# zhibaishouheilab/HealthiVert-GAN

Hardware: AMD Instinct MI355X
Metric: sagittal slices/sec (train step, G+D) at 256x256 bs=16 (higher is better)
Workload: dtype f16; 1 GPU; two-stage coarse+refine generator + 3x PatchGAN D train step, 256x256, per-GPU bs=16, norm=batch, vanilla GAN; global_batch=16, parallelism=dp1, launch=hipGraph replay (1 graphs/step), 4 streams

## Files before the change

healthivert-gan_amd/csrc/conv_g4.hip:

```cpp
#include <stdlib.h>
#include <type_traits>

#include "conv_halo.h"

struct G4K {
    const void* x; const _Float16* w; const float* bias; void* y; const void* mul_src;
    float* stats;
    const void* bn_x; const float* bn_stats; float* bstats;
    int bn_x_ld, bn_x_coff, bn_ipg;
    int B, H, W, x_ld, x_coff, Cin;
    int Ho, Wo, y_ld, y_coff, Cout;
    int mul_ld, mul_coff, mul_act, act, accumulate;
    float alpha;
    int tiles_x, tiles;
    int Hc, Wc;
    unsigned x_bytes, w_bytes, w_rb;
    int dbg;
};

typedef __attribute__((address_space(3))) void* lds_ptr;
__device__ __forceinline__ void lds_dma16(__amdgpu_buffer_rsrc_t r, lds_ptr dst, unsigned voff, int soff) {
#if defined(__HIP_DEVICE_COMPILE__)
    __builtin_amdgcn_raw_ptr_buffer_load_lds(r, dst, 16, voff, soff, 0, 0);
#endif
}

__device__ __forceinline__ void g4_load_bias(const G4K& p, int cob, int lane, f32x4 (&bias_r)[4]) {
    const __amdgpu_buffer_rsrc_t bsrc = __builtin_amdgcn_make_buffer_rsrc(const_cast<float*>(p.bias), 0, p.bias ? (unsigned)p.Cout * 4u : 0u, 0x00020000);
#pragma unroll
    for (int n = 0; n < 4; ++n)
        bias_r[n] = __builtin_bit_cast(f32x4, __builtin_amdgcn_raw_buffer_load_b128(bsrc, (unsigned)(cob + n * 16 + (lane >> 4) * 4) * 4u, 0, 0));
}

template <int MODE, int MT>
__device__ __forceinline__ void g4_epilogue(const G4K& p, f32x4 (&acc)[4][MT], char* smem, const int (&cls_s)[2], const int (&cob_s)[2], int n_img, int i0,
                                            int j0, const f32x4 (&bias_r)[4]) {
    constexpr int TW = 16, TH = 4 * MT, NTHR = 512, LDO = 128 + 8;
    const int tid = threadIdx.x, lane = tid & 63, wave = __builtin_amdgcn_readfirstlane(tid >> 6);
    const int wm = wave >> 1, wn = wave & 1;
    _Float16* As = reinterpret_cast<_Float16*>(smem);
    constexpr int OITEMS = TH * TW * 16 / NTHR;
    const __amdgpu_buffer_rsrc_t msrc = __builtin_amdgcn_make_buffer_rsrc(const_cast<void*>(p.mul_src), 0, p.mul_src ? 0x7ffffff0u : 0u, 0x00020000);
    const __amdgpu_buffer_rsrc_t ysrc = __builtin_amdgcn_make_buffer_rsrc(p.y, 0, p.accumulate ? 0x7ffffff0u : 0u, 0x00020000);
    u32x4 mreg[OITEMS], yreg[OITEMS];
    long long ooff[OITEMS];
#pragma unroll
    for (int k = 0; k < OITEMS; ++k) {
        const int it = tid + k * NTHR;
        const int q = it >> 4, pc = it & 15, s = pc >> 3;
        const int i = i0 + (q >> 4), j = j0 + (q & 15);
        const int ch = cob_s[s] + (pc & 7) * 8;
        const bool ok = i < p.Hc && j < p.Wc && ch < p.Cout;
        int ho = i, wo = j;
        if (MODE == 1) { ho = 2 * i + (cls_s[s] >> 1); wo = 2 * j + (cls_s[s] & 1); }
        const long long opix = (long long)(n_img * p.Ho + ho) * p.Wo + wo;
        ooff[k] = ok ? opix * p.y_ld + p.y_coff + ch : -1;
        mreg[k] = __builtin_amdgcn_raw_buffer_load_b128(msrc, ok ? (unsigned)((opix * p.mul_ld + p.mul_coff + ch) * 2) : HV_OOB, 0, 0);
        yreg[k] = __builtin_amdgcn_raw_buffer_load_b128(ysrc, ok ? (unsigned)(ooff[k] * 2) : HV_OOB, 0, 0);
    }
    _Float16* ot = As;
    auto stage = [&](auto actf) __attribute__((always_inline)) {
#pragma unroll
        for (int m = 0; m < MT; ++m) {
            const int q = (wm * MT + m) * 16 + (lane & 15);
#pragma unroll
            for (int n = 0; n < 4; ++n) {
                f16x4v h;
#pragma unroll
                for (int r = 0; r < 4; ++r) h[r] = (_Float16)actf(acc[n][m][r] * p.alpha + bias_r[n][r]);
                *reinterpret_cast<f16x4v*>(ot + q * LDO + wn * 64 + n * 16 + (lane >> 4) * 4) = h;
            }
        }
    };
    switch (p.act) {
        case HV_ACT_ELU:
            stage([](float v) { const float e = __builtin_amdgcn_exp2f(v * 1.44269504f) - 1.f, sm = v + 0.5f * v * v; return v > 0.f ? v : (v > -0.00390625f ? sm : e); });
            break;
        case HV_ACT_RELU: stage([](float v) { return v > 0.f ? v : 0.f; }); break;
        case HV_ACT_LRELU: stage([](float v) { return v > 0.f ? v : 0.2f * v; }); break;
        case HV_ACT_SIGMOID: stage([](float v) { return __builtin_amdgcn_rcpf(1.f + __builtin_amdgcn_exp2f(-v * 1.44269504f)); }); break;
        case HV_ACT_CLAMP: stage([](float v) { return fminf(fmaxf(v, -1.f), 1.f); }); break;
        default: stage([](float v) { return v; }); break;
    }
    __syncthreads();
    _Float16* yb = reinterpret_cast<_Float16*>(p.y);
    u32x4 o[OITEMS];
#pragma unroll
    for (int k = 0; k < OITEMS; ++k) {
        const int it = tid + k * NTHR;
        o[k] = *reinterpret_cast<const u32x4*>(ot + (it >> 4) * LDO + (it & 15) * 8);
    }
    if (MODE != 1 && p.stats) {
        float s1[8], s2[8];
#pragma unroll
        for (int e = 0; e < 8; ++e) s1[e] = s2[e] = 0.f;
#pragma unroll
        for (int k = 0; k < OITEMS; ++k) {
            if (ooff[k] < 0) continue;
            const f16x8 v8 = __builtin_bit_cast(f16x8, o[k]);
#pragma unroll
            for (int e = 0; e < 8; ++e) { const float v = (float)v8[e]; s1[e] += v; s2[e] += v * v; }
        }
        __syncthreads();
        float* red = reinterpret_cast<float*>(smem);
        float* mine = red + ((tid >> 4) * 16 + (tid & 15)) * 16;
#pragma unroll
        for (int e = 0; e < 8; ++e) { mine[e] = s1[e]; mine[8 + e] = s2[e]; }
        __syncthreads();
        if (tid < 256) {
            const int pc = tid >> 4, e = tid & 15;
            float s = 0.f;
#pragma unroll 8
            for (int r = 0; r < 32; ++r) s += red[(r * 16 + pc) * 16 + e];
            const int ch = (int)blockIdx.y * 128 + pc * 8 + (e & 7);
            if (ch < p.Cout) p.stats[((long long)blockIdx.x * p.Cout + ch) * 2 + (e >> 3)] = s;
        }
    }
    if (p.mul_src) {
        auto mulf = [&](auto gradf) __attribute__((always_inline)) {
#pragma unroll
            for (int k = 0; k < OITEMS; ++k) {
                const f16x8 m8 = __builtin_bit_cast(f16x8, mreg[k]);
                f16x8 v8 = __builtin_bit_cast(f16x8, o[k]);
#pragma unroll
                for (int e = 0; e < 8; ++e) v8[e] = (_Float16)((float)v8[e] * gradf((float)m8[e]));
                o[k] = __builtin_bit_cast(u32x4, v8);
            }
        };
        switch (p.mul_act) {
            case HV_ACT_ELU: mulf([](float y) { return y > 0.f ? 1.f : y + 1.f; }); break;
            case HV_ACT_RELU: mulf([](float y) { return y > 0.f ? 1.f : 0.f; }); break;
            case HV_ACT_LRELU: mulf([](float y) { return y > 0.f ? 1.f : 0.2f; }); break;
            case HV_ACT_SIGMOID: mulf([](float y) { return y * (1.f - y); }); break;
            case HV_ACT_CLAMP: mulf([](float y) { return (y > -1.f && y < 1.f) ? 1.f : 0.f; }); break;
            default: break;
        }
    }
    if (p.accumulate) {
#pragma unroll
        for (int k = 0; k < OITEMS; ++k) {
            const f16x8 y8 = __builtin_bit_cast(f16x8, yreg[k]);
            f16x8 v8 = __builtin_bit_cast(f16x8, o[k]);
#pragma unroll
            for (int e = 0; e < 8; ++e) v8[e] = (_Float16)((float)v8[e] + (float)y8[e]);
            o[k] = __builtin_bit_cast(u32x4, v8);
        }
    }
#pragma unroll
    for (int k = 0; k < OITEMS; ++k)
        if (ooff[k] >= 0) *reinterpret_cast<u32x4*>(yb + ooff[k]) = o[k];
    if (p.bstats) {
        const int pc = tid & 15, s = pc >> 3;
        const int ch0 = cob_s[s] + (pc & 7) * 8;
        const int grp = n_img / p.bn_ipg;
        const __amdgpu_buffer_rsrc_t xsrc = __builtin_amdgcn_make_buffer_rsrc(const_cast<void*>(p.bn_x), 0, 0x7ffffff0u, 0x00020000);
        u32x4 xreg[OITEMS];
#pragma unroll
        for (int k = 0; k < OITEMS; ++k) {
            const int q = (tid + k * NTHR) >> 4;
            int ho = i0 + (q >> 4), wo = j0 + (q & 15);
            if (MODE == 1) { ho = 2 * ho + (cls_s[s] >> 1); wo = 2 * wo + (cls_s[s] & 1); }
            const long long opix = (long long)(n_img * p.Ho + ho) * p.Wo + wo;
            xreg[k] = __builtin_amdgcn_raw_buffer_load_b128(xsrc, ooff[k] >= 0 ? (unsigned)((opix * p.bn_x_ld + p.bn_x_coff + ch0) * 2) : HV_OOB, 0, 0);
        }
        float s1[8], s2[8];
#pragma unroll
        for (int e = 0; e < 8; ++e) s1[e] = s2[e] = 0.f;
#pragma unroll
        for (int k = 0; k < OITEMS; ++k) {
            if (ooff[k] < 0) continue;
            const f16x8 v8 = __builtin_bit_cast(f16x8, o[k]), x8 = __builtin_bit_cast(f16x8, xreg[k]);
#pragma unroll
            for (int e = 0; e < 8; ++e) {
                const float g = (float)v8[e];
                s1[e] += g; s2[e] += g * (float)x8[e];
            }
        }
        __syncthreads();
        float* red = reinterpret_cast<float*>(smem);
        float* mine = red + ((tid >> 4) * 16 + (tid & 15)) * 16;
#pragma unroll
        for (int e = 0; e < 8; ++e) { mine[e] = s1[e]; mine[8 + e] = s2[e]; }
        __syncthreads();
        if (tid < 128) {
            const int pq = tid >> 3, e = tid & 7;
            float sg = 0.f, sgx = 0.f;
#pragma unroll 8
            for (int r = 0; r < 32; ++r) { sg += red[(r * 16 + pq) * 16 + e]; sgx += red[(r * 16 + pq) * 16 + 8 + e]; }
            const int sl = pq >> 3, ch = cob_s[sl] + (pq & 7) * 8 + e;
            const long long part = MODE == 1 ? (long long)blockIdx.x * 4 + cls_s[sl] : (long long)blockIdx.x;
            if (ch < p.Cout) {
                const float mean = p.bn_stats[(long long)grp * 2 * p.Cout + ch], rstd = p.bn_stats[(long long)grp * 2 * p.Cout + p.Cout + ch];
                float* o2 = p.bstats + (part * p.Cout + ch) * 2;
                o2[0] = sg;
                o2[1] = rstd * (sgx - mean * sg);
            }
        }
    }
}

template <int MODE, int MT>
__global__ __launch_bounds__(512, 2) void conv_g4_kernel(const G4K p) {
    constexpr int TW = 16, TH = 4 * MT, NTHR = 512;
    constexpr int PH = TH + 1 + MODE, PW = TW + 1 + MODE;
    constexpr int NBP = (PH * PW + 15) / 16;
    constexpr int BPW = (NBP + 7) / 8;
    constexpr int ABUF = 32 * 512;
    constexpr int BBUF = NBP * 512;
    constexpr int NBUF = 3;
    constexpr int LDO = 128 + 8;
    extern __shared__ __attribute__((aligned(16))) char smem[];
    _Float16* As = reinterpret_cast<_Float16*>(smem);
    _Float16* Bs = As + NBUF * ABUF;

    const int tid = threadIdx.x, lane = tid & 63, wave = __builtin_amdgcn_readfirstlane(tid >> 6);
#ifdef G4_STAMPS
    unsigned long long st[8];
#define G4_STAMP(i) st[i] = __builtin_amdgcn_s_memrealtime()
#else
#define G4_STAMP(i)
#endif
    G4_STAMP(0);
    const int wm = wave >> 1, wn = wave & 1;
    int t = (int)blockIdx.x;
    const int n_img = t / p.tiles;
    t -= n_img * p.tiles;
    const int tile_y = t / p.tiles_x, tile_x = t - tile_y * p.tiles_x;
    const int i0 = tile_y * TH, j0 = tile_x * TW;
    const int Cin = p.Cin, KC = Cin >> 5;
    const int NCH = MODE == 0 ? 4 * KC : KC;

    int cls_s[2], cob_s[2];
#pragma unroll
    for (int s = 0; s < 2; ++s) {
        if (MODE == 0) { cls_s[s] = 0; cob_s[s] = (int)blockIdx.y * 128 + s * 64; }
        else {
            const int nco = p.Cout >> 6, sl = (int)blockIdx.y * 2 + s;
            cls_s[s] = sl / nco; cob_s[s] = (sl - cls_s[s] * nco) * 64;
        }
    }
    const __amdgpu_buffer_rsrc_t wsrc = __builtin_amdgcn_make_buffer_rsrc(const_cast<_Float16*>(p.w), 0, p.w_bytes, 0x00020000);
    const __amdgpu_buffer_rsrc_t xsrc = __builtin_amdgcn_make_buffer_rsrc(const_cast<void*>(p.x), 0, p.x_bytes, 0x00020000);
    f32x4 bias_r[4];
    g4_load_bias(p, cob_s[wn], lane, bias_r);

    int pbase[BPW], pval[BPW];
    const int xbase = (n_img * p.H * p.W * p.x_ld + p.x_coff) * 2;
#pragma unroll
    for (int i = 0; i < BPW; ++i) {
        const int pix = (wave + 8 * i) * 16 + (lane >> 2);
        const int c8 = (lane & 3) ^ (((pix >> 2) & 1) << 1);
        const int pr = pix / PW, pc = pix - pr * PW;
        const bool in = pix < PH * PW && wave + 8 * i < NBP;
        if (MODE == 0) {
            const int r0 = 2 * (i0 + pr) - 1, c0 = 2 * (j0 + pc) - 1;
            pbase[i] = xbase + ((r0 * p.W + c0) * p.x_ld + c8 * 8) * 2;
            int v = 0;
#pragma unroll
            for (int dd = 0; dd < 4; ++dd)
                if (in && (unsigned)(r0 + (dd >> 1)) < (unsigned)p.H && (unsigned)(c0 + (dd & 1)) < (unsigned)p.W) v |= 1 << dd;
            pval[i] = v;
        } else {
            const int r0 = i0 - 1 + pr, c0 = j0 - 1 + pc;
            pbase[i] = xbase + ((r0 * p.W + c0) * p.x_ld + c8 * 8) * 2;
            pval[i] = (in && (unsigned)r0 < (unsigned)p.H && (unsigned)c0 < (unsigned)p.W) ? 15 : 0;
        }
    }
    constexpr int DMA_PER_CHUNK = 4 + BPW;
    auto issue = [&](int c, int b) __attribute__((always_inline)) {
        int dy = 0, dx = 0, kc = c;
        if (MODE == 0) { dy = c / (2 * KC); const int rem = c - dy * 2 * KC; dx = rem / KC; kc = rem - dx * KC; }
#pragma unroll
        for (int i = 0; i < 4; ++i) {
            const int f = wave + 8 * i, rbw = f >> 2, tt = f & 3, s = rbw >> 2;
            const int rb = (cob_s[s] >> 4) + (rbw & 3);
            int tap;
            if (MODE == 0) tap = (2 * (tt >> 1) + dy) * 4 + 2 * (tt & 1) + dx;
            else { const int py = cls_s[s] >> 1, px = cls_s[s] & 1; tap = (1 - py + 2 * (tt >> 1)) * 4 + (1 - px + 2 * (tt & 1)); }
            lds_dma16(wsrc, (lds_ptr)(As + b * ABUF + f * 512), (unsigned)lane * 16u, rb * (int)p.w_rb + (tap * Cin + kc * 32) * 32);
        }
        const int coff = MODE == 0 ? ((dy * p.W + dx) * p.x_ld + kc * 32) * 2 : kc * 64;
        const int vb = MODE == 0 ? dy * 2 + dx : 0;
#pragma unroll
        for (int i = 0; i < BPW; ++i) {
            _Float16* dst = wave + 8 * i < NBP ? Bs + b * BBUF + (wave + 8 * i) * 512 : Bs + NBUF * BBUF;
            lds_dma16(xsrc, (lds_ptr)dst, ((pval[i] >> vb) & 1) ? (unsigned)(pbase[i] + coff) : HV_OOB, 0);
        }
    };

    int boffs[4][MT];
#pragma unroll
    for (int tt = 0; tt < 4; ++tt) {
        int dh, dw;
        if (MODE == 0) { dh = tt >> 1; dw = tt & 1; }
        else { const int py = cls_s[wn] >> 1, px = cls_s[wn] & 1; dh = py - (tt >> 1) + 1; dw = px - (tt & 1) + 1; }
#pragma unroll
        for (int m = 0; m < MT; ++m) {
            const int pix = (wm * MT + m + dh) * PW + (lane & 15) + dw;
            boffs[tt][m] = pix * 32 + (((lane >> 4) ^ (((pix >> 2) & 1) << 1)) << 3);
        }
    }
    f32x4 acc[4][MT];
#pragma unroll
    for (int n = 0; n < 4; ++n)
#pragma unroll
        for (int m = 0; m < MT; ++m) acc[n][m] = (f32x4){0.f, 0.f, 0.f, 0.f};
    const int aoff = (wn * 16) * 512 + lane * 8;

    f16x8 a[2][4], bf[2][MT];
    auto frags = [&](int b, int tt, int buf) __attribute__((always_inline)) {
        const _Float16* Ab = As + b * ABUF + aoff;
        const _Float16* Bb = Bs + b * BBUF;
#pragma unroll
        for (int n = 0; n < 4; ++n) a[buf][n] = *reinterpret_cast<const f16x8*>(Ab + (n * 4 + tt) * 512);
#pragma unroll
        for (int m = 0; m < MT; ++m) bf[buf][m] = *reinterpret_cast<const f16x8*>(Bb + boffs[tt][m]);
    };
    auto mfmas = [&](int buf) __attribute__((always_inline)) {
#ifdef G4_STAMPS
        if (p.dbg & 4) return;
#endif
#pragma unroll
        for (int m = 0; m < MT; ++m)
#pragma unroll
            for (int n = 0; n < 4; ++n) acc[n][m] = __builtin_amdgcn_mfma_f32_16x16x32_f16(a[buf][n], bf[buf][m], acc[n][m], 0, 0, 0);
    };
    auto chunk = [&](int c, int b) __attribute__((always_inline)) {
        const int bn = b == 2 ? 0 : b + 1;
#ifdef G4_STAMPS
        if (c + 2 < NCH && !(p.dbg & 1)) issue(c + 2, b == 0 ? 2 : b - 1);
#else
        if (c + 2 < NCH) issue(c + 2, b == 0 ? 2 : b - 1);
#endif
#pragma unroll
        for (int tt = 0; tt < 3; ++tt) {
            __builtin_amdgcn_sched_barrier(0);
            frags(b, tt + 1, (tt + 1) & 1);
            mfmas(tt & 1);
#pragma unroll
            for (int i = 0; i < 4 + MT; ++i) {
                __builtin_amdgcn_sched_group_barrier(0x100, 1, 0);
                __builtin_amdgcn_sched_group_barrier(0x008, (4 * MT) / (4 + MT), 0);
            }
            __builtin_amdgcn_sched_barrier(0);
        }
        if (c + 2 < NCH) __builtin_amdgcn_s_waitcnt(0x0070 | (DMA_PER_CHUNK & 15) | ((DMA_PER_CHUNK >> 4) << 14));
        else __builtin_amdgcn_s_waitcnt(0x0070);
        __builtin_amdgcn_s_barrier();
        if (c + 1 < NCH) frags(bn, 0, 0);
        mfmas(1);
#pragma unroll
        for (int i = 0; i < 4 + MT; ++i) {
            __builtin_amdgcn_sched_group_barrier(0x100, 1, 0);
            __builtin_amdgcn_sched_group_barrier(0x008, (4 * MT) / (4 + MT), 0);
        }
        __builtin_amdgcn_sched_barrier(0);
    };
    issue(0, 0);
    if (NCH > 1) issue(1, 1);
    G4_STAMP(1);
    if (NCH > 1) __builtin_amdgcn_s_waitcnt(0x0F70 | (DMA_PER_CHUNK & 15) | ((DMA_PER_CHUNK >> 4) << 14));
    else __builtin_amdgcn_s_waitcnt(0x0F70);
    __builtin_amdgcn_s_barrier();
    G4_STAMP(2);
    frags(0, 0, 0);
    for (int c = 0; c < NCH; c += 3) {
        chunk(c, 0);
        if (c + 1 < NCH) chunk(c + 1, 1);
        if (c + 2 < NCH) chunk(c + 2, 2);
    }
    __syncthreads();
    G4_STAMP(3);

    g4_epilogue<MODE, MT>(p, acc, smem, cls_s, cob_s, n_img, i0, j0, bias_r);
#ifdef G4_STAMPS
    __builtin_amdgcn_s_waitcnt(0);
    G4_STAMP(5);
    if (tid == 0 && blockIdx.x == gridDim.x / 2 && blockIdx.y == 0) {
        unsigned long long* d = reinterpret_cast<unsigned long long*>(p.y);
        for (int i = 0; i < 6; ++i) d[i] = st[i];
    }
#endif
}

template <int DG, int MT>
__device__ __forceinline__ void conv_g4s1_body(const G4K& p) {
    constexpr int TW = 16, TH = 4 * MT, PH = TH + 3, PW = 20;
    constexpr int NBP = (PH * PW + 15) / 16, BPW = (NBP + 7) / 8;
    static_assert(BPW <= 4, "one patch piece per tap");
    constexpr int ABUF = 32 * 512, BBUF = NBP * 512;
    extern __shared__ __attribute__((aligned(16))) char smem[];
    _Float16* As = reinterpret_cast<_Float16*>(smem);
    _Float16* Bs = As + 3 * ABUF;
    const int tid = threadIdx.x, lane = tid & 63, wave = __builtin_amdgcn_readfirstlane(tid >> 6);
    const int wm = wave >> 1, wn = wave & 1;
#ifdef G4_STAMPS
    unsigned long long st[8];
    st[0] = __builtin_amdgcn_s_memrealtime();
#endif
    int t = (int)blockIdx.x;
    const int n_img = t / p.tiles;
    t -= n_img * p.tiles;
    const int tile_y = t / p.tiles_x, tile_x = t - tile_y * p.tiles_x;
    const int i0 = tile_y * TH, j0 = tile_x * TW;
    const int Cin = p.Cin, KC = Cin >> 5, NS = 4 * KC;
    int cls_s[2] = {0, 0}, cob_s[2] = {(int)blockIdx.y * 128, (int)blockIdx.y * 128 + 64};
    const __amdgpu_buffer_rsrc_t wsrc = __builtin_amdgcn_make_buffer_rsrc(const_cast<_Float16*>(p.w), 0, p.w_bytes, 0x00020000);
    const __amdgpu_buffer_rsrc_t xsrc = __builtin_amdgcn_make_buffer_rsrc(const_cast<void*>(p.x), 0, p.x_bytes, 0x00020000);
    f32x4 bias_r[4];
    g4_load_bias(p, cob_s[wn], lane, bias_r);
    constexpr int ORG = DG ? 2 : 1;
    unsigned pvo[BPW];
    const int xbase = (n_img * p.H * p.W * p.x_ld + p.x_coff) * 2;
#pragma unroll
    for (int i = 0; i < BPW; ++i) {
        const int pix = (wave + 8 * i) * 16 + (lane >> 2);
        const int c8 = (lane & 3) ^ (((pix >> 2) & 1) << 1);
        const int pr = pix / PW, pc = pix - pr * PW;
        const int r0 = i0 - ORG + pr, c0 = j0 - ORG + pc;
        const bool ok = wave + 8 * i < NBP && pr < PH && pc < PW - 1 && (unsigned)r0 < (unsigned)p.H && (unsigned)c0 < (unsigned)p.W;
        pvo[i] = ok ? (unsigned)(xbase + ((r0 * p.W + c0) * p.x_ld + c8 * 8) * 2) : HV_OOB;
    }
    auto issueA = [&](int kc, int kh, int ab) __attribute__((always_inline)) {
#pragma unroll
        for (int i = 0; i < 4; ++i) {
            const int f = wave + 8 * i, rbw = f >> 2, kw = f & 3;
            const int rb = (cob_s[rbw >> 2] >> 4) + (rbw & 3);
            lds_dma16(wsrc, (lds_ptr)(As + ab * ABUF + f * 512), (unsigned)lane * 16u, rb * (int)p.w_rb + ((kh * 4 + kw) * Cin + kc * 32) * 32);
        }
    };
    auto issueA1 = [&](int kc, int kh, int ab, int i, bool live) __attribute__((always_inline)) {
        const int f = wave + 8 * i, rbw = f >> 2, kw = f & 3;
        const int rb = (cob_s[rbw >> 2] >> 4) + (rbw & 3);
        lds_dma16(wsrc, (lds_ptr)(As + ab * ABUF + f * 512), live ? (unsigned)lane * 16u : HV_OOB, rb * (int)p.w_rb + ((kh * 4 + kw) * Cin + kc * 32) * 32);
    };
    auto issueB1 = [&](int kc, int bb, int i, bool live) __attribute__((always_inline)) {
        _Float16* dst = wave + 8 * i < NBP ? Bs + bb * BBUF + (wave + 8 * i) * 512 : Bs + 2 * BBUF;
        lds_dma16(xsrc, (lds_ptr)dst, live ? pvo[i] : HV_OOB, kc * 64);
    };
    auto issueB = [&](int kc, int bb) __attribute__((always_inline)) {
#pragma unroll
        for (int i = 0; i < BPW; ++i) {
            _Float16* dst = wave + 8 * i < NBP ? Bs + bb * BBUF + (wave + 8 * i) * 512 : Bs + 2 * BBUF;
            lds_dma16(xsrc, (lds_ptr)dst, pvo[i], kc * 64);
        }
    };
    int bo[2][4][MT];
#pragma unroll
    for (int kw = 0; kw < 4; ++kw)
#pragma unroll
        for (int m = 0; m < MT; ++m) {
            const int pix = (wm * MT + m) * PW + (lane & 15) + (DG ? 3 - kw : kw);
            const int s0 = (pix >> 2) & 1;
            bo[0][kw][m] = pix * 32 + (((lane >> 4) ^ (s0 << 1)) << 3);
            bo[1][kw][m] = pix * 32 + (((lane >> 4) ^ ((s0 ^ 1) << 1)) << 3);
        }
    f32x4 acc[4][MT];
#pragma unroll
    for (int n = 0; n < 4; ++n)
#pragma unroll
        for (int m = 0; m < MT; ++m) acc[n][m] = (f32x4){0.f, 0.f, 0.f, 0.f};
    const int aoff = (wn * 16) * 512 + lane * 8;
    f16x8 a[2][4], bf[2][MT];
    auto sub = [&](int kc, auto KH, int ab) __attribute__((always_inline)) {
        constexpr int kh = decltype(KH)::value;
        constexpr int rs = DG ? 3 - kh : kh;
        const int s_ = kc * 4 + kh;
        constexpr int kh2 = (kh + 2) & 3;
        const int kc2 = kc + (kh >= 2 ? 1 : 0);
        const int ab2 = ab == 0 ? 2 : ab - 1;
        const bool live = s_ + 2 < NS;
        const _Float16* Ab = As + ab * ABUF + aoff;
        const _Float16* Bb = Bs + (kc & 1) * BBUF + rs * PW * 32;
        auto frags = [&](int kw, int buf) __attribute__((always_inline)) {
#pragma unroll
            for (int n = 0; n < 4; ++n) a[buf][n] = *reinterpret_cast<const f16x8*>(Ab + (n * 4 + kw) * 512);
#pragma unroll
            for (int m = 0; m < MT; ++m) bf[buf][m] = *reinterpret_cast<const f16x8*>(Bb + bo[rs & 1][kw][m]);
        };
        frags(0, 0);
#pragma unroll
        for (int kw = 0; kw < 4; ++kw) {
            __builtin_amdgcn_sched_barrier(0);
            issueA1(kc2, kh2, ab2, kw, live);
            if (kh == 2 && kw < BPW) issueB1(kc + 1, (kc + 1) & 1, kw, live);
            __builtin_amdgcn_sched_barrier(0);
            if (kw + 1 < 4) frags(kw + 1, (kw + 1) & 1);
#pragma unroll
            for (int m = 0; m < MT; ++m)
#pragma unroll
                for (int n = 0; n < 4; ++n) acc[n][m] = __builtin_amdgcn_mfma_f32_16x16x32_f16(a[kw & 1][n], bf[kw & 1][m], acc[n][m], 0, 0, 0);
            if (kw + 1 < 4) {
#pragma unroll
                for (int i = 0; i < 4 + MT; ++i) {
                    __builtin_amdgcn_sched_group_barrier(0x100, 1, 0);
                    __builtin_amdgcn_sched_group_barrier(0x008, (4 * MT) / (4 + MT), 0);
                }
            }
            __builtin_amdgcn_sched_barrier(0);
        }
        if (kh == 2) __builtin_amdgcn_s_waitcnt(0x0070 | ((4 + BPW) & 15));
        else __builtin_amdgcn_s_waitcnt(0x0070 | 4);
        __builtin_amdgcn_s_barrier();
    };
    issueB(0, 0);
    issueA(0, 0, 0);
    issueA(0, 1, 1);
    __builtin_amdgcn_s_waitcnt(0x0F70 | 4);
    __builtin_amdgcn_s_barrier();
#ifdef G4_STAMPS
    st[1] = __builtin_amdgcn_s_memrealtime();
#endif
    int ab = 0;
    for (int kc = 0; kc < KC; ++kc) {
        sub(kc, std::integral_constant<int, 0>(), ab); ab = ab == 2 ? 0 : ab + 1;
        sub(kc, std::integral_constant<int, 1>(), ab); ab = ab == 2 ? 0 : ab + 1;
        sub(kc, std::integral_constant<int, 2>(), ab); ab = ab == 2 ? 0 : ab + 1;
        sub(kc, std::integral_constant<int, 3>(), ab); ab = ab == 2 ? 0 : ab + 1;
    }
    __builtin_amdgcn_s_waitcnt(0x0F70);
    __syncthreads();
#ifdef G4_STAMPS
    st[2] = __builtin_amdgcn_s_memrealtime();
#endif
    g4_epilogue<0, MT>(p, acc, smem, cls_s, cob_s, n_img, i0, j0, bias_r);
#ifdef G4_STAMPS
    st[3] = __builtin_amdgcn_s_memrealtime();
    __builtin_amdgcn_s_waitcnt(0);
    st[4] = __builtin_amdgcn_s_memrealtime();
    if (tid == 0 && blockIdx.x == gridDim.x / 2 && blockIdx.y == 0) {
        unsigned long long* d = reinterpret_cast<unsigned long long*>(p.y);
        for (int i = 0; i < 5; ++i) d[i] = st[i];
    }
#endif
}

template <int DG, int MT>
__global__ __launch_bounds__(512, 2) void conv_g4s1_kernel(const G4K p) { conv_g4s1_body<DG, MT>(p); }

template <int DG, int MT>
static int launch_g4s1(G4K& k, int ny, hipStream_t s) {
    constexpr int TH = 4 * MT, PH = TH + 3, NBP = (PH * 20 + 15) / 16;
    constexpr size_t lds_loop = (size_t)(3 * 32 * 512 + (2 * NBP + 1) * 512) * 2, lds_out = (size_t)TH * 16 * 136 * 2, lds_red = 32 * 16 * 16 * 4;
    constexpr size_t lds = lds_loop > lds_out ? (lds_loop > lds_red ? lds_loop : lds_red) : (lds_out > lds_red ? lds_out : lds_red);
    static_assert(lds <= 160 * 1024, "LDS");
    k.tiles_x = hv_cdiv(k.Wc, 16);
    k.tiles = k.tiles_x * hv_cdiv(k.Hc, TH);
    auto kern = conv_g4s1_kernel<DG, MT>;
    static bool raised = false;
    if (!raised) {
        hipError_t e = hipFuncSetAttribute(reinterpret_cast<const void*>(kern), hipFuncAttributeMaxDynamicSharedMemorySize, 160 * 1024);
        if (e != hipSuccess) return -1000 - (int)e;
        raised = true;
    }
    hv_path_note = 8;
    HV_KNAME("conv_g4s1_kernel<%d, %d>", DG, MT);
    HV_WUSE(4);
    hipLaunchKernelGGL(kern, dim3(k.tiles * k.B, ny), dim3(512), lds, s, k);
    HV_LAUNCH_CHECK();
    return HV_OK;
}

template <int MODE, int MT>
static int launch_g4(G4K& k, int ny, hipStream_t s) {
    constexpr int TH = 4 * MT, PH = TH + 1 + MODE, PW = 17 + MODE;
    constexpr size_t lds_loop = (size_t)(3 * 32 * 512 + (3 * ((PH * PW + 15) / 16) + 1) * 512) * 2, lds_out = (size_t)TH * 16 * 136 * 2, lds_red = 32 * 16 * 16 * 4;
    constexpr size_t lds = lds_loop > lds_out ? (lds_loop > lds_red ? lds_loop : lds_red) : (lds_out > lds_red ? lds_out : lds_red);
    static_assert(lds <= 160 * 1024, "LDS");
    k.tiles_x = hv_cdiv(k.Wc, 16);
    k.tiles = k.tiles_x * hv_cdiv(k.Hc, TH);
    auto kern = conv_g4_kernel<MODE, MT>;
    static bool raised = false;
    if (!raised) {
        hipError_t e = hipFuncSetAttribute(reinterpret_cast<const void*>(kern), hipFuncAttributeMaxDynamicSharedMemorySize, 160 * 1024);
        if (e != hipSuccess) return -1000 - (int)e;
        raised = true;
    }
    hv_path_note = 8;
    HV_KNAME("conv_g4_kernel<%d, %d>", MODE, MT);
    HV_WUSE(4);
    hipLaunchKernelGGL(kern, dim3(k.tiles * k.B, ny), dim3(512), lds, s, k);
    HV_LAUNCH_CHECK();
    return HV_OK;
}

static int g4_tile_rows(int B, int Hc, int Wc, int ny) {
    return (long long)B * hv_cdiv(Hc, 16) * hv_cdiv(Wc, 16) * ny >= 200 ? 16 : 8;
}

size_t hv_conv2d_g4_bstats_parts(const hv_conv_desc* d);
static bool g4_eligible(const hv_conv_desc* d) {
    if (d->KH != 4 || d->KW != 4 || (d->stride != 2 && d->stride != 1) || d->pad != 1 || d->dil != 1 || d->in_shift || d->w_bstride || d->ch_scale) return false;
    if (d->precision != HV_F16 || !d->w_f16_tiled || !d->x_f16 || !d->y_f16 || d->accumulate > 1) return false;
    if (d->stride == 1) {
        if ((d->Cout & 127) || (d->Cin & 31)) return false;
    }
    if ((d->Cin & 31) || (d->Cout & 63) || (!d->transposed && (d->Cout & 127))) return false;
    if ((d->x_ld & 7) || (d->x_coff & 7) || ((uintptr_t)d->x & 15) || (d->y_ld & 7) || (d->y_coff & 7) || ((uintptr_t)d->y & 15) || ((uintptr_t)d->w_f16_tiled & 15))
        return false;
    if (d->mul_src && (!d->mul_f16 || (d->mul_ld & 7) || (d->mul_coff & 7) || ((uintptr_t)d->mul_src & 15))) return false;
    if (d->stride == 2 && !d->transposed && (d->Ho != d->H / 2 || d->Wo != d->W / 2 || (d->H & 1) || (d->W & 1))) return false;
    if (d->stride == 2 && d->transposed && (d->Ho != 2 * d->H || d->Wo != 2 * d->W)) return false;
    if (d->stride == 1 && (d->Ho != d->H + (d->transposed ? 1 : -1) || d->Wo != d->W + (d->transposed ? 1 : -1) || d->Ho < 1 || d->Wo < 1)) return false;
    if ((long long)d->B * d->H * d->W * d->x_ld >= (1ll << 30) || (long long)d->B * d->Ho * d->Wo * d->y_ld >= (1ll << 30)) return false;
    return true;
}

int hv_conv2d_g4(const hv_conv_desc* d, hipStream_t s) {
    if (!g4_eligible(d)) return HV_ERR_UNSUPPORTED;
    G4K k;
    k.dbg = 0;
#ifdef G4_STAMPS
    if (getenv("HV_G4_DBG")) k.dbg = atoi(getenv("HV_G4_DBG"));
#endif
    k.x = d->x; k.w = reinterpret_cast<const _Float16*>(d->w_f16_tiled); k.bias = d->bias; k.y = d->y; k.mul_src = d->mul_src;
    k.stats = d->transposed ? nullptr : d->stats;
    k.bn_x = nullptr; k.bn_stats = nullptr; k.bstats = nullptr; k.bn_x_ld = k.bn_x_coff = 0; k.bn_ipg = 1;
    if (d->bstats) {
        if (!hv_conv2d_g4_bstats_parts(d)) return HV_ERR_UNSUPPORTED;
        k.bn_x = d->bn_x; k.bn_stats = d->bn_stats; k.bstats = d->bstats; k.bn_x_ld = d->bn_x_ld; k.bn_x_coff = d->bn_x_coff;
        k.bn_ipg = d->B / (d->bn_groups > 0 ? d->bn_groups : 1);
    }
    k.B = d->B; k.H = d->H; k.W = d->W; k.x_ld = d->x_ld; k.x_coff = d->x_coff; k.Cin = d->Cin;
    k.Ho = d->Ho; k.Wo = d->Wo; k.y_ld = d->y_ld; k.y_coff = d->y_coff; k.Cout = d->Cout;
    k.mul_ld = d->mul_ld; k.mul_coff = d->mul_coff; k.mul_act = d->mul_act; k.act = d->act; k.accumulate = d->accumulate; k.alpha = d->alpha;
    k.x_bytes = (unsigned)((size_t)d->B * d->H * d->W * d->x_ld * 2);
    k.w_rb = (unsigned)(16 * 16 * d->Cin * 2);
    k.w_bytes = (unsigned)((size_t)hv_cdiv(d->Cout, 16) * k.w_rb);
    if (d->stride == 1) {
        k.Hc = d->Ho; k.Wc = d->Wo;
        const int ny = d->Cout / 128;
        k.stats = d->transposed ? nullptr : d->stats;
        if (g4_tile_rows(d->B, k.Hc, k.Wc, ny) == 16) return d->transposed ? launch_g4s1<1, 4>(k, ny, s) : launch_g4s1<0, 4>(k, ny, s);
        return d->transposed ? launch_g4s1<1, 2>(k, ny, s) : launch_g4s1<0, 2>(k, ny, s);
    }
    if (!d->transposed) {
        k.Hc = d->Ho; k.Wc = d->Wo;
        const int ny = d->Cout / 128;
        return g4_tile_rows(d->B, k.Hc, k.Wc, ny) == 16 ? launch_g4<0, 4>(k, ny, s) : launch_g4<0, 2>(k, ny, s);
    }
    k.Hc = d->H; k.Wc = d->W;
    const int ny = 2 * (d->Cout / 64);
    return g4_tile_rows(d->B, k.Hc, k.Wc, ny) == 16 ? launch_g4<1, 4>(k, ny, s) : launch_g4<1, 2>(k, ny, s);
}

size_t hv_conv2d_g4_bstats_parts(const hv_conv_desc* d) {
    if (!d->transposed || d->accumulate || !g4_eligible(d)) return 0;
    if (!d->bn_x || !d->bn_stats || !d->mul_src || (d->bn_x_ld & 7) || (d->bn_x_coff & 7) || ((uintptr_t)d->bn_x & 15) || ((uintptr_t)d->bn_stats & 15) || (d->Cout & 7)) return 0;
    const int G = d->bn_groups > 0 ? d->bn_groups : 1;
    if (d->B % G) return 0;
    if ((long long)d->B * d->Ho * d->Wo * d->bn_x_ld >= (1ll << 30)) return 0;
    if (d->stride == 1) {
        const int th = g4_tile_rows(d->B, d->Ho, d->Wo, d->Cout / 128);
        return (size_t)d->B * hv_cdiv(d->Ho, th) * hv_cdiv(d->Wo, 16);
    }
    const int th = g4_tile_rows(d->B, d->H, d->W, 2 * (d->Cout / 64));
    return (size_t)d->B * hv_cdiv(d->H, th) * hv_cdiv(d->W, 16) * 4;
}

size_t hv_conv2d_g4_stats_floats(const hv_conv_desc* d, int* nparts) {
    hv_conv_desc t = *d;
    if (t.transposed || t.accumulate || !g4_eligible(&t)) return 0;
    const int th = g4_tile_rows(t.B, t.Ho, t.Wo, t.Cout / 128);
    const int parts = t.B * hv_cdiv(t.Ho, th) * hv_cdiv(t.Wo, 16);
    if (nparts) *nparts = parts;
    return (size_t)parts * t.Cout * 2;
}
```

healthivert-gan_amd/csrc/conv_igemm.hip:

```cpp
#include <string.h>

#include "hv_common.h"
#include <stdlib.h>

#define HV_MAX_TAPS 25
#define HV_BK 32

thread_local int hv_path_note = 0;
thread_local int hv_wtable_used = 0;
extern "C" int hv_last_weight_tables(void) { return hv_wtable_used; }
thread_local char hv_kname[192] = "";
extern "C" const char* hv_last_kernel_name(void) { return hv_kname; }
extern "C" int hv_last_kernel_path(void) { return hv_path_note; }
thread_local hipEvent_t hv_ev_start = nullptr, hv_ev_stop = nullptr;
extern "C" int hv_set_kernel_timing(void* ev_start, void* ev_stop) {
    hv_ev_start = (hipEvent_t)ev_start; hv_ev_stop = (hipEvent_t)ev_stop;
    return HV_OK;
}

int hv_conv2d_halo(const hv_conv_desc* d, const void* w_f16, hipStream_t s);
int hv_conv2d_g4(const hv_conv_desc* d, hipStream_t s);
int hv_conv2d_thin_dgrad(const hv_conv_desc* d, hipStream_t s);
int hv_conv2d_logits_dgrad(const hv_conv_desc* d, hipStream_t s);
size_t hv_conv2d_g4_stats_floats(const hv_conv_desc* d, int* nparts);
size_t hv_conv2d_g4_bstats_parts(const hv_conv_desc* d);
size_t hv_conv2d_logits_bstats_parts(const hv_conv_desc* d);
size_t hv_wgrad_halo_workspace_bytes(const hv_wgrad_desc* d);
int hv_wgrad_halo(const hv_wgrad_desc* d, int* nslabs, hipStream_t s);
size_t hv_wgrad_tr_workspace_bytes(const hv_wgrad_desc* d);
int hv_wgrad_tr(const hv_wgrad_desc* d, int* nslabs, hipStream_t s);
int hv_wgrad_thin(const hv_wgrad_desc* d, int* nslabs, hipStream_t s);
size_t hv_wgrad_thin_workspace_bytes(const hv_wgrad_desc* d);
int hv_conv2d_narrow(const hv_conv_desc* d, hipStream_t s);
int hv_conv2d_thin_in(const hv_conv_desc* d, hipStream_t s);
int hv_conv2d_stem5(const hv_conv_desc* d, hipStream_t s);
int hv_conv2d_stem5_dgrad(const hv_conv_desc* d, hipStream_t s);
int hv_conv2d_head(const hv_conv_desc* d, hipStream_t s);
int hv_conv2d_px(const hv_conv_desc* d, hipStream_t s);
int hv_conv2d_s2t(const hv_conv_desc* d, hipStream_t s);

struct ConvCls {
    int ph, pw, Hc, Wc, ntaps, Ktot, m0, mcount;
    uint32_t taps[HV_MAX_TAPS];
};
struct ConvK {
    const void* x; const float* w; const float* bias; const float* scale; void* y;
    int x_half, y_half, mul_half;
    long long w_bs, scale_bs;
    int B, Hl, Wl, in_shift, Wp, img_stride, x_ld, x_coff, Cin;
    int Cout, w_row, y_ld, y_coff, Ho, Wo;
    int bstep, boff, ostep;
    float alpha; int act, accumulate, vec_store, ncls;
    int xcd_swizzle;
    const void* mul_src; int mul_ld, mul_coff, mul_act, mul_vec;
    ConvCls cls[4];
};

template <typename T> struct Stage;
template <> struct Stage<float> {
    static constexpr int LD = HV_BK + 4;
    static __device__ __forceinline__ void st4(float* dst, float4 v) { *reinterpret_cast<float4*>(dst) = v; }
};
template <> struct Stage<_Float16> {
    static constexpr int LD = HV_BK + 8;
    static __device__ __forceinline__ void st4(_Float16* dst, float4 v) {
        f16x4 h = {(_Float16)v.x, (_Float16)v.y, (_Float16)v.z, (_Float16)v.w};
        *reinterpret_cast<f16x4*>(dst) = h;
    }
};

template <typename T, int MT, int NT> struct Frags;
template <int MT, int NT> struct Frags<float, MT, NT> {
    float4 w[NT][2], x[MT][2];
    __device__ __forceinline__ void load(const float* Bs, const float* As, int wrow0, int xrow0, int lane) {
        const int off = (lane & 15) * Stage<float>::LD + (lane >> 4) * 8;
#pragma unroll
        for (int n = 0; n < NT; ++n) {
            const float* p = Bs + (wrow0 + n * 16) * Stage<float>::LD + off;
            w[n][0] = *reinterpret_cast<const float4*>(p);
            w[n][1] = *reinterpret_cast<const float4*>(p + 4);
        }
#pragma unroll
        for (int m = 0; m < MT; ++m) {
            const float* p = As + (xrow0 + m * 16) * Stage<float>::LD + off;
            x[m][0] = *reinterpret_cast<const float4*>(p);
            x[m][1] = *reinterpret_cast<const float4*>(p + 4);
        }
    }
    __device__ __forceinline__ void mma(f32x4 (&acc)[NT][MT]) {
#pragma unroll
        for (int n = 0; n < NT; ++n)
#pragma unroll
            for (int m = 0; m < MT; ++m) {
                f32x4 a = acc[n][m];
                a = __builtin_amdgcn_mfma_f32_16x16x4f32(w[n][0].x, x[m][0].x, a, 0, 0, 0);
                a = __builtin_amdgcn_mfma_f32_16x16x4f32(w[n][0].y, x[m][0].y, a, 0, 0, 0);
                a = __builtin_amdgcn_mfma_f32_16x16x4f32(w[n][0].z, x[m][0].z, a, 0, 0, 0);
                a = __builtin_amdgcn_mfma_f32_16x16x4f32(w[n][0].w, x[m][0].w, a, 0, 0, 0);
                a = __builtin_amdgcn_mfma_f32_16x16x4f32(w[n][1].x, x[m][1].x, a, 0, 0, 0);
                a = __builtin_amdgcn_mfma_f32_16x16x4f32(w[n][1].y, x[m][1].y, a, 0, 0, 0);
                a = __builtin_amdgcn_mfma_f32_16x16x4f32(w[n][1].z, x[m][1].z, a, 0, 0, 0);
                a = __builtin_amdgcn_mfma_f32_16x16x4f32(w[n][1].w, x[m][1].w, a, 0, 0, 0);
                acc[n][m] = a;
            }
    }
};
template <int MT, int NT> struct Frags<_Float16, MT, NT> {
    f16x8 w[NT], x[MT];
    __device__ __forceinline__ void load(const _Float16* Bs, const _Float16* As, int wrow0, int xrow0, int lane) {
        const int off = (lane & 15) * Stage<_Float16>::LD + (lane >> 4) * 8;
#pragma unroll
        for (int n = 0; n < NT; ++n) w[n] = *reinterpret_cast<const f16x8*>(Bs + (wrow0 + n * 16) * Stage<_Float16>::LD + off);
#pragma unroll
        for (int m = 0; m < MT; ++m) x[m] = *reinterpret_cast<const f16x8*>(As + (xrow0 + m * 16) * Stage<_Float16>::LD + off);
    }
    __device__ __forceinline__ void mma(f32x4 (&acc)[NT][MT]) {
#pragma unroll
        for (int n = 0; n < NT; ++n)
#pragma unroll
            for (int m = 0; m < MT; ++m) acc[n][m] = __builtin_amdgcn_mfma_f32_16x16x32_f16(w[n], x[m], acc[n][m], 0, 0, 0);
    }
};

template <typename T, int BM, int BN, int WM, int WN, bool ASC, bool XH>
__global__ __launch_bounds__(256) void conv_igemm_kernel(const ConvK p) {
    constexpr int LD = Stage<T>::LD;
    constexpr int APASS = BM / 32;
    constexpr int BPASS = (BN + 31) / 32;
    constexpr int TMW = BM / WM, TNW = BN / WN;
    constexpr int MT = TMW / 16, NT = TNW / 16;
    static_assert(WM * WN == 4 && MT >= 1 && NT >= 1, "bad tile");
    __shared__ __attribute__((aligned(16))) T As[BM * LD];
    __shared__ __attribute__((aligned(16))) T Bs[BN * LD];
    __shared__ uint32_t taps_s[32];

    const int tid = threadIdx.x, lane = tid & 63, wave = tid >> 6;
    int bx = blockIdx.x;
    if (p.xcd_swizzle) {
        const int q = gridDim.x >> 3, r = gridDim.x & 7, xcd = bx & 7, loc = bx >> 3;
        bx = xcd < r ? xcd * (q + 1) + loc : r * (q + 1) + (xcd - r) * q + loc;
    }
    int ci = 0;
#pragma unroll
    for (int i = 1; i < 4; ++i)
        if (i < p.ncls && bx >= p.cls[i].m0) ci = i;
    const ConvCls& C = p.cls[ci];
    const int ntaps = C.ntaps, Ktot = C.Ktot, Hc = C.Hc, Wc = C.Wc, Mc = C.mcount, ph = C.ph, pw = C.pw;
    if (tid < ntaps) taps_s[tid] = C.taps[tid];
    const int m_base = (bx - C.m0) * BM;
    const int n_base = blockIdx.y * BN;
    const int HWc = Hc * Wc;

    const int chunk = tid & 7, prow = tid >> 3;
    int a_nb[APASS], a_hw[APASS];
    const int sample0 = m_base / HWc;
#pragma unroll
    for (int i = 0; i < APASS; ++i) {
        const int m = m_base + prow + i * 32;
        int bh = -20000, bw = -20000, nb = 0;
        if (m < Mc) {
            const int n = m / HWc, rem = m - n * HWc;
            const int ii = rem / Wc, jj = rem - ii * Wc;
            bh = ii * p.bstep + p.boff;
            bw = jj * p.bstep + p.boff;
            nb = n * p.img_stride;
        }
        a_nb[i] = nb;
        a_hw[i] = (int)(((uint32_t)bh << 16) | ((uint32_t)bw & 0xffffu));
    }
    const float* wbase = p.w + (p.w_bs ? (long long)sample0 * p.w_bs : 0ll);
    const int nk = (Ktot + HV_BK - 1) / HV_BK;

    float4 ra[APASS], rb[BPASS];
    auto gload = [&](int kt) {
        const int kg = kt * HV_BK + chunk * 4;
        if (!ASC) {
            const bool kok = kg < Ktot;
            int tapi = 0, c = 0, dh = 0, dw = 0, widx = 0;
// ... 26 lines not shown
            int dh[4], dw[4], wo[4], cc[4];
            bool kok[4];
#pragma unroll
            for (int e4 = 0; e4 < 4; ++e4) {
                const int k = kg + e4;
                kok[e4] = k < Ktot;
                const int tapi = kok[e4] ? k / p.Cin : 0;
                cc[e4] = k - tapi * p.Cin;
                const uint32_t e = taps_s[tapi];
                dh[e4] = (int)(int8_t)(e & 0xff);
                dw[e4] = (int)(int8_t)((e >> 8) & 0xff);
                wo[e4] = (int)(e >> 16) * p.Cin + cc[e4];
            }
#pragma unroll
            for (int i = 0; i < APASS; ++i) {
                float v[4];
#pragma unroll
                for (int e4 = 0; e4 < 4; ++e4) {
                    const int hi = (a_hw[i] >> 16) + dh[e4], wi = (int)(int16_t)(a_hw[i] & 0xffff) + dw[e4];
                    v[e4] = 0.f;
                    if (kok[e4] && (unsigned)hi < (unsigned)p.Hl && (unsigned)wi < (unsigned)p.Wl)
                        v[e4] = hv_ld1(p.x, a_nb[i] + ((hi >> p.in_shift) * p.Wp + (wi >> p.in_shift)) * p.x_ld + p.x_coff + cc[e4], XH);
                }
                ra[i] = make_float4(v[0], v[1], v[2], v[3]);
            }
#pragma unroll
            for (int i = 0; i < BPASS; ++i) {
                const int r = prow + i * 32, n = n_base + r;
                float v[4];
#pragma unroll
                for (int e4 = 0; e4 < 4; ++e4) v[e4] = (kok[e4] && r < BN && n < p.Cout) ? wbase[(long long)n * p.w_row + wo[e4]] : 0.f;
                rb[i] = make_float4(v[0], v[1], v[2], v[3]);
            }
        }
    };
    auto lstore = [&]() {
#pragma unroll
        for (int i = 0; i < APASS; ++i) Stage<T>::st4(As + (prow + i * 32) * LD + chunk * 4, ra[i]);
#pragma unroll
        for (int i = 0; i < BPASS; ++i) {
            const int r = prow + i * 32;
            if (r < BN) Stage<T>::st4(Bs + r * LD + chunk * 4, rb[i]);
        }
    };

    f32x4 acc[NT][MT];
#pragma unroll
    for (int n = 0; n < NT; ++n)
#pragma unroll
        for (int m = 0; m < MT; ++m) acc[n][m] = (f32x4){0.f, 0.f, 0.f, 0.f};

    const int wm = wave / WN, wn = wave % WN;
    __syncthreads();
    if (nk > 0) {
        gload(0);
        lstore();
    }
    __syncthreads();
    Frags<T, MT, NT> fr;
    for (int kt = 0; kt < nk; ++kt) {
        const bool more = kt + 1 < nk;
        if (more) gload(kt + 1);
        fr.load(Bs, As, wn * TNW, wm * TMW, lane);
        fr.mma(acc);
        __syncthreads();
        if (more) lstore();
        __syncthreads();
    }

    const float* scale = p.scale ? p.scale + (p.scale_bs ? (long long)sample0 * p.scale_bs : 0ll) : nullptr;
    const HvEpi epi = {p.alpha, p.act, p.accumulate, p.vec_store, p.Cout, p.bias, scale, p.mul_act, p.mul_vec, p.y_half, p.mul_half};
#pragma unroll
    for (int m = 0; m < MT; ++m) {
        const int mm = m_base + wm * TMW + m * 16 + (lane & 15);
        if (mm >= Mc) continue;
        const int n = mm / HWc, rem = mm - n * HWc;
        const int ii = rem / Wc, jj = rem - ii * Wc;
        const int ho = ph + ii * p.ostep, wo = pw + jj * p.ostep;
        const long long opix = (long long)(n * p.Ho + ho) * p.Wo + wo;
        void* yp = hv_eptr(p.y, opix * p.y_ld + p.y_coff, p.y_half);
        const void* mp = p.mul_src ? hv_eptr(p.mul_src, opix * p.mul_ld + p.mul_coff, p.mul_half) : nullptr;
#pragma unroll
        for (int nn = 0; nn < NT; ++nn) {
            const int ch0 = n_base + wn * TNW + nn * 16 + (lane >> 4) * 4;
            hv_conv_epilogue4<!std::is_same<T, float>::value>(epi, acc[nn][m], ch0, yp, mp);
        }
    }
}

template <typename T, int BM, int BN, int WM, int WN, bool ASC>
static int launch_conv(const ConvK& k, int mtiles, hipStream_t s) {
    dim3 grid(mtiles, hv_cdiv(k.Cout, BN));
    const bool xh = sizeof(T) == 2 && k.x_half;
    HV_KNAME("conv_igemm_kernel<%s, %d, %d, %d, %d, %s, %s>", sizeof(T) == 2 ? "_Float16" : "float", BM, BN, WM, WN, ASC ? "true" : "false", xh ? "true" : "false");
    if constexpr (sizeof(T) == 2) {
        if (xh) {
            hipLaunchKernelGGL((conv_igemm_kernel<T, BM, BN, WM, WN, ASC, true>), grid, dim3(256), 0, s, k);
            HV_LAUNCH_CHECK();
            return HV_OK;
        }
    }
    hipLaunchKernelGGL((conv_igemm_kernel<T, BM, BN, WM, WN, ASC, false>), grid, dim3(256), 0, s, k);
    HV_LAUNCH_CHECK();
    return HV_OK;
}

template <typename T, bool ASC>
static int dispatch_conv(ConvK& k, hipStream_t s) {
    long long M = 0;
    for (int c = 0; c < k.ncls; ++c) M += k.cls[c].mcount;
    int BM, BN;
    if (k.Cout <= 16) { BN = 16; BM = 256; }
    else if (k.Cout <= 32) { BN = 32; BM = 256; }
    else if (k.Cout <= 64) { BN = 64; BM = 128; }
    else { BN = 128; BM = 128; }
    if (BN >= 64) {
        long long tiles = ((M + BM - 1) / BM) * ((k.Cout + BN - 1) / BN);
        constexpr long long kSmallTiles = 600;
        if (tiles < kSmallTiles) { BM = 64; BN = 64; }
    } else if (BN == 16 && (M + 255) / 256 < 256) {
        BM = 64;
    }
    if (k.w_bs || k.scale_bs) {
        for (int c = 0; c < k.ncls; ++c)
            if ((k.cls[c].Hc * k.cls[c].Wc) % BM) {
                if ((k.cls[c].Hc * k.cls[c].Wc) % 64 == 0) { BM = 64; BN = 64; }
                else return HV_ERR_UNSUPPORTED;
            }
    }
    int mt = 0;
    for (int c = 0; c < k.ncls; ++c) {
        k.cls[c].m0 = mt;
        mt += hv_cdiv(k.cls[c].mcount, BM);
    }
    if (mt <= 0) return HV_OK;
    {
        const int gy = (k.Cout + BN - 1) / BN;
        k.xcd_swizzle = (mt >= 64 && (gy == 1 || (mt & 7) == 0)) ? 1 : 0;
    }
    if (BM == 256 && BN == 16) return launch_conv<T, 256, 16, 4, 1, ASC>(k, mt, s);
    if (BM == 64 && BN == 16) return launch_conv<T, 64, 16, 4, 1, ASC>(k, mt, s);
    if (BM == 256 && BN == 32) return launch_conv<T, 256, 32, 4, 1, ASC>(k, mt, s);
    if (BM == 128 && BN == 64) return launch_conv<T, 128, 64, 2, 2, ASC>(k, mt, s);
    if (BM == 128 && BN == 128) return launch_conv<T, 128, 128, 2, 2, ASC>(k, mt, s);
    return launch_conv<T, 64, 64, 2, 2, ASC>(k, mt, s);
}

extern "C" size_t hv_conv2d_bstats_parts(const hv_conv_desc* d) {
    if (!d || !d->transposed || d->precision != HV_F16) return 0;
    if (d->Cin == 4 && d->KH == 4 && d->stride == 1) return hv_conv2d_logits_bstats_parts(d);
    return hv_conv2d_g4_bstats_parts(d);
}

static int conv2d_dispatch(const hv_conv_desc* d, void* stream) {
    hv_wtable_used = 0;
    if (!d || !d->x || !d->w || !d->y) return HV_ERR_ARG;
    if (d->B <= 0 || d->H <= 0 || d->W <= 0 || d->Cin <= 0 || d->Cout <= 0 || d->KH <= 0 || d->KW <= 0 ||
        d->stride <= 0 || d->dil <= 0 || d->pad < 0 || d->Ho <= 0 || d->Wo <= 0)
        return HV_ERR_ARG;
    if (d->KH * d->KW > HV_MAX_TAPS || d->in_shift < 0 || d->in_shift > 1) return HV_ERR_UNSUPPORTED;
    if (d->in_shift && ((d->H | d->W) & 1)) return HV_ERR_UNSUPPORTED;
    if (d->x_ld < d->x_coff + d->Cin || d->y_ld < d->y_coff + d->Cout) return HV_ERR_ARG;
    if (d->act < HV_ACT_NONE || d->act > HV_ACT_CLAMP) return HV_ERR_ARG;
    if (d->precision != HV_F32 && d->precision != HV_F16) return HV_ERR_ARG;
    if (d->precision == HV_F32 && (d->x_f16 || d->y_f16 || d->mul_f16)) return HV_ERR_UNSUPPORTED;
    const int Hp = d->H >> d->in_shift, Wp = d->W >> d->in_shift;
    if ((long long)d->B * Hp * Wp * d->x_ld >= (1ll << 31) || (long long)d->B * d->Ho * d->Wo * d->y_ld >= (1ll << 31))
        return HV_ERR_UNSUPPORTED;
    if (d->H > 16000 || d->W > 16000 || (d->KH - 1) * d->dil > 120 || (d->KW - 1) * d->dil > 120) return HV_ERR_UNSUPPORTED;

    if (d->stats && !hv_conv2d_g4_stats_floats(d, nullptr)) return HV_ERR_UNSUPPORTED;
    if (d->bstats && !hv_conv2d_bstats_parts(d)) return HV_ERR_UNSUPPORTED;
    if (d->xn_stats) {
        if (d->Cout != 1 || !d->workspace) return HV_ERR_UNSUPPORTED;
        return hv_conv2d_head(d, (hipStream_t)stream);
    }
    if (d->x1) {
        if (d->precision != HV_F16 || !d->w_f16 || !d->w_f16_tiled || !d->y_f16 || d->transposed || d->dil != 1 || d->stride != 1 || d->KH != 3 || d->KW != 3 || !d->w1 ||
            d->pool2 || d->stats || d->x1_ld < 1)
            return HV_ERR_UNSUPPORTED;
        return hv_conv2d_halo(d, d->w_f16, (hipStream_t)stream);
    }
    if (d->pool2) {
        if (d->precision != HV_F16 || !d->w_f16 || !d->y_f16 || (d->Ho & 1) || (d->Wo & 1) || d->dil != 1 || d->stride != 1 || d->KH != 3 || d->KW != 3 || d->bias ||
            d->act != HV_ACT_NONE || d->in_shift || d->stats)
            return HV_ERR_UNSUPPORTED;
        return hv_conv2d_halo(d, d->w_f16, (hipStream_t)stream);
    }
    if (d->precision == HV_F16 && d->Cin <= 16 && d->Cout <= 16 && d->stride == 1) {
        const int rc = hv_conv2d_px(d, (hipStream_t)stream);
        if (rc != HV_ERR_UNSUPPORTED) return rc;
    }
    constexpr int kNarrowMaxCin = 15;
    const bool halo_ok = d->precision == HV_F16 && d->w_f16 && d->dil == 1 && (d->Cin & 15) == 0 && !d->w_bstride && !d->ch_scale;
    if (d->Cout == 1 && d->workspace) {
        const int rc = hv_conv2d_head(d, (hipStream_t)stream);
        if (rc != HV_ERR_UNSUPPORTED) return rc;
    }
    if (d->Cout == 1 && !d->transposed && !d->mul_src && !(halo_ok && d->Cin > kNarrowMaxCin)) {
        const int rc = hv_conv2d_narrow(d, (hipStream_t)stream);
        if (rc != HV_ERR_UNSUPPORTED) return rc;
    }
    if (d->Cin <= 4 && !d->transposed && !d->mul_src) {
        const int rc = hv_conv2d_thin_in(d, (hipStream_t)stream);
        if (rc != HV_ERR_UNSUPPORTED) return rc;
    }
    if (d->Cin == 4 && d->KH == 5 && d->precision == HV_F16 && d->w_f16) {
        const int rc = hv_conv2d_stem5(d, (hipStream_t)stream);
        if (rc != HV_ERR_UNSUPPORTED) return rc;
    }
    if (d->Cout == 4 && d->Cin == 16 && d->KH == 5 && d->transposed && d->precision == HV_F16 && d->w_f16) {
        const int rc = hv_conv2d_stem5_dgrad(d, (hipStream_t)stream);
        if (rc != HV_ERR_UNSUPPORTED) return rc;
    }
    if (d->precision == HV_F16 && d->transposed && d->Cin == 4 && d->KH == 4 && d->stride == 1) {
        const int rc = hv_conv2d_logits_dgrad(d, (hipStream_t)stream);
        if (rc != HV_ERR_UNSUPPORTED) return rc;
    }
    if (d->precision == HV_F16 && d->transposed && d->Cin <= 4 && d->KH == 3) {
        const int rc = hv_conv2d_thin_dgrad(d, (hipStream_t)stream);
        if (rc != HV_ERR_UNSUPPORTED) return rc;
    }
    if (d->precision == HV_F16 && d->w_f16 && d->KH == 4 && d->w_f16_tiled) {
        const int rc = hv_conv2d_g4(d, (hipStream_t)stream);
        if (rc != HV_ERR_UNSUPPORTED) return rc;
    }
    if (d->precision == HV_F16 && d->w_f16 && d->transposed && d->stride == 2) {
        const int rc = hv_conv2d_s2t(d, (hipStream_t)stream);
        if (rc != HV_ERR_UNSUPPORTED) return rc;
    }
    if (d->precision == HV_F16 && d->w_f16) {
        const int rc = hv_conv2d_halo(d, d->w_f16, (hipStream_t)stream);
        if (rc != HV_ERR_UNSUPPORTED) return rc;
    }
    ConvK k;
    k.x_half = d->x_f16 ? 1 : 0; k.y_half = d->y_f16 ? 1 : 0; k.mul_half = d->mul_f16 ? 1 : 0;
    k.x = d->x; k.w = d->w; k.bias = d->bias; k.scale = d->ch_scale; k.y = d->y;
    k.w_bs = d->w_bstride; k.scale_bs = d->ch_scale ? d->ch_scale_bstride : 0;
    k.mul_src = d->mul_src; k.mul_ld = d->mul_ld; k.mul_coff = d->mul_coff; k.mul_act = d->mul_act;
    k.mul_vec = (d->mul_src && !(d->mul_ld & 3) && !(d->mul_coff & 3) && !((uintptr_t)d->mul_src & 15)) ? 1 : 0;
    k.B = d->B; k.Hl = d->H; k.Wl = d->W; k.in_shift = d->in_shift; k.Wp = Wp; k.img_stride = Hp * Wp * d->x_ld;
    k.x_ld = d->x_ld; k.x_coff = d->x_coff; k.Cin = d->Cin;
    k.Cout = d->Cout; k.w_row = d->KH * d->KW * d->Cin; k.y_ld = d->y_ld; k.y_coff = d->y_coff; k.Ho = d->Ho; k.Wo = d->Wo;
    k.alpha = d->alpha; k.act = d->act; k.accumulate = d->accumulate;
    k.vec_store = ((d->y_ld & 3) == 0 && (d->y_coff & 3) == 0 && ((uintptr_t)d->y & 15) == 0) ? 1 : 0;
    if (!d->transposed) {
        const int eh = (d->H + 2 * d->pad - d->dil * (d->KH - 1) - 1) / d->stride + 1;
        const int ew = (d->W + 2 * d->pad - d->dil * (d->KW - 1) - 1) / d->stride + 1;
        if (eh != d->Ho || ew != d->Wo) return HV_ERR_ARG;
        k.ncls = 1; k.bstep = d->stride; k.boff = -d->pad; k.ostep = 1;
        ConvCls& c = k.cls[0];
        c.ph = c.pw = 0; c.Hc = d->Ho; c.Wc = d->Wo; c.ntaps = d->KH * d->KW; c.Ktot = c.ntaps * d->Cin;
        c.mcount = d->B * d->Ho * d->Wo;
        for (int r = 0; r < d->KH; ++r)
            for (int s = 0; s < d->KW; ++s) {
                const int t = r * d->KW + s;
                c.taps[t] = (uint32_t)(uint8_t)(int8_t)(r * d->dil) | ((uint32_t)(uint8_t)(int8_t)(s * d->dil) << 8) | ((uint32_t)t << 16);
            }
    } else {
        if (d->stride > 2) return HV_ERR_UNSUPPORTED;
        k.bstep = 1; k.boff = 0; k.ostep = d->stride; k.ncls = 0;
        for (int ph = 0; ph < d->stride; ++ph)
            for (int pw = 0; pw < d->stride; ++pw) {
                ConvCls& c = k.cls[k.ncls];
                c.ph = ph; c.pw = pw;
                c.Hc = (d->Ho - ph + d->stride - 1) / d->stride;
                c.Wc = (d->Wo - pw + d->stride - 1) / d->stride;
                if (c.Hc <= 0 || c.Wc <= 0) continue;
                c.ntaps = 0;
                for (int r = 0; r < d->KH; ++r) {
                    const int vh = ph + d->pad - r * d->dil;
                    if (((vh % d->stride) + d->stride) % d->stride) continue;
                    for (int s = 0; s < d->KW; ++s) {
                        const int vw = pw + d->pad - s * d->dil;
                        if (((vw % d->stride) + d->stride) % d->stride) continue;
                        const int dh = vh / d->stride, dw = vw / d->stride;
                        if (dh < -127 || dh > 127 || dw < -127 || dw > 127) return HV_ERR_UNSUPPORTED;
                        c.taps[c.ntaps++] = (uint32_t)(uint8_t)(int8_t)dh | ((uint32_t)(uint8_t)(int8_t)dw << 8) |
                                            ((uint32_t)(r * d->KW + s) << 16);
                    }
                }
                c.Ktot = c.ntaps * d->Cin;
                c.mcount = d->B * c.Hc * c.Wc;
                ++k.ncls;
            }
        if (k.ncls == 0) return HV_ERR_ARG;
    }
    const bool vec_in = (d->Cin & 3) == 0 && (d->x_ld & 3) == 0 && (d->x_coff & 3) == 0 && ((uintptr_t)d->x & 15) == 0 &&
                        ((uintptr_t)d->w & 15) == 0 && (d->w_bstride & 3) == 0;
    hipStream_t s = (hipStream_t)stream;
    hv_path_note = 0;
    HV_WUSE(1);
    if (d->precision == HV_F32) return vec_in ? dispatch_conv<float, false>(k, s) : dispatch_conv<float, true>(k, s);
    return vec_in ? dispatch_conv<_Float16, false>(k, s) : dispatch_conv<_Float16, true>(k, s);
}

thread_local int hv_probe_only = 0;
extern "C" int hv_conv2d_supported(const hv_conv_desc* d) {
    if (!d) return 0;
    if (d->bstats && !hv_conv2d_bstats_parts(d)) return 0;
    if (!d->x1 && !d->pool2 && !d->xn_stats) return d->stats ? (hv_conv2d_g4_stats_floats(d, nullptr) ? 1 : 0) : 1;
    hv_probe_only = 1;
    const int rc = conv2d_dispatch(d, nullptr);
    hv_probe_only = 0;
    return rc == HV_OK ? 1 : 0;
}

extern "C" int hv_conv2d(const hv_conv_desc* d, void* stream) {
    HV_TIMING_BEGIN((hipStream_t)stream);
    const int rc = conv2d_dispatch(d, stream);
    HV_TIMING_END((hipStream_t)stream);
    return rc;
}

struct WgradK {
    const void* x; const void* g; float* out;
    int half;
    int B, Hl, Wl, in_shift, Wp, img_stride, x_ld, x_coff, Cin;
    int Ho, Wo, g_ld, g_coff, Cout;
    int KW, stride, pad, dil, J , M , chunk;
    int lw, lhw;
    int kt_q, kt_r;
    unsigned x_bytes, g_bytes;
    long long slab;
    float* bias_out;
};

typedef unsigned int u32x4 __attribute__((ext_vector_type(4)));
#define HV_OOB 0x80000000u

template <typename T, int BN, int BC, int WN, int WC, int KT, bool FAST, bool SH>
__global__ __launch_bounds__(WN * WC * 64) void wgrad_kernel(const WgradK p) {
    typedef HvSt<SH> SS;
    typedef typename SS::R SR;
    constexpr unsigned SB = SS::B;
    constexpr int NTHR = WN * WC * 64;
    constexpr bool F16 = sizeof(T) == 2;
    constexpr int LDG = F16 ? (KT + 16) : (BN + ((BN % 32 == 16) ? 0 : 16));
    constexpr int LDX = F16 ? (KT + 16) : (BC + ((BC % 32 == 16) ? 0 : 16));
    __shared__ __attribute__((aligned(16))) T Gs[F16 ? BN * LDG : KT * LDG];
    __shared__ __attribute__((aligned(16))) T Xs[F16 ? BC * LDX : KT * LDX];
    constexpr int TNW = BN / WN, TCW = BC / WC, NT = TNW / 16, CT = TCW / 16;
    static_assert(WN * WC == 4 && NT >= 1 && CT >= 1 && KT % 32 == 0 && (!F16 || KT % 64 == 0), "bad tile");
    constexpr int GI = (BN / 4) * (KT / 8);
    constexpr int XI = (BC / 4) * (KT / 8);
    constexpr int XPT = (XI + NTHR - 1) / NTHR;
    static_assert(GI <= NTHR && (XI <= NTHR || XI % NTHR == 0), "one G item per thread; X items fill whole thread passes");

    const int tid = threadIdx.x, lane = tid & 63, wave = tid >> 6;
    const int n_base = blockIdx.y * BN, j_base = blockIdx.z * BC;
    const int pix_begin = blockIdx.x * p.chunk;
    const int pix_end = min(p.M, pix_begin + p.chunk);
    const int HWo = p.Ho * p.Wo;

    const bool has_g = tid < GI;
    const int xt = XI < NTHR ? tid - (NTHR - XI) : tid;
    const bool has_x = xt >= 0;
    const int g_cg = tid % (BN / 4), g_run = tid / (BN / 4);
    int x_cg[XPT], x_run[XPT], dh[XPT], dw[XPT], cx[XPT];
    bool jok[XPT];
#pragma unroll
    for (int it = 0; it < XPT; ++it) {
        const int xi = (has_x ? xt : 0) + it * NTHR;
        x_cg[it] = xi % (BC / 4);
        x_run[it] = xi / (BC / 4);
        const int jx = j_base + x_cg[it] * 4;
        jok[it] = has_x && jx < p.J;
        dh[it] = dw[it] = cx[it] = 0;
        if (jok[it]) {
            const int tap = jx / p.Cin;
            cx[it] = jx - tap * p.Cin;
            const int r = tap / p.KW, q = tap - r * p.KW;
            dh[it] = r * p.dil - p.pad;
            dw[it] = q * p.dil - p.pad;
        }
    }
    const int gch = n_base + g_cg * 4;
    const bool gok = has_g && gch < p.Cout;

    const __amdgpu_buffer_rsrc_t xsrc = __builtin_amdgcn_make_buffer_rsrc(const_cast<void*>(p.x), 0, p.x_bytes, 0x00020000);
    const __amdgpu_buffer_rsrc_t gsrc = __builtin_amdgcn_make_buffer_rsrc(const_cast<void*>(p.g), 0, p.g_bytes, 0x00020000);

    int xs_n[XPT], xs_ho[XPT], xs_wo[XPT];
#pragma unroll
    for (int it = 0; it < XPT; ++it) {
        xs_n[it] = xs_ho[it] = xs_wo[it] = 0;
        if (!FAST) {
            const int m0 = pix_begin + x_run[it] * 8;
            xs_n[it] = m0 / HWo;
            const int rem = m0 - xs_n[it] * HWo;
            xs_ho[it] = rem / p.Wo;
            xs_wo[it] = rem - xs_ho[it] * p.Wo;
        }
    }
    SR rg[8], rx[XPT][8];
    auto load_g = [&](int pix0) __attribute__((always_inline)) {
        const int m0 = pix0 + g_run * 8;
        if (FAST) {
            unsigned off = (gok && m0 < pix_end) ? (unsigned)(m0 * p.g_ld + p.g_coff + gch) * SB : HV_OOB;
            const unsigned step = (unsigned)p.g_ld * SB;
#pragma unroll
            for (int e = 0; e < 8; ++e, off += step) rg[e] = SS::ld(gsrc, off, 0);
        } else {
#pragma unroll
            for (int e = 0; e < 8; ++e) {
                const unsigned off = (gok && m0 + e < pix_end) ? (unsigned)((m0 + e) * p.g_ld + p.g_coff + gch) * SB : HV_OOB;
                rg[e] = SS::ld(gsrc, off, 0);
            }
        }
    };
    auto load_x1 = [&](int pix0, int it, SR (&r)[8]) __attribute__((always_inline)) {
        const int m0 = pix0 + x_run[it] * 8;
        if (FAST) {
            const int n = m0 >> p.lhw, ho = (m0 >> p.lw) & (p.Ho - 1), wo0 = m0 & (p.Wo - 1);
            const int hi = ho * p.stride + dh[it];
            const bool rok = jok[it] && m0 < pix_end && (unsigned)hi < (unsigned)p.Hl;
            const int base = n * p.img_stride + (hi >> p.in_shift) * p.Wp * p.x_ld + p.x_coff + cx[it];
            int wi = wo0 * p.stride + dw[it];
#pragma unroll
            for (int e = 0; e < 8; ++e, wi += p.stride) {
                const unsigned off = (rok && (unsigned)wi < (unsigned)p.Wl) ? (unsigned)(base + (wi >> p.in_shift) * p.x_ld) * SB : HV_OOB;
                r[e] = SS::ld(xsrc, off, 0);
            }
        } else if (p.Wo >= 8) {
            const int cross = p.Wo - xs_wo[it];
            int ho1 = xs_ho[it] + 1, n1 = xs_n[it];
            if (ho1 == p.Ho) { ho1 = 0; ++n1; }
            const int hiA = xs_ho[it] * p.stride + dh[it], hiB = ho1 * p.stride + dh[it];
            const bool rokA = jok[it] && (unsigned)hiA < (unsigned)p.Hl, rokB = jok[it] && (unsigned)hiB < (unsigned)p.Hl;
            const int baseA = xs_n[it] * p.img_stride + (hiA >> p.in_shift) * p.Wp * p.x_ld + p.x_coff + cx[it];
            const int baseB = n1 * p.img_stride + (hiB >> p.in_shift) * p.Wp * p.x_ld + p.x_coff + cx[it];
#pragma unroll
            for (int e = 0; e < 8; ++e) {
                const bool nb = e >= cross;
                const int wi = (xs_wo[it] + e - (nb ? p.Wo : 0)) * p.stride + dw[it];
                const bool ok = (nb ? rokB : rokA) && m0 + e < pix_end && (unsigned)wi < (unsigned)p.Wl;
                const unsigned off = ok ? (unsigned)((nb ? baseB : baseA) + (wi >> p.in_shift) * p.x_ld) * SB : HV_OOB;
                r[e] = SS::ld(xsrc, off, 0);
            }
        } else {
            int n = xs_n[it], ho = xs_ho[it], wo = xs_wo[it];
#pragma unroll
            for (int e = 0; e < 8; ++e) {
                const int hi = ho * p.stride + dh[it], wi = wo * p.stride + dw[it];
                const bool ok = jok[it] && m0 + e < pix_end && (unsigned)hi < (unsigned)p.Hl && (unsigned)wi < (unsigned)p.Wl;
                const unsigned off = ok ? (unsigned)(n * p.img_stride + ((hi >> p.in_shift) * p.Wp + (wi >> p.in_shift)) * p.x_ld + p.x_coff + cx[it]) * SB : HV_OOB;
                r[e] = SS::ld(xsrc, off, 0);
                if (++wo == p.Wo) { wo = 0; if (++ho == p.Ho) { ho = 0; ++n; } }
            }
        }
        if (!FAST) {
            xs_wo[it] += p.kt_r; xs_ho[it] += p.kt_q;
            if (xs_wo[it] >= p.Wo) { xs_wo[it] -= p.Wo; ++xs_ho[it]; }
// ... 354 lines not shown
```

healthivert-gan_amd/csrc/prep.hip:

```cpp
#include <stdlib.h>

#include "hv_common.h"

#define SN_EPS 1e-12f
#define PREP_THREADS 512
#define PREP_MAXK 4608
#define PREP_MAXCO 1024

__device__ __forceinline__ long long wsrc_index(const hv_wprep_layer& L, int co, int ci, int tap) {
    return L.transposed_src ? ((long long)ci * L.Cout + co) * L.taps + tap : ((long long)co * L.Cin + ci) * L.taps + tap;
}

__global__ __launch_bounds__(PREP_THREADS) void weight_prep_kernel(const hv_wprep_layer* __restrict__ layers) {
    const hv_wprep_layer L = layers[blockIdx.x];
    __shared__ float v_s[PREP_MAXK];
    __shared__ float u_s[PREP_MAXCO];
    __shared__ float red[20];
    const int tid = threadIdx.x, lane = tid & 63, wave = tid >> 6, nwave = PREP_THREADS / 64;
    const int K = L.Cin * L.taps;
    float sigma = 1.f;
    if (L.sn) {
        const float* W = L.w_orig;
        for (int i = tid; i < L.Cout; i += PREP_THREADS) u_s[i] = L.u[i];
        for (int i = tid; i < K; i += PREP_THREADS) v_s[i] = L.v[i];
// ... 551 lines not shown
    return HV_OK;
}

__global__ void adam_tick_kernel(float* step) { step[0] += 1.f; }

__global__ __launch_bounds__(256) void adam_kernel(const hv_adam_tensor* __restrict__ ts, const float* __restrict__ lr_p, float beta1,
                                                   float beta2, float eps, const float* __restrict__ step_p) {
    const hv_adam_tensor t = ts[blockIdx.y];
    const long long base = (long long)blockIdx.x * 1024;
    if (base >= t.n) return;
    const float step = step_p[0], lr = lr_p[0];
    const float bc1 = 1.f - powf(beta1, step), bc2 = 1.f - powf(beta2, step);
    const float step_size = lr / bc1, bc2_sqrt = sqrtf(bc2);
#pragma unroll
    for (int k = 0; k < 4; ++k) {
        const long long i = base + k * 256 + threadIdx.x;
        if (i < t.n) {
            const float g = t.g[i];
            const float m = t.m[i] + (g - t.m[i]) * (1.f - beta1);
            const float v = t.v[i] * beta2 + (1.f - beta2) * g * g;
            t.m[i] = m;
            t.v[i] = v;
            const float denom = sqrtf(v) / bc2_sqrt + eps;
            t.p[i] = t.p[i] - step_size * (m / denom);
        }
    }
}

__global__ __launch_bounds__(256) void grad_unscale_check_kernel(float* __restrict__ g, long long n, float mul, float* __restrict__ state) {
    bool bad = false;
    const bool scale = mul != 1.f;
    for (long long i = ((long long)blockIdx.x * 256 + threadIdx.x) * 4; i < n; i += (long long)gridDim.x * 1024) {
        if (i + 3 < n) {
            float4 v = *reinterpret_cast<const float4*>(g + i);
            bad |= !(fabsf(v.x) <= 3.0e38f) | !(fabsf(v.y) <= 3.0e38f) | !(fabsf(v.z) <= 3.0e38f) | !(fabsf(v.w) <= 3.0e38f);
            if (scale) { v.x *= mul; v.y *= mul; v.z *= mul; v.w *= mul; *reinterpret_cast<float4*>(g + i) = v; }
        } else {
            for (long long j = i; j < n; ++j) { bad |= !(fabsf(g[j]) <= 3.0e38f); if (scale) g[j] *= mul; }
        }
    }
    if (__any(bad) && (threadIdx.x & 63) == 0) { hv_publish(state + 1, 1.f); hv_stores_done(); }
    __syncthreads();
    if (threadIdx.x == 0) {
        unsigned* ticket = reinterpret_cast<unsigned*>(state + 4);
        if (hv_take_ticket_is_last(ticket, gridDim.x)) {
            const bool any_bad = hv_collect(state + 1) != 0.f;
            if (any_bad) state[2] += 1.f; else state[0] += 1.f;
            state[3] = any_bad ? 1.f : 0.f;
            hv_publish(state + 1, 0.f);
            hv_ticket_reset(ticket);
        }
    }
}
__global__ __launch_bounds__(256) void adam_guarded_kernel(const hv_adam_tensor* __restrict__ ts, const float* __restrict__ lr_p, float beta1,
                                                           float beta2, float eps, const float* __restrict__ state) {
    if (state[3] != 0.f) return;
    const hv_adam_tensor t = ts[blockIdx.y];
    const long long base = (long long)blockIdx.x * 1024;
    if (base >= t.n) return;
    const float step = state[0], lr = lr_p[0];
    const float bc1 = 1.f - powf(beta1, step), bc2 = 1.f - powf(beta2, step);
    const float step_size = lr / bc1, bc2_sqrt = sqrtf(bc2);
#pragma unroll
    for (int k = 0; k < 4; ++k) {
        const long long i = base + k * 256 + threadIdx.x;
        if (i < t.n) {
            const float g = t.g[i];
            const float m = t.m[i] + (g - t.m[i]) * (1.f - beta1);
            const float v = t.v[i] * beta2 + (1.f - beta2) * g * g;
            t.m[i] = m;
            t.v[i] = v;
            const float denom = sqrtf(v) / bc2_sqrt + eps;
            t.p[i] = t.p[i] - step_size * (m / denom);
        }
    }
}
extern "C" int hv_adam_step_guarded(const hv_adam_tensor* d_tensors, int n_tensors, long long max_numel, const float* d_lr, float beta1,
                                    float beta2, float eps, float* d_state, float* flat_grad, long long n_grad, float grad_mul, void* stream) {
    if (!d_tensors || n_tensors <= 0 || max_numel <= 0 || !d_lr || !d_state || !flat_grad || n_grad <= 0 || ((uintptr_t)flat_grad & 15) || !(grad_mul > 0.f))
        return HV_ERR_ARG;
    const int blocks = (int)(n_grad / 4096 + 1 < 256 ? n_grad / 4096 + 1 : 256);
    hipLaunchKernelGGL(grad_unscale_check_kernel, dim3(blocks), dim3(256), 0, (hipStream_t)stream, flat_grad, n_grad, grad_mul, d_state);
    HV_LAUNCH_CHECK();
    dim3 grid(hv_cdiv(max_numel, 1024), n_tensors);
    hipLaunchKernelGGL(adam_guarded_kernel, grid, dim3(256), 0, (hipStream_t)stream, d_tensors, d_lr, beta1, beta2, eps, d_state);
    HV_LAUNCH_CHECK();
    return HV_OK;
}

extern "C" int hv_adam_step(const hv_adam_tensor* d_tensors, int n_tensors, long long max_numel, const float* d_lr, float beta1,
                            float beta2, float eps, float* d_step, void* stream) {
    if (!d_tensors || n_tensors <= 0 || max_numel <= 0 || !d_lr || !d_step) return HV_ERR_ARG;
    hipLaunchKernelGGL(adam_tick_kernel, dim3(1), dim3(1), 0, (hipStream_t)stream, d_step);
    HV_LAUNCH_CHECK();
    dim3 grid(hv_cdiv(max_numel, 1024), n_tensors);
    hipLaunchKernelGGL(adam_kernel, grid, dim3(256), 0, (hipStream_t)stream, d_tensors, d_lr, beta1, beta2, eps, d_step);
    HV_LAUNCH_CHECK();
    return HV_OK;
}

__global__ void fill_kernel(float* p, long long n, float v) {
    long long i = (long long)blockIdx.x * blockDim.x + threadIdx.x;
    const long long st = (long long)gridDim.x * blockDim.x;
    for (; i < n; i += st) p[i] = v;
}
__global__ void axpy_kernel(float* y, const float* x, long long n, float a, int assign) {
    long long i = (long long)blockIdx.x * blockDim.x + threadIdx.x;
    const long long st = (long long)gridDim.x * blockDim.x;
    for (; i < n; i += st) y[i] = assign ? a * x[i] : y[i] + a * x[i];
}
static int ew_grid(long long n) { long long b = (n + 255) / 256; return (int)(b > 4096 ? 4096 : (b < 1 ? 1 : b)); }
extern "C" int hv_fill(float* p, long long n, float value, void* stream) {
    if (!p || n <= 0) return HV_ERR_ARG;
    hipLaunchKernelGGL(fill_kernel, dim3(ew_grid(n)), dim3(256), 0, (hipStream_t)stream, p, n, value);
    HV_LAUNCH_CHECK();
    return HV_OK;
}
extern "C" int hv_axpy(float* y, const float* x, long long n, float a, void* stream) {
    if (!y || !x || n <= 0) return HV_ERR_ARG;
    hipLaunchKernelGGL(axpy_kernel, dim3(ew_grid(n)), dim3(256), 0, (hipStream_t)stream, y, x, n, a, 0);
    HV_LAUNCH_CHECK();
    return HV_OK;
}
__global__ void affine_kernel(float* y, const float* x, long long n, float a, float b) {
    long long i = (long long)blockIdx.x * blockDim.x + threadIdx.x;
    const long long st = (long long)gridDim.x * blockDim.x;
    for (; i < n; i += st) y[i] = a * x[i] + b;
}
extern "C" int hv_affine(float* y, const float* x, long long n, float a, float b, void* stream) {
    if (!y || !x || n <= 0) return HV_ERR_ARG;
    hipLaunchKernelGGL(affine_kernel, dim3(ew_grid(n)), dim3(256), 0, (hipStream_t)stream, y, x, n, a, b);
    HV_LAUNCH_CHECK();
    return HV_OK;
}

__global__ void mul_kernel(float* y, const float* x, const float* z, long long n) {
    long long i = (long long)blockIdx.x * blockDim.x + threadIdx.x;
    const long long st = (long long)gridDim.x * blockDim.x;
    for (; i < n; i += st) y[i] = z ? (y[i] * x[i]) * z[i] : y[i] * x[i];
}
extern "C" int hv_mul(float* y, const float* x, long long n, void* stream) {
    if (!y || !x || n <= 0) return HV_ERR_ARG;
    hipLaunchKernelGGL(mul_kernel, dim3(ew_grid(n)), dim3(256), 0, (hipStream_t)stream, y, x, (const float*)nullptr, n);
    HV_LAUNCH_CHECK();
    return HV_OK;
}
extern "C" int hv_mul3(float* y, const float* x, const float* z, long long n, void* stream) {
    if (!y || !x || !z || n <= 0) return HV_ERR_ARG;
    hipLaunchKernelGGL(mul_kernel, dim3(ew_grid(n)), dim3(256), 0, (hipStream_t)stream, y, x, z, n);
    HV_LAUNCH_CHECK();
    return HV_OK;
}

extern "C" int hv_version(void) { return 104; }
extern "C" const char* hv_arch(void) { return "gfx950"; }
```

healthivert-gan_amd/engine.py:

```python
import contextlib
import ctypes
import os
import types

import torch

from . import lib as _lib
from . import ops
from .lib import ptr, stream
from .ops import Act, rup


def precision_note(precision):
    if precision in ('fp16', 'f16'):
        return 'fp16 MFMA operands / fp32 accumulate; activations and gradients stored as fp16 (image tensors, attention scores, weights, statistics fp32)'
    return 'fp32 MFMA (v_mfma_f32_16x16x4_f32), fp32 storage'


class ConvParams:

    def __init__(self, name, weight, bias, cin, cout, k, cin_fwd=None, cin_wg=None, u=None, v=None, transposed_src=False):
        self.name, self.weight, self.bias = name, weight, bias
        self.cin, self.cout, self.k, self.taps = cin, cout, k, k * k
        self.cin_fwd = rup(cin, 4) if cin_fwd is None else cin_fwd
# ... 56 lines not shown
        for c in self.convs:
            a, b, d = c.sizes()
            c.w_fwd = store[off:off + a]; off += a
            c.w_bwd = store[off:off + b]; off += b
            c.dw = store[off:off + d]; off += d
            c.sigma = store[off:off + 4]; off += 4
            c.sigma[0] = 1.0
        self._store = store
        hstore = torch.zeros(sum(c.sizes()[0] + c.sizes()[1] + 16 for c in self.convs), dtype=torch.float16, device=device)
        off = 0
        for c in self.convs:
            a, b, _ = c.sizes()
            c.w_fwd_h = hstore[off:off + a]; off += (a + 7) // 8 * 8
            c.w_bwd_h = hstore[off:off + b]; off += (b + 7) // 8 * 8
        self._hstore = hstore
        tsz = [(ops.tiled_elems(c.cout, c.taps, c.cin_fwd), ops.tiled_elems(c.cin_fwd, c.taps, c.coutP),
                ops.tiled_elems(c.cout, c.taps, c.split_k) if c.split_k else 0) for c in self.convs]
        tstore = torch.zeros(sum(a + b + e for a, b, e in tsz) + 8, dtype=torch.float16, device=device)
        off = 0
        for c, (a, b, e) in zip(self.convs, tsz):
            c.w_fwd_t = tstore[off:off + a] if a else None; off += a
            c.w_bwd_t = tstore[off:off + b] if b else None; off += b
            c.w_fwd_t2 = tstore[off:off + e] if e else None; off += e
        self._tstore = tstore
        ps = self.trainable()
        n = sum(p.numel() for p in ps)
        home = getattr(self, 'grad_home', None)
        if home is not None and home.numel() == n and home.device == torch.device(device) and home.dtype == torch.float32:
            self.flat_grad = home
            self.flat_grad.zero_()
        else:
            self.flat_grad = torch.zeros(n, dtype=torch.float32, device=device)
        self.grad_factor = 1.0
        off = 0
        for p in ps:
            p.grad = self.flat_grad[off:off + p.numel()].view_as(p)
            off += p.numel()
        for pi in (True, False):
            self.t_prep[pi].update(self._prep_rows(pi, False), key, device)
        for acc in (True, False):
            rows = []
            for c in self.convs:
                rows.append(dict(dw_ohwi=c.dw, w_fwd=c.w_fwd, u=c.u if c.sn else None, v=c.v if c.sn else None, sigma=c.sigma,
                                 dw_orig=c.weight.grad, Cout=c.cout, Cin=c.cin, taps=c.taps,
                                 CinP=c.coutP if c.transposed_src else c.cin_wg, sn=int(c.sn),
                                 transposed_src=int(c.transposed_src), accumulate=int(acc)))
            self.t_bwd[acc].update(rows, key, device)

    def attach_grads(self):
        self.grad_factor = 1.0
        off = 0
        for p in self.trainable():
            n = p.numel()
            if p.grad is None or p.grad.data_ptr() != self.flat_grad.data_ptr() + 4 * off:
                p.grad = self.flat_grad[off:off + n].view_as(p)
            off += n

    def _prep_rows(self, pi, lean):
        rows = []
        for c in self.convs:
            mf = mb = 7
            if lean and not c.transposed_src:
                mf = (c.use_fwd or 7) | (1 if c.sn else 0)
                mb = c.use_bwd or 7
            rows.append(dict(w_orig=c.weight.data, u=c.u if c.sn else None, v=c.v if c.sn else None, sigma=c.sigma,
                             w_fwd=c.w_fwd if mf & 1 else None, w_bwd=c.w_bwd if mb & 1 else None, w_fwd_h=c.w_fwd_h if mf & 2 else None,
                             w_bwd_h=c.w_bwd_h if mb & 2 else None, w_fwd_t=c.w_fwd_t if mf & 4 else None, w_bwd_t=c.w_bwd_t if mb & 4 else None,
                             Cout=c.cout, Cin=c.cin, taps=c.taps, CinP=c.cin_fwd, CoutF=c.cout, CoutP=c.coutP, CinB=c.cin_fwd, sn=int(c.sn),
                             power_iter=int(pi and c.sn), transposed_src=int(c.transposed_src), w_fwd_t2=c.w_fwd_t2, K2=int(c.split_k or 0)))
        return rows

    def weights_changed(self):
        self.version += 1

    def prep(self, device, power_iter, only_if_stale=False):
        self._ensure(device)
        pi = bool(power_iter)
        table = self.t_prep[pi]
        tset = 'full'
        if LEAN and ops.precision_id(None) == ops.F16:
            tset = tuple((c.use_fwd, c.use_bwd) for c in self.convs)
        if only_if_stale and not pi and PREP_SKIP and self.prepared is not None and self.prepared[0] == self.version and self.prepared[1] in ('full', tset):
            return
        self.prepared = (self.version, tset)
        if LEAN and ops.precision_id(None) == ops.F16:
            key = (self._key, pi, tuple((c.use_fwd, c.use_bwd) for c in self.convs))
            table = self.t_lean.get(key)
            if table is None:
                table = self.t_lean[key] = ops.LayerTable('hv_wprep_layer')
                table.update(self._prep_rows(pi, True), key, device)
        ops.weight_prep(table, max(c.sizes()[0] + c.sizes()[1] for c in self.convs), any_sn=any(c.sn for c in self.convs),
                        any_legacy=any(c.transposed_src for c in self.convs))

    def fold_chain(self):
        h = torch.cuda.current_stream().cuda_stream
        c = self.fold_chains.get(h)
        if c is None:
            c = self.fold_chains[h] = ops.FoldChain(h)
        return c

    def flush_folds(self):
        h = torch.cuda.current_stream().cuda_stream
        for k, c in self.fold_chains.items():
            if k == h:
                c.flush()
            else:
                assert c.pending is None, 'a weight-gradient fold chain of another stream was not flushed before finish_backward()'

    def finish_backward(self, accumulate=False):
        self.flush_folds()
        ops.weight_prep_backward(self.t_bwd[bool(accumulate)], max(c.cout * c.cin * c.taps for c in self.convs), any(c.sn for c in self.convs))


class ConvNode:
    __slots__ = ('p', 'x', 'y', 'k', 's', 'pad', 'd', 'act', 'shift', 'need_dx', 'transposed', 'use_bias', 'dx_c', 'pool_to', 'split', 'full')

    def __init__(self, p, x, y, s=1, pad=0, d=1, act='none', shift=0, need_dx=True, transposed=False, use_bias=True, dx_c=None):
        self.p, self.x, self.y, self.k, self.s, self.pad, self.d = p, x, y, p.k, s, pad, d
        self.act, self.shift, self.need_dx, self.transposed, self.use_bias = act, shift, need_dx, transposed, use_bias
        self.dx_c = dx_c
        self.pool_to = None
        self.split = None
        self.full = None

    def forward_call(self, prec, xn=None, x_raw=None):
        p = self.p
        kw = dict(bias=p.bias if self.use_bias else None, act=self.act, w_h=p.w_fwd_h, precision=prec, cout=p.cout, wuse=(p, 'use_fwd'))
        if self.split is not None and p.w_fwd_t2 is not None and ops.precision_id(prec) == ops.F16:
            low, x1 = self.split
            if low.f16 and self.y.f16 and low.C == p.split_k:
                call = ops.ConvCall(low, p.w_fwd, self.y, self.k, self.s, self.pad, self.d, w_t=p.w_fwd_t2, in_shift=1, cin=p.split_k,
                                    x1=(x1, p.w_fwd, p.split_k, p.taps * p.cin_fwd, p.cin_fwd), **kw)
                if call.supported():
                    return call
        src = self.x if x_raw is None else x_raw
        return ops.ConvCall(Act(src.t, p.cin_fwd, src.coff), p.w_fwd, self.y, self.k, self.s, self.pad, self.d, w_t=p.w_fwd_t, in_shift=self.shift,
                            transposed=self.transposed, xn=xn, **kw)

    def split_forward(self, prec):
        return bool(self.forward_call(prec).d.x1)

    def forward(self, prec, stats=None, xn=None, x_raw=None):
        self.forward_call(prec, xn, x_raw).launch(stats)

    def stats_parts(self, prec):
        return self.forward_call(prec).stats_parts()

    def dx_view(self, book, form):
        a = self.pool_to[0] if form == 'pool_to' else self.x
        g = book.twin(a)
        C = a.C if form == 'pool_to' else self.p.cin_fwd
        return Act(g.t, C if form == 'src' else self.dx_c or C, g.coff)

    def dx_call(self, book, prec, form, dst, accumulate, mul_x=None, bn=None):
        p = self.p
        gy = book.twin(self.y)
        mul = None
        if form == 'pool_to' and self.pool_to[1] != 'none':
            mul = (Act(self.pool_to[0].t, dst.C, self.pool_to[0].coff), self.pool_to[1])
        elif form in ('pool', 'plain') and mul_x:
            mul = (Act(self.x.t, p.cin_fwd, self.x.coff), mul_x)
        return ops.ConvCall(Act(gy.t, p.coutP, gy.coff), p.w_bwd, dst, self.k, self.s, self.pad, self.d, transposed=form != 'src', pool2=form in ('pool', 'pool_to'),
                            accumulate=int(accumulate), precision=prec, w_h=p.w_bwd_h, w_t=p.w_bwd_t, mul=mul, bn=bn, wuse=(p, 'use_bwd'))

    def full_scratch(self):
        if self.full is None:
            x = self.x
            self.full = Act(torch.zeros(x.B, x.H * 2, x.W * 2, x.ld, dtype=x.t.dtype, device=x.t.device), self.p.cin_fwd, 0)
        return self.full

    def pooled(self, book, prec, form='pool', mul_x=None):
        dst = self.dx_view(book, form)
        return self.dx_call(book, prec, form, dst, book.accumulates(dst), mul_x=mul_x).supported()


NO_FORK_STREAMS = set()
_named_streams = {}


def named_stream(name, device, priority=0):
    dev = torch.device(device)
    key = (name, dev.index if dev.index is not None else torch.cuda.current_device(), priority)
    st = _named_streams.get(key)
    if st is None:
        st = _named_streams[key] = torch.cuda.Stream(device=dev, priority=priority)
    return st


PREP_SKIP = os.environ.get('HV_PREP_SKIP', '1') != '0'
LEAN = False


@contextlib.contextmanager
def lean_tables(on=True):
    global LEAN
    prev, LEAN = LEAN, bool(on)
    try:
        yield
    finally:
        LEAN = prev


SERIAL = False


class GradBook:

    def __init__(self):
        self.twins = {}
        self.written = set()
        self.side = None
        self._side_of = None
        self.wgrad_block = WgradBlock()

    def fork(self):
        cur = torch.cuda.current_stream()
        if self.side is None or self._side_of != cur.cuda_stream:
            self.side, self._side_of = named_stream('wgrad-side-of-%x' % cur.cuda_stream, cur.device), cur.cuda_stream
        self.side.wait_stream(cur)
        return self.side

    def join(self):
        if self.side is not None:
            torch.cuda.current_stream().wait_stream(self.side)

    def twin(self, a):
        t = self.twins.get(id(a.t))
        if t is None:
            t = torch.zeros_like(a.t)
            self.twins[id(a.t)] = t
        return Act(t, a.C, a.coff)

    def reset(self):
        self.written.clear()

    def accumulates(self, a):
        return (id(a.t), a.coff, a.C) in self.written

    def mark(self, a):
        acc = self.accumulates(a)
        self.written.add((id(a.t), a.coff, a.C))
        return acc


class WgradBlock:
    __slots__ = ('side', 'collecting', 'queue', 'later', 'pset')

    def __init__(self):
        self.side, self.collecting, self.queue, self.later, self.pset = None, False, [], [], None

    def open(self, pset, device):
        fork = not SERIAL and torch.cuda.current_stream().cuda_stream not in NO_FORK_STREAMS
        self.side = named_stream('generator-wgrad-block', device) if fork else None
        self.collecting, self.queue, self.later, self.pset = fork, [], [], pset

    def add(self, run):
        self.queue.append(run)

    def before_next_block(self, run):
        if self.collecting:
            self.later.append(run)
        else:
            run()

    def launch(self, keep_collecting=False):
        if self.side is None:
            return
        self.side.wait_stream(torch.cuda.current_stream())
        with torch.cuda.stream(self.side):
            for run in self.queue:
                run()
            self.pset.fold_chain().flush()
        self.queue, self.later, self.collecting = self.later, [], keep_collecting

    def join(self):
        assert not self.queue and not self.later, 'WgradBlock.join(): queued weight gradients were never launched'
        if self.side is not None:
            torch.cuda.current_stream().wait_stream(self.side)
        self.side, self.collecting = None, False


def _wgrad(node, p, xin, gfull, accumulate, prec, dbias=None, dbias_accumulate=False):
    chain = p.owner.fold_chain() if p.owner is not None else None
    if node.transposed:
        ops.conv2d_wgrad(gfull, xin, p.dw, node.k, node.s, node.pad, node.d, accumulate=accumulate, precision=prec, chain=chain)
    else:
        ops.conv2d_wgrad(xin, gfull, p.dw, node.k, node.s, node.pad, node.d, in_shift=node.shift, accumulate=accumulate, precision=prec,
                         dbias=dbias, dbias_accumulate=dbias_accumulate, chain=chain)


def conv_backward(node, book, prec, dbias_accumulate=False, wgrad_accumulate=False, wgrad=True, x_wg=None, premultiplied=False,
                  mul_x=None, dbias_done=False, bn=None):
    p = node.p
    assert bn is None or (node.need_dx and not node.transposed and node.pool_to is None and not node.shift), 'conv_backward: bn= needs the plain data-gradient branch'
    gy = book.twin(node.y)
    want_dbias = p.bias is not None and node.use_bias and wgrad and not dbias_done
    fuse_dbias = want_dbias and not node.transposed and p.coutP == p.cout
    if (node.act != 'none' and not premultiplied) or (want_dbias and not fuse_dbias):
        ops.act_backward(gy, node.y, 'none' if premultiplied else node.act, dbias=p.bias.grad if (want_dbias and not fuse_dbias) else None, dbias_accumulate=dbias_accumulate)
    gfull = Act(gy.t, p.coutP, gy.coff)
    if wgrad:
        xs = node.x if x_wg is None else x_wg
        xin = Act(xs.t, p.cin_wg, xs.coff)
        if book.wgrad_block.collecting:
            book.wgrad_block.add(lambda node=node, p=p, xin=xin, gfull=gfull, acc=wgrad_accumulate, db=p.bias.grad if fuse_dbias else None, dba=dbias_accumulate:
                                 _wgrad(node, p, xin, gfull, acc, prec, dbias=db, dbias_accumulate=dba))
        else:
            _wgrad(node, p, xin, gfull, wgrad_accumulate, prec, dbias=p.bias.grad if fuse_dbias else None, dbias_accumulate=dbias_accumulate)
    if not node.need_dx:
        return
    if node.transposed:
        form = 'src'
    elif node.pool_to is not None and node.pooled(book, prec, 'pool_to'):
        form = 'pool_to'
    elif node.shift:
        form = 'pool' if node.pooled(book, prec, 'pool', mul_x) else 'full'
    else:
        form = 'plain'
    if form == 'full':
        assert not mul_x
        full = node.full_scratch()
        node.dx_call(book, prec, 'full', full, False).launch()
        gx = node.dx_view(book, 'plain')
        ops.copy_channels(full, gx, mode=3, accumulate=book.mark(gx))
    else:
        dst = node.dx_view(book, form)
        node.dx_call(book, prec, form, dst, book.mark(dst), mul_x=mul_x, bn=bn).launch()


_branch_streams = {}


def branch_stream():
    if SERIAL:
        return None
    cur = torch.cuda.current_stream()
    if cur.cuda_stream in NO_FORK_STREAMS:
        return None
    key = cur.device.index
    st = _branch_streams.get(key)
    if st is None:
        st = _branch_streams[key] = named_stream('generator-branch', cur.device)
        NO_FORK_STREAMS.add(st.cuda_stream)
    return st


def chain_link(n, nxt, book, prec):
    if not (nxt is not None and n.need_dx and not n.transposed and nxt.act != 'none'
            and n.x.t is nxt.y.t and n.x.coff == nxt.y.coff and n.p.cin_fwd <= nxt.y.t.shape[-1] - nxt.y.coff):
        return False
    return not n.shift or n.pooled(book, prec, 'pool', nxt.act)


def conv_backward_chain(nodes, book, prec, premultiplied_first=False, stop_before=None):
    pre = premultiplied_first
    for i, n in enumerate(nodes):
        nxt = nodes[i + 1] if i + 1 < len(nodes) else stop_before
        link = chain_link(n, nxt, book, prec)
        conv_backward(n, book, prec, premultiplied=pre, mul_x=nxt.act if link else None)
        pre = link


CA_GRAM = True
CA_GEMM = True


def _bgemm(A, B, C, M, N, K, batch, alpha=1.0, colscale=None, b_split=0):
    _lib.get().call('hv_bgemm_nt_h' if C.dtype == torch.float16 else 'hv_bgemm_nt', ptr(A), int(A.dtype == torch.float16), K, ctypes.c_longlong(M * K), ptr(B), int(B.dtype == torch.float16), K,
                    ctypes.c_longlong(N * K), ptr(C), N, ctypes.c_longlong(M * N), M, N, K, batch, ctypes.c_float(alpha), ptr(colscale),
                    ctypes.c_longlong(N if colscale is not None else 0), int(b_split), stream())


def attention_route(prec, f, C, h, w):
    if not (CA_GEMM and ops.precision_id(prec) == ops.F16 and (9 * C) % 32 == 0 and (h * w) % 32 == 0 and C % 4 == 0):
        return 'conv'
    return 'gram' if CA_GRAM and f.f16 and C == 64 and w in (32, 64) and f.ld % 8 == 0 and f.coff == 0 else 'gemm'


CA_TABLES = dict(conv=dict(forward='fd wp wpT raw rawT A f32 out32', backward='AT dOrawT dwp dout32 df32'),
                 gemm=dict(forward='fd wp wp_h raw_h rawT_h A_h O', backward='wpT_h dwp dOraw_h dOrawT_h AT_h df32'),
                 gram=dict(forward='fd_h fdT_h q raw_h rawT_h A_h O', backward='dOraw_h dOrawT_h AT_h df32'),
                 shared=dict(forward='S0 S1 norm rnorm mm argmax', per_sample='mm_b', backward='dA dS1 dS0 Gs coef'))


class AttentionPlan:

    def __init__(self, B, H, W, C, device, img_hw, scale=10.0, fuse=True):
        self.B, self.H, self.W, self.C, self.dims, self.device = B, H, W, C, (B, H, W, C), device
        self.h, self.w, self.L = h, w, L = H // 2, W // 2, (H // 2) * (W // 2)
        assert h == w and H % 2 == 0, "contextual attention expects a square, even-sized feature map"
        self.img_hw, self.scale, self.fuse = img_hw, scale, fuse
        self.fused_adjoint = fuse and h == 32 and w == 32
        self.unused = set() if fuse and not self.fused_adjoint else {'dS0'} if fuse else {'S1', 'dS0'}
        f32, f16 = torch.float32, torch.float16
        LL, fmap, vec, tab, tabT = (f32, (B, h, w, L)), (f32, (B, H, W, C)), (f32, (B, L)), (f16, (B, L, 16 * C)), (f16, (B, 16 * C, L))
        self.spec = dict(S0=LL, S1=LL, dS0=LL, A=LL, AT=LL, dA=LL, dS1=LL, Gs=LL, f32=fmap, out32=fmap, dout32=fmap, df32=fmap, norm=vec, rnorm=vec, q=vec, mm_b=vec, mm=(f32, (L,)),
                         argmax=(torch.int32, (B * L,)), coef=(f32, (33 * B, L)), fd=(f32, (B, h, w, C)), dwp=(f32, (B, h, w, 9 * C)), wp=(f32, (B, L, 9 * C)), wpT=(f32, (B, 9 * C, L)),
                         raw=(f32, (B, L, 16 * C)), rawT=(f32, (B, C, 16 * L)), dOrawT=(f32, (B, C, 16 * L)), wp_h=(f16, (B, L, 9 * C)), wpT_h=(f16, (B, 9 * C, L)), raw_h=tab, rawT_h=tabT,
                         O=tab, dOraw_h=tab, dOrawT_h=tabT, A_h=(f16, (B, L, L)), AT_h=(f16, (B, L, L)), fd_h=(f16, (B, L, C)), fdT_h=(f16, (B, C, L)))
        self.owned, self.sets, self.route, self.last = {}, {}, None, None
        self.buffers('shared', 'forward')

    gemm = property(lambda self: self.route in ('gemm', 'gram'))
    gram = property(lambda self: self.route == 'gram')
    nbytes = lambda self: sum(t.numel() * t.element_size() for t in self.owned.values())

    def buffers(self, route, stage, skip=()):
        r = self if route == 'shared' else self.sets.setdefault(route, types.SimpleNamespace())
        for n in CA_TABLES[route][stage].split():
            if (route, n) in self.owned or n in self.unused or n in skip:
                continue
            if torch.cuda.is_current_stream_capturing():
                raise RuntimeError('AttentionPlan%s: %s route, %s would allocate %s inside a stream capture -- run it eagerly once first' % (self.dims, route, stage, n))
            t = self.owned[route, n] = torch.zeros(*self.spec[n][1], dtype=self.spec[n][0], device=self.device)
            setattr(r, n, Act(t) if t.dim() == 4 else t)
        return r

    def forward(self, f, mask_img, out, prec, want_argmax=False, per_sample_mask=False):
        route, self.route, self.last = attention_route(prec, f, self.C, self.h, self.w), None, None
        L_, B, L, (patches, scores, paste) = _lib.get(), self.B, self.L, self.steps[route][:3]
        r = self.buffers(route, 'forward', skip=[n for n, a in (('f32', f), ('out32', out)) if not a.f16])
        mm, mm_stride = (self.buffers('shared', 'per_sample').mm_b, L) if per_sample_mask else (self.mm, 0)
        patches(self, r, f)
        mask = ('hv_ca_mask_batched', ptr(mask_img), B, ctypes.c_longlong(self.img_hw[0] * self.img_hw[1])) if per_sample_mask else ('hv_ca_mask', ptr(mask_img))
        L_.call(*mask, *self.img_hw, self.h, self.w, ptr(mm), stream())
        scores(self, r, prec)
        if self.fuse:
            L_.call('hv_ca_fuse', ptr(self.S0.t), ptr(self.S1.t), B, self.h, self.w, 0, stream())
        s = self.S1 if self.fuse else self.S0
        if route != 'conv':
            L_.call('hv_ca_softmax_f16', ptr(s.t), ptr(mm), ctypes.c_longlong(mm_stride), ptr(r.A_h), B, L, ctypes.c_float(self.scale), ptr(self.argmax) if want_argmax else None, stream())
        elif per_sample_mask:
            L_.call('hv_ca_softmax_batched', ptr(s.t), ptr(mm), ctypes.c_longlong(mm_stride), ptr(r.A.t), B, L, ctypes.c_float(self.scale), ptr(self.argmax) if want_argmax else None, stream())
        else:
            L_.call('hv_ca_softmax', ptr(s.t), ptr(mm), ptr(r.A.t), B, L, ctypes.c_float(self.scale), ptr(self.argmax) if want_argmax else None, stream())
        paste(self, r, out, prec)
        self.route, self.last = route, (ops.precision_id(prec), per_sample_mask)

    def backward(self, dout, df, accumulate, prec):
        if self.route is None or self.last != (ops.precision_id(prec), False):
            raise RuntimeError('AttentionPlan%s: backward(prec=%s) does not follow the last forward: route %s, (precision, per-sample mask) %s' % (self.dims, prec, self.route, self.last))
        L_, B, L, (paste_grad, score_grad) = _lib.get(), self.B, self.L, self.steps[self.route][3:]
        r = self.buffers(self.route, 'backward', skip=[n for n, a in (('dout32', dout), ('df32', df)) if not a.f16])
        self.buffers('shared', 'backward')
        df_user, df = df, r.df32 if df.f16 else df
        paste_grad(self, r, dout, df, accumulate and df is df_user, prec)
        name, A = ('hv_ca_softmax_backward', r.A.t) if self.route == 'conv' else ('hv_ca_softmax_backward_f16', r.A_h)
        L_.call(name, ptr(self.dA.t), ptr(A), ptr(self.mm), ptr(self.dS1.t), B, L, ctypes.c_float(self.scale), stream())
        if self.fused_adjoint:
            L_.call('hv_ca_fuse_backward_prep', ptr(self.dS1.t), ptr(self.S0.t), ptr(self.norm), ptr(self.rnorm), ptr(self.Gs.t), ptr(self.coef), B, self.h, self.w, stream())
        else:
            if self.fuse:
                L_.call('hv_ca_fuse', ptr(self.dS1.t), ptr(self.dS0.t), B, self.h, self.w, 1, stream())
            L_.call('hv_ca_score_backward_prep', ptr((self.dS0 if self.fuse else self.dS1).t), ptr(self.S0.t), ptr(self.norm), ptr(self.rnorm), ptr(self.Gs.t), ptr(self.coef), B, L, stream())
        score_grad(self, r, df, prec)
        if df is not df_user:
            ops.copy_channels(df, df_user, mode=0, accumulate=bool(accumulate))

    def _conv_patches(self, r, f):
        if f.f16:
            ops.copy_channels(f, r.f32, mode=0)
            f = r.f32
        _lib.get().call('hv_ca_patches', ptr(f.t), f.f16, *self.dims, f.ld, ptr(r.fd.t), ptr(r.wp), ptr(r.wpT), ptr(self.norm), ptr(self.rnorm), stream())
        _lib.get().call('hv_ca_raw_patches', ptr(f.t), *self.dims, f.ld, ptr(r.raw), ptr(r.rawT), stream())

    def _conv_scores(self, r, prec):
        ops.conv2d(r.fd, r.wp, self.S0, 3, 1, 1, 1, w_bstride=self.L * 9 * self.C, ch_scale=self.rnorm, ch_scale_bstride=self.L, precision=prec)

    def _conv_paste(self, r, out, prec):
        ops.conv2d(r.A, r.rawT, r.out32 if out.f16 else out, 4, 2, 1, 1, transposed=True, alpha=0.25, w_bstride=self.C * 16 * self.L, precision=prec)
        if out.f16:
            ops.copy_channels(r.out32, out, mode=0)

    def _conv_paste_grad(self, r, dout, df, accumulate, prec):
        if dout.f16:
            ops.copy_channels(dout, r.dout32, mode=0)
            dout = r.dout32
# ... 45 lines not shown
```

healthivert-gan_amd/models/networks.py:

```python
import functools

import torch
import torch.nn as nn
from torch.nn import init
from torch.optim import lr_scheduler

from ._backend import engine as E
from ._backend import lib as _lib
from ._backend import ops
Act, rup = ops.Act, ops.rup


class Identity(nn.Module):
    def forward(self, x):
        return x


def get_norm_layer(norm_type='instance'):
    if norm_type == 'batch':
        return functools.partial(nn.BatchNorm2d, affine=True, track_running_stats=True)
    if norm_type == 'instance':
        return functools.partial(nn.InstanceNorm2d, affine=False, track_running_stats=False)
    if norm_type == 'none':
        return lambda x: Identity()
    raise NotImplementedError('normalization layer [%s] is not found' % norm_type)


def get_scheduler(optimizer, opt):
    if opt.lr_policy == 'linear':
        def lambda_rule(epoch):
            return 1.0 - max(0, epoch + opt.epoch_count - opt.n_epochs) / float(opt.n_epochs_decay + 1)
        return lr_scheduler.LambdaLR(optimizer, lr_lambda=lambda_rule)
    if opt.lr_policy == 'step':
        return lr_scheduler.StepLR(optimizer, step_size=opt.lr_decay_iters, gamma=0.1)
    if opt.lr_policy == 'plateau':
        return lr_scheduler.ReduceLROnPlateau(optimizer, mode='min', factor=0.2, threshold=0.01, patience=5)
    if opt.lr_policy == 'cosine':
        return lr_scheduler.CosineAnnealingLR(optimizer, T_max=opt.n_epochs, eta_min=0)
    return NotImplementedError('learning rate policy [%s] is not implemented', opt.lr_policy)


def init_weights(net, init_type='normal', init_gain=0.02):
    def init_func(m):
        classname = m.__class__.__name__
        if hasattr(m, 'weight') and (classname.find('Conv') != -1 or classname.find('Linear') != -1):
            if init_type == 'normal':
                init.normal_(m.weight.data, 0.0, init_gain)
            elif init_type == 'xavier':
                init.xavier_normal_(m.weight.data, gain=init_gain)
            elif init_type == 'kaiming':
                init.kaiming_normal_(m.weight.data, a=0, mode='fan_in')
            elif init_type == 'orthogonal':
                init.orthogonal_(m.weight.data, gain=init_gain)
            else:
                raise NotImplementedError('initialization method [%s] is not implemented' % init_type)
            if hasattr(m, 'bias') and m.bias is not None:
                init.constant_(m.bias.data, 0.0)
        elif classname.find('BatchNorm2d') != -1:
            init.normal_(m.weight.data, 1.0, init_gain)
            init.constant_(m.bias.data, 0.0)

    print('initialize network with %s' % init_type)
    net.apply(init_func)


def init_net(net, init_type='normal', init_gain=0.02, gpu_ids=[]):
    init_weights(net, init_type, init_gain=init_gain)
    if len(gpu_ids) > 0:
        assert torch.cuda.is_available()
        net.to(gpu_ids[0])
    return net


def define_G(input_nc, output_nc, ngf, netG, norm='batch', use_dropout=False, init_type='normal', init_gain=0.02, gpu_ids=[]):
    if netG in ('resnet_9blocks', 'resnet_6blocks', 'unet_128', 'unet_256'):
        raise NotImplementedError("define_G('%s'): not on the HealthiVert-GAN hot path (Pix2PixModel builds inpaint_networks.Generator; "
                                  "UnetG_CT_mask.define_G is the U-Net variant provided)" % netG)
    raise NotImplementedError('Generator model name [%s] is not recognized' % netG)


def define_D(input_nc, ndf, netD, n_layers_D=3, norm='batch', init_type='normal', init_gain=0.02, gpu_ids=[]):
    norm_layer = get_norm_layer(norm_type=norm)
    if netD == 'basic':
        net = NLayerDiscriminator(input_nc, ndf, n_layers=3, norm_layer=norm_layer)
    elif netD == 'n_layers':
        net = NLayerDiscriminator(input_nc, ndf, n_layers_D, norm_layer=norm_layer)
    elif netD in ('pixel', 'seg'):
        raise NotImplementedError("define_D('%s'): not on the HealthiVert-GAN hot path" % netD)
    else:
        raise NotImplementedError('Discriminator model name [%s] is not recognized' % netD)
    return init_net(net, init_type, init_gain, gpu_ids)


class _GanLossFn(torch.autograd.Function):
    @staticmethod
    def forward(ctx, pred, target_is_real, mode):
        loss = torch.zeros((), device=pred.device)
        dz = torch.empty_like(pred)
        ops.gan_loss(pred.contiguous(), target_is_real, mode, loss=loss, dz=dz)
        ctx.save_for_backward(dz)
        return loss

    @staticmethod
    def backward(ctx, g):
        (dz,) = ctx.saved_tensors
        return dz * g, None, None


class GANLoss(nn.Module):
    def __init__(self, gan_mode, target_real_label=1.0, target_fake_label=0.0):
        super().__init__()
        self.register_buffer('real_label', torch.tensor(target_real_label))
        self.register_buffer('fake_label', torch.tensor(target_fake_label))
        self.gan_mode = gan_mode
        if gan_mode not in ('lsgan', 'vanilla', 'wgangp'):
            raise NotImplementedError('gan mode %s not implemented' % gan_mode)
        if target_real_label != 1.0 or target_fake_label != 0.0:
            raise NotImplementedError("GANLoss HIP path: labels 1.0 / 0.0")

    def get_target_tensor(self, prediction, target_is_real):
        return (self.real_label if target_is_real else self.fake_label).expand_as(prediction)

    def __call__(self, prediction, target_is_real):
        if self.gan_mode == 'wgangp':
            raise NotImplementedError("GANLoss('wgangp') is not on the HealthiVert-GAN hot path")
        _lib.require_gpu(prediction)
        return _GanLossFn.apply(prediction, bool(target_is_real), self.gan_mode)


CONV_BSTATS = True
HEAD_NORM = True


class _Stem:
    __slots__ = ('p', 'y', 'node')

    def __init__(self, p, y):
        self.p, self.y, self.node = p, y, None


class _Normed:
    __slots__ = ('p', 'node', 'z', 'y', 'stats', 'norm', 'bparts_used', 'head_fused', '_fstats', '_bsums', '_head_ok')

    def __init__(self, p, node, z, y, stats, norm):
        self.p, self.node, self.z, self.y, self.stats, self.norm = p, node, z, y, stats, norm
        self.bparts_used = 0
        self.head_fused = False
        self._fstats = None
        self._bsums = {}
        self._head_ok = {}

    def _partials(self, parts):
        return torch.zeros(max(1, parts) * self.p.cout * 2, dtype=torch.float32, device=self.z.t.device), parts

    def forward_stats(self, prec):
        if self._fstats is None:
            self._fstats = self._partials(int(self.node.stats_parts(prec)))
        return self._fstats if self._fstats[1] else (None, 0)

    def backward_sums(self, consumer, book, prec, mul_x, groups):
        if groups not in self._bsums:
            gx = consumer.dx_view(book, 'plain')
            call = consumer.dx_call(book, prec, 'plain', gx, book.accumulates(gx), mul_x=mul_x, bn=(self.z, self.stats, groups, None))
            self._bsums[groups] = self._partials(call.bstats_parts())
        return self._bsums[groups] if self._bsums[groups][1] else (None, 0)

    def head_call(self, head, prec, groups):
        nm = self.norm
        bn = isinstance(nm, nn.BatchNorm2d)
        xn = (self.stats, nm.weight if bn else None, nm.bias if bn else None, groups if bn else self.z.B, 'lrelu', self.y)
        call = head.node.forward_call(prec, xn=xn, x_raw=self.z)
        if groups not in self._head_ok:
            self._head_ok[groups] = call.supported()
        return call if self._head_ok[groups] else None


class _Logits:
    __slots__ = ('p', 'node', 'y', 'carrier')

    def __init__(self, p, node, y, carrier):
        self.p, self.node, self.y, self.carrier = p, node, y, carrier

    @property
    def loss_head_ready(self):
        g = self.carrier
        return g.f16 and g.t.shape[-1] == 4 and g.coff == 0


class _DiscPlan:
    def __init__(self, net, B, H, W, device):
        self.B, self.H, self.W = B, H, W
        dt = ops.storage_dtype(net.precision)
        z = lambda h, w, C: Act(torch.zeros(B, h, w, rup(C, 4), dtype=dt, device=device), C, 0)
        self.book = E.GradBook()
        self.x4 = z(H, W, 1)
        self.layers = []
        h, w = H, W
        prev = None
        for li, L in enumerate(net._spec):
            ho, wo = ops.conv_out_size(h, 4, L['stride'], 1, 1), ops.conv_out_size(w, 4, L['stride'], 1, 1)
            p = net._pset_convs[li]
            if li == 0:
                ent = _Stem(p, z(ho, wo, p.cout))
            elif L['last']:
                self.logits = torch.zeros(B, 1, ho, wo, dtype=torch.float32, device=device)
                y = Act(self.logits.view(B, ho, wo, 1))
                ent = _Logits(p, E.ConvNode(p, prev, y, L['stride'], 1, 1, 'none', use_bias=True), y, z(ho, wo, 1))
                self.book.twins[id(y.t)] = ent.carrier.t
            else:
                zraw = z(ho, wo, p.cout)
                ent = _Normed(p, E.ConvNode(p, prev, zraw, L['stride'], 1, 1, 'none', use_bias=L['bias']), zraw, z(ho, wo, p.cout),
                              torch.zeros(2 * B * p.cout, dtype=torch.float32, device=device), net.model[L['norm']])
            prev = ent.y
            h, w = ho, wo
            self.layers.append(ent)
        self.dx = torch.zeros(B, 1, H, W, dtype=torch.float32, device=device)
        self.pending = None
        self.x_in = None
        self.training, self.groups = False, 1

    def bind_input(self, x, training, groups):
        if self.x_in is not None:
            self.book.twins.pop(id(self.x_in.t), None)
        self.x_in = Act(x.view(self.B, self.H, self.W, 1))
        self.book.twins[id(self.x_in.t)] = self.dx.view(self.B, self.H, self.W, 1)
        stem = self.layers[0]
        stem.node = E.ConvNode(stem.p, self.x_in, stem.y, 2, 1, 1, 'lrelu', use_bias=True)
        self.training, self.groups = training, groups


def _stat_momentum(m, order):
    if order == 'swapped_first':
        return m / (1.0 - m * (1.0 - m))
    if order == 'swapped_second':
        return m * (1.0 - m)
    return m


class NLayerDiscriminator(nn.Module):

    def __init__(self, input_nc, ndf=64, n_layers=3, norm_layer=nn.BatchNorm2d):
        super().__init__()
        if type(norm_layer) == functools.partial:
            use_bias = norm_layer.func == nn.InstanceNorm2d
            norm_cls = norm_layer.func
        else:
            use_bias = norm_layer == nn.InstanceNorm2d
            norm_cls = norm_layer
        print(norm_layer)
        if input_nc != 1:
            raise NotImplementedError("NLayerDiscriminator HIP path: input_nc == 1")
        if norm_cls not in (nn.BatchNorm2d, nn.InstanceNorm2d):
            raise NotImplementedError("NLayerDiscriminator HIP path: norm in {batch, instance}")
        self.norm_kind = 'batch' if norm_cls == nn.BatchNorm2d else 'instance'
        kw, padw = 4, 1
        seq = [nn.Conv2d(input_nc, ndf, kernel_size=kw, stride=2, padding=padw), nn.LeakyReLU(0.2, True)]
        spec = [dict(conv=0, norm=None, stride=2, bias=True, last=False)]
        nf_mult = 1
        for n in range(1, n_layers):
            nf_prev, nf_mult = nf_mult, min(2 ** n, 8)
            spec.append(dict(conv=len(seq), norm=len(seq) + 1, stride=2, bias=use_bias, last=False))
            seq += [nn.Conv2d(ndf * nf_prev, ndf * nf_mult, kernel_size=kw, stride=2, padding=padw, bias=use_bias),
                    norm_layer(ndf * nf_mult), nn.LeakyReLU(0.2, True)]
        nf_prev, nf_mult = nf_mult, min(2 ** n_layers, 8)
        spec.append(dict(conv=len(seq), norm=len(seq) + 1, stride=1, bias=use_bias, last=False))
        seq += [nn.Conv2d(ndf * nf_prev, ndf * nf_mult, kernel_size=kw, stride=1, padding=padw, bias=use_bias),
                norm_layer(ndf * nf_mult), nn.LeakyReLU(0.2, True)]
        spec.append(dict(conv=len(seq), norm=None, stride=1, bias=True, last=True))
        seq += [nn.Conv2d(ndf * nf_mult, 1, kernel_size=kw, stride=1, padding=padw)]
        self.model = nn.Sequential(*seq)
        self._spec = spec
        self.precision = None
        self._pset = None
        self._pset_convs = None
        self._plans = {}

    def paramset(self):
        if self._pset is None:
            convs, extra = [], []
            for li, L in enumerate(self._spec):
                m = self.model[L['conv']]
                cin, cout = m.in_channels, m.out_channels
                if li == 0:
                    convs.append(E.ConvParams('model.%d' % L['conv'], m.weight, m.bias, cin, cout, 4, cin_fwd=1, cin_wg=4))
                else:
                    convs.append(E.ConvParams('model.%d' % L['conv'], m.weight, m.bias, cin, cout, 4))
                if L['norm'] is not None and self.norm_kind == 'batch':
                    nm = self.model[L['norm']]
                    extra += [nm.weight, nm.bias]
            self._pset_convs = convs
            self._pset = E.ParamSet(convs, extra)
        return self._pset

    def load_state_dict(self, *args, **kwargs):
        r = super().load_state_dict(*args, **kwargs)
        if self._pset is not None:
            self._pset.weights_changed()
        return r

    def _plan(self, B, H, W, device, slot=0):
        key = (B, H, W, str(device), slot, ops.precision_id(self.precision))
        if key not in self._plans:
            self.paramset()
            self._plans[key] = _DiscPlan(self, B, H, W, device)
        return self._plans[key]

    def _free_plan_slot(self, B, H, W, device):
        slot = 1
        while True:
            P = self._plans.get((B, H, W, str(device), slot, ops.precision_id(self.precision)))
            if P is None or P.pending is None or P.pending() is None:
                return slot
            slot += 1

    def run_forward(self, x, training=None, prep=True, groups=1, stat_order=None, slot=0):
        _lib.require_gpu(x)
        training = self.training if training is None else training
        prec = ops.precision_id(self.precision)
        x = x.contiguous().float()
        B, _, H, W = x.shape
        P = self._plan(B, H, W, x.device, slot)
        P.book.join()
        if prep:
            self.paramset().prep(x.device, power_iter=False, only_if_stale=(prep == 'if_stale'))
        P.bind_input(x, training, groups)
        bn = self.norm_kind == 'batch'
        head = P.layers[-1]
        P.layers[0].node.forward(prec)
        for ent in P.layers[1:-1]:
            nm = ent.norm
            fused = ent.head_call(head, prec, groups) if (HEAD_NORM and ent is P.layers[-2] and ent.z.f16) else None
            ent.head_fused = fused is not None
            partials, parts = ent.forward_stats(prec) if (bn and training) else (None, 0)
            ent.node.forward(prec, stats=partials)
            y_out = None if fused is not None else ent.y
            if bn:
                ops.norm_act_forward(ent.z, y_out, 'batch', training, ent.stats, nm.weight, nm.bias, nm.running_mean,
                                     nm.running_var, nm.num_batches_tracked, act='lrelu', eps=nm.eps, momentum=_stat_momentum(nm.momentum, stat_order),
                                     groups=groups, partials=partials, n_partials=parts)
            else:
                ops.norm_act_forward(ent.z, y_out, 'instance', training, ent.stats, act='lrelu', eps=nm.eps)
        (fused or head.node.forward_call(prec)).launch()
        return P

    def _loss_seed(self, P, ranges, mode, grad_weight, loss_weight=1.0, param_grads=True, accumulate=False, dz=None):
        head = P.layers[-1]
        if head.loss_head_ready:
            want_db = param_grads and head.p.bias is not None and head.node.use_bias
            args = [a for rows, real, loss in ranges for a in (P.logits[rows], real, loss, Act(head.carrier.t[rows], 4, 0))]
            ops.gan_loss_pair(*args, mode=mode, loss_weight=loss_weight, grad_weight=grad_weight, dbias=head.p.bias.grad if want_db else None,
                              dbias_accumulate=accumulate)
            return None, True
        if dz is None:
            dz = torch.empty_like(P.logits)
        for rows, real, loss in ranges:
            ops.gan_loss(P.logits[rows], real, mode, loss=loss, loss_weight=loss_weight, dz=dz[rows], grad_weight=grad_weight)
        return dz, False

    def loss_backward(self, P, target_is_real, mode, loss, grad_weight, need_dx=False, param_grads=True, accumulate=False, loss_weight=1.0, dz=None,
                      backward=True):
        dz, ready = self._loss_seed(P, [(slice(None), target_is_real, loss)], mode, grad_weight, loss_weight, param_grads, accumulate, dz)
        if not backward:
            return None
        return self.run_backward(P, dz, need_dx=need_dx, param_grads=param_grads, accumulate=accumulate, logits_ready=ready)

    def loss_backward_halves(self, P, mode, loss_fake, loss_real, grad_weight, dz=None):
        B = P.B // 2
        dz, ready = self._loss_seed(P, [(slice(0, B), False, loss_fake), (slice(B, None), True, loss_real)], mode, grad_weight, dz=dz)
        return self.run_backward(P, dz, need_dx=False, param_grads=True, accumulate=False, logits_ready=ready)

    def run_backward(self, P, dlogits, need_dx=False, param_grads=True, accumulate=False, logits_ready=False):
        prec = ops.precision_id(self.precision)
        book = P.book
        book.reset()
        B = P.B
        stem, head = P.layers[0], P.layers[-1]
        if not logits_ready:
            ops.copy_channels(Act(dlogits.contiguous().view(B, head.y.H, head.y.W, 1)), head.carrier, mode=0)
        bn = self.norm_kind == 'batch'
        fuse0 = stem.node.act != 'none' and not P.layers[1].node.shift
        sums = (None, 0)
        for li in range(len(P.layers) - 1, 0, -1):
            ent, below = P.layers[li], P.layers[li - 1]
            node = ent.node
            prev_normed = li >= 2 and not node.shift
            if ent is not head:
                nm = ent.norm
                ent.bparts_used = sums[1]
                ops.norm_act_backward(book.twin(ent.y), ent.y, ent.z, book.twin(ent.z), self.norm_kind, P.training, ent.stats,
                                      gamma=nm.weight if bn else None, act='none', dgamma=nm.weight.grad if (bn and param_grads) else None,
                                      dbeta=nm.bias.grad if (bn and param_grads) else None, param_accumulate=accumulate,
                                      groups=P.groups, partials=sums[0], n_partials=sums[1])
            mul_x = stem.node.act if (li == 1 and fuse0) else ('lrelu' if prev_normed else None)
            sums = (None, 0)
            if prev_normed and mul_x and CONV_BSTATS and bn and P.training:
                sums = below.backward_sums(node, book, prec, mul_x, P.groups)
            E.conv_backward(node, book, prec, dbias_accumulate=accumulate, wgrad_accumulate=accumulate, wgrad=param_grads, dbias_done=bool(logits_ready and ent is head),
                            mul_x=mul_x, bn=(below.z, below.stats, P.groups, sums[0]) if sums[1] else None)
        if param_grads:
            ops.copy_channels(P.x_in, P.x4, mode=0)
        stem.node.need_dx = need_dx
        E.conv_backward(stem.node, book, prec, dbias_accumulate=accumulate, wgrad_accumulate=accumulate, wgrad=param_grads,
                        x_wg=P.x4 if param_grads else None, premultiplied=fuse0)
        return book.twin(P.x_in).t.view(B, 1, P.H, P.W) if need_dx else None

    def finish(self):
        for P in self._plans.values():
            P.book.join()
        self.paramset().finish_backward(accumulate=False)
        self.paramset().attach_grads()

    def forward(self, input):
        if torch.is_grad_enabled() and (input.requires_grad or any(p.requires_grad for p in self.parameters())):
            B, _, H, W = input.shape
            P = self.run_forward(input, slot=self._free_plan_slot(B, H, W, input.device))
            anchor = next((p for p in self.parameters() if p.requires_grad), None)
            return _DiscFn.apply(input, anchor, self, P, P.logits)
        return self.run_forward(input).logits.clone()


class _PlanToken:
    """Alive as long as the autograd node that owns a plan's activations is."""


def grads_are_fresh(net):
    ps = list(net.parameters())
    fresh = getattr(ps[0], '_hv_fresh', False) or ps[0].grad is None
    for p in ps:
        p._hv_fresh = False
    return fresh


class _DiscFn(torch.autograd.Function):
    @staticmethod
    def forward(ctx, x, anchor, net, plan, logits):
        import weakref
        ctx.net, ctx.plan, ctx.need_dx = net, plan, x.requires_grad
        ctx.token = _PlanToken()
        plan.pending = weakref.ref(ctx.token)
        return logits.clone()

    @staticmethod
    def backward(ctx, g):
        net, plan = ctx.net, ctx.plan
        if plan.pending is None or plan.pending() is not ctx.token:
            raise RuntimeError("NLayerDiscriminator: the activations of this forward pass were overwritten before its backward ran")
        pg = any(p.requires_grad for p in net.parameters())
        acc = pg and not grads_are_fresh(net)
        S = ops.grad_scale(net.precision)
        pset = net.paramset()
        if acc:
            ops.scale_inplace(pset.flat_grad, S / pset.grad_factor)
        if pg:
            pset.attach_grads()
        dx = net.run_backward(plan, g.contiguous() * S if S != 1.0 else g.contiguous(), need_dx=ctx.need_dx, param_grads=pg, accumulate=acc)
        if pg:
            net.finish()
            ops.scale_inplace(pset.flat_grad, 1.0 / S)
        plan.pending = None
        if dx is not None:
            dx = dx.clone()
            ops.scale_inplace(dx, 1.0 / S)
        return dx, None, None, None, None
```

healthivert-gan_amd/ops.py:

```python
import ctypes
import os

import torch

from . import lib as _lib
from .lib import ACT, NORM, F16, F32, ptr, stream

_PRECISION = {'fp32': F32, 'f32': F32, 'fp16': F16, 'f16': F16}


_TIMER = None


def timer():
    return _TIMER


def set_timer(t):
    global _TIMER
    _TIMER = t


def default_precision():
    return _PRECISION[os.environ.get('HV_PRECISION', 'fp32').lower()]


def precision_id(p):
    if p is None:
        return default_precision()
    if isinstance(p, str):
        return _PRECISION[p.lower()]
    return int(p)


def rup(v, m):
    return (v + m - 1) // m * m


def cpad(C):
    return rup(C, 8) if C > 16 else rup(C, 4)


def grad_scale(precision):
    s = float(os.environ.get('HV_GRAD_SCALE', '8192' if precision_id(precision) == F16 else '1'))
    if s <= 0 or (s != 1 and not s.is_integer()) or int(s) & (int(s) - 1):
        raise ValueError('HV_GRAD_SCALE must be a power of two')
    return s


def scale_inplace(t, factor):
    if factor != 1.0 and t is not None and t.numel():
        _lib.get().call('hv_affine', ptr(t), ptr(t), ctypes.c_longlong(t.numel()), ctypes.c_float(factor), ctypes.c_float(0.0), stream())


def storage_dtype(precision):
    return torch.float16 if precision_id(precision) == F16 else torch.float32


class Act:
    __slots__ = ('t', 'B', 'H', 'W', 'C', 'ld', 'coff', 'f16')

    def __init__(self, t, C=None, coff=0):
        assert t.dim() == 4 and t.dtype in (torch.float32, torch.float16) and t.is_contiguous(), (t.shape, t.dtype)
        _lib.require_gpu(t)
        self.t = t
        self.f16 = int(t.dtype == torch.float16)
        self.B, self.H, self.W, self.ld = t.shape
        self.coff = coff
        self.C = self.ld - coff if C is None else C
        assert 0 < self.C and self.coff + self.C <= self.ld

    @staticmethod
    def empty(B, H, W, C, device, ld=None, zero=False, dtype=torch.float32):
        ld = C if ld is None else ld
        t = (torch.zeros if zero else torch.empty)(B, H, W, ld, dtype=dtype, device=device)
        return Act(t, C, 0)

    def slice(self, coff, C):
        return Act(self.t, C, self.coff + coff)

    def like(self, zero=False):
        return Act.empty(self.B, self.H, self.W, self.ld, self.t.device, zero=zero, dtype=self.t.dtype).slice(self.coff, self.C) \
            if (self.coff or self.C != self.ld) else Act.empty(self.B, self.H, self.W, self.C, self.t.device, zero=zero, dtype=self.t.dtype)

    @property
    def npix(self):
        return self.B * self.H * self.W

    def nchw(self):
        if self.C == 1 and self.ld == 1 and not self.f16:
            return self.t.view(self.B, 1, self.H, self.W)
        out = torch.empty(self.B, self.C, self.H, self.W, dtype=torch.float32, device=self.t.device)
        L = _lib.get()
        L.call('hv_nhwc_to_nchw', ptr(self.t), self.f16, ptr(out), self.B, self.C, self.H, self.W, self.ld, self.coff, 0, stream())
        return out


def from_nchw(x, CP=None, dtype=torch.float32):
    _lib.require_gpu(x)
    x = x.contiguous().float()
    B, C, H, W = x.shape
    if C == 1 and CP in (None, 1) and dtype == torch.float32:
        return Act(x.view(B, H, W, 1))
    ld = C if CP is None else CP
    a = Act.empty(B, H, W, C, x.device, ld=ld, zero=ld != C, dtype=dtype)
    _lib.get().call('hv_nchw_to_nhwc', ptr(x), ptr(a.t), a.f16, B, C, H, W, ld, 0, stream())
    return a


class _Workspace:
    def __init__(self):
        self.buf = {}
        self.retired = []

    def get(self, nbytes, device, slot=0):
        key = (device, slot)
        b = self.buf.get(key)
        if b is None or b.numel() < nbytes:
            if b is not None:
                self.retired.append(b)
            b = torch.empty(max(int(nbytes), 1 << 20), dtype=torch.uint8, device=device)
            self.buf[key] = b
        return b


WS = _Workspace()


def _ws(nbytes, device, slot=0):
    b = WS.get(nbytes + 64, device, (slot, torch.cuda.current_stream(device).cuda_stream))
    return b, ctypes.c_size_t(b.numel())


def conv_out_size(n, k, stride, pad, dil):
    return (n + 2 * pad - dil * (k - 1) - 1) // stride + 1


_PROBES = {}


class ConvCall:
    __slots__ = ('d', 'x', 'y', 'wuse')

    def __init__(self, x, w, y, k, stride=1, pad=0, dil=1, bias=None, act='none', transposed=False, in_shift=0, alpha=1.0, accumulate=0, ch_scale=None,
                 w_bstride=0, ch_scale_bstride=0, precision=None, cin=None, cout=None, w_h=None, mul=None, w_t=None, pool2=False, x1=None, wuse=None, bn=None,
                 xn=None):
        L = _lib.get()
        self.d = d = L.hv_conv_desc()
        self.x, self.y, self.wuse = x, y, wuse
        kh, kw = (k, k) if isinstance(k, int) else k
        d.x = ptr(x.t).value
        d.B, d.H, d.W = x.B, x.H << in_shift, x.W << in_shift
        d.in_shift, d.x_ld, d.x_coff, d.Cin = in_shift, x.ld, x.coff, (x.C if cin is None else cin)
        d.w = ptr(w).value
        d.w_bstride = w_bstride
        d.Cout, d.KH, d.KW, d.stride, d.pad, d.dil, d.transposed = (y.C if cout is None else cout), kh, kw, stride, pad, dil, int(transposed)
        d.bias = None if bias is None else ptr(bias).value
        d.ch_scale = None if ch_scale is None else ptr(ch_scale).value
        d.ch_scale_bstride = ch_scale_bstride
        d.alpha, d.act, d.accumulate = alpha, ACT[act], int(accumulate)
        d.y = ptr(y.t).value
        d.Ho, d.Wo, d.y_ld, d.y_coff = (y.H << 1 if pool2 else y.H), (y.W << 1 if pool2 else y.W), y.ld, y.coff
        d.pool2 = int(bool(pool2))
        if x1 is not None:
            xa, wfull, ch, w1_row, w1_tap = x1
            assert xa.C == 1 and xa.H == d.H and xa.W == d.W
            d.x1, d.x1_f16, d.x1_ld, d.x1_coff = ptr(xa.t).value, xa.f16, xa.ld, xa.coff
            d.w1, d.w1_row, d.w1_tap = ptr(wfull).value + 4 * ch, w1_row, w1_tap
        d.precision = precision_id(precision)
        d.w_f16 = None if w_h is None else ptr(w_h).value
        d.w_f16_tiled = None if (w_t is None or w_h is None) else ptr(w_t).value
        d.x_f16, d.y_f16 = x.f16, y.f16
        if mul is not None:
            m, mact = mul
            d.mul_src, d.mul_ld, d.mul_coff, d.mul_act, d.mul_f16 = ptr(m.t).value, m.ld, m.coff, ACT[mact], m.f16
        if bn is not None:
            bx, bstat, bgroups, bpart = bn
            assert bx.f16 == y.f16 and bx.H == y.H and bx.W == y.W and bx.B == y.B
            d.bn_x, d.bn_x_ld, d.bn_x_coff = ptr(bx.t).value, bx.ld, bx.coff
            d.bn_stats, d.bn_groups = ptr(bstat).value, int(bgroups)
            if bpart is not None:
                d.bstats = ptr(bpart).value
        if xn is not None:
            nstat, ngam, nbet, ngroups, nact, nout = xn
            d.xn_stats, d.xn_groups, d.xn_act = ptr(nstat).value, int(ngroups), ACT[nact]
            if ngam is not None:
                d.xn_gamma, d.xn_beta = ptr(ngam).value, ptr(nbet).value
            if nout is not None:
                assert nout.f16 and nout.B == x.B and nout.H == x.H and nout.W == x.W
                d.xn_out, d.xn_out_ld, d.xn_out_coff = ptr(nout.t).value, nout.ld, nout.coff
        if d.Cout == 1:
            need = L.size('hv_conv2d_workspace_bytes', ctypes.byref(d))
            if need:
                b, _ = _ws(need, x.t.device, slot=1)
                d.workspace, d.workspace_bytes = ptr(b).value, b.numel()

    def _probe(self, fn):
        key = (fn, bytes(self.d))
        if key not in _PROBES:
            _PROBES[key] = _lib.get().size(fn, ctypes.byref(self.d))
        return _PROBES[key]

    def supported(self):
        return bool(self._probe('hv_conv2d_supported'))

    def stats_parts(self):
        return self._probe('hv_conv2d_stats_parts')

    def bstats_parts(self):
        return self._probe('hv_conv2d_bstats_parts')

    def launch(self, stats=None):
        L, d, x, y = _lib.get(), self.d, self.x, self.y
        if stats is not None:
            d.stats = ptr(stats).value
        if _TIMER is not None:
            taps = d.KH * d.KW if not d.transposed else max(1, (d.KH * d.KW) // (d.stride * d.stride))
            flops = 2.0 * y.B * y.H * y.W * d.Cout * taps * d.Cin
            wbytes = (2 if (d.w_f16 and d.precision == F16 and not d.w_bstride) else 4) * d.Cout * d.KH * d.KW * d.Cin * (x.B if d.w_bstride else 1)
            xb, yb = (2 if x.f16 else 4), (2 if y.f16 else 4)
            nbytes = xb * x.B * x.H * x.W * d.Cin + yb * y.B * y.H * y.W * d.Cout * (2 if d.accumulate else 1) + wbytes + \
                ((2 if d.mul_f16 else 4) * y.B * y.H * y.W * d.Cout if d.mul_src else 0)
            _TIMER.wrap(('conv', x.B, d.H, d.W, d.Cin, d.Cout, d.KH, d.stride, d.dil, d.transposed), flops,
                        lambda: L.call('hv_conv2d', ctypes.byref(d), stream()), nbytes)
        else:
            L.call('hv_conv2d', ctypes.byref(d), stream())
        if self.wuse is not None:
            setattr(self.wuse[0], self.wuse[1], getattr(*self.wuse) | int(L.cdll.hv_last_weight_tables()))
        return y


def conv2d(*args, stats=None, **kw):
    return ConvCall(*args, **kw).launch(stats)


def conv2d_supported(*args, **kw):
    return ConvCall(*args, **kw).supported()


def conv2d_stats_parts(*args, **kw):
    return ConvCall(*args, **kw).stats_parts()


def conv2d_bstats_parts(*args, **kw):
    return ConvCall(*args, **kw).bstats_parts()


def pool2_ok(g, y_low, k, stride, pad, dil, precision, w_h, w_t, cout=None, w=None):
    if w_h is None or w_t is None or precision_id(precision) != F16 or g.H != 2 * y_low.H or g.W != 2 * y_low.W:
        return False
    return conv2d_supported(g, w_h if w is None else w, Act(y_low.t, y_low.C if cout is None else cout, y_low.coff), k, stride, pad, dil, transposed=True,
                            pool2=True, precision=precision, w_h=w_h, w_t=w_t)


class FoldChain:
    __slots__ = ('pending', 'slot', 'stream')

    def __init__(self, stream_handle):
        self.pending, self.slot, self.stream = None, 0, stream_handle

    def flush(self):
        if self.pending is not None:
            assert torch.cuda.current_stream().cuda_stream == self.stream, 'FoldChain.flush() on another stream than its weight gradients'
            f, self.pending = self.pending, None
            _lib.get().call('hv_wgrad_fold_now', ctypes.byref(f), stream())


FOLD_CHAIN = True


def conv2d_wgrad(x, g, dw, k, stride=1, pad=0, dil=1, in_shift=0, accumulate=False, precision=None, cin=None, cout=None, dbias=None,
                 dbias_accumulate=False, chain=None):
    L = _lib.get()
    d = L.hv_wgrad_desc()
    kh, kw = (k, k) if isinstance(k, int) else k
    d.x = ptr(x.t).value
    d.B, d.H, d.W, d.in_shift = x.B, x.H << in_shift, x.W << in_shift, in_shift
    d.x_ld, d.x_coff, d.Cin = x.ld, x.coff, (x.C if cin is None else cin)
    d.g = ptr(g.t).value
    d.Ho, d.Wo, d.g_ld, d.g_coff, d.Cout = g.H, g.W, g.ld, g.coff, (g.C if cout is None else cout)
    d.KH, d.KW, d.stride, d.pad, d.dil = kh, kw, stride, pad, dil
    d.dw = ptr(dw).value
    d.accumulate = int(accumulate)
    d.precision = precision_id(precision)
    d.dbias = None if dbias is None else ptr(dbias).value
    d.dbias_accumulate = int(dbias_accumulate)
    d.x_f16, d.g_f16 = x.f16, g.f16
    d.workspace, d.workspace_bytes = None, 0
    if chain is not None and not FOLD_CHAIN:
        chain = None
    need = L.size('hv_conv2d_wgrad_workspace_bytes', ctypes.byref(d))
    fold = None
    if chain is not None:
        assert torch.cuda.current_stream(x.t.device).cuda_stream == chain.stream, 'a FoldChain belongs to one stream'
        if chain.pending is not None:
            d.carry = ctypes.pointer(chain.pending)
        if need:
            b, _ = _ws(need, x.t.device, slot=('fold-chain', chain.slot))
            chain.slot ^= 1
            d.workspace, d.workspace_bytes = ptr(b).value, b.numel()
            fold = L.hv_wgrad_fold()
            d.pending = ctypes.pointer(fold)
    elif need:
        b, _ = _ws(need, x.t.device)
        d.workspace, d.workspace_bytes = ptr(b).value, b.numel()
    if _TIMER is not None:
        flops = 2.0 * g.B * g.H * g.W * d.Cout * kh * kw * d.Cin
        nbytes = (2 if x.f16 else 4) * x.B * x.H * x.W * d.Cin + (2 if g.f16 else 4) * g.B * g.H * g.W * d.Cout + 4 * d.Cout * kh * kw * d.Cin
        _TIMER.wrap(('wgrad', x.B, d.H, d.W, d.Cin, d.Cout, kh, stride, dil, 0), flops,
                    lambda: L.call('hv_conv2d_wgrad', ctypes.byref(d), stream()), nbytes)
    else:
        L.call('hv_conv2d_wgrad', ctypes.byref(d), stream())
    if chain is not None:
        chain.pending = fold if (fold is not None and fold.nslabs > 0) else None
    return dw


class LayerTable:

    def __init__(self, struct_name):
        self.struct_name = struct_name
        self.key = None
        self.dev = None
        self.n = 0

    def update(self, rows, key, device):
        if key == self.key:
            return
        L = _lib.get()
        S = getattr(L, self.struct_name)
        arr = (S * len(rows))()
        for i, r in enumerate(rows):
            for f, v in r.items():
                if torch.is_tensor(v):
                    v = ptr(v).value
                setattr(arr[i], f, v)
        raw = bytes(arr)
        host = torch.frombuffer(bytearray(raw), dtype=torch.uint8)
        self.dev = host.to(device)
        self.key, self.n = key, len(rows)

    def ptr(self):
        return ptr(self.dev)


def tiled_elems(rows, taps, K):
    return _lib.get().size('hv_weight_tiled_elems', int(rows), int(taps), int(K))


def tile_weights(w_h, rows, taps, K):
    n = tiled_elems(rows, taps, K)
    if not n:
        return None
    out = torch.empty(n, dtype=torch.float16, device=w_h.device)
    _lib.get().call('hv_weight_tile_f16', ptr(w_h), ptr(out), int(rows), int(taps), int(K), stream())
    return out


def weight_prep(table, max_numel, any_sn=True, any_legacy=True):
    _lib.get().call('hv_weight_prep2', ctypes.cast(table.ptr(), ctypes.POINTER(_lib.get().hv_wprep_layer)), table.n,
                    ctypes.c_longlong(max_numel), int(any_sn), int(any_legacy), stream())


def weight_prep_backward(table, max_numel, any_sn):
    _lib.get().call('hv_weight_prep_backward', ctypes.cast(table.ptr(), ctypes.POINTER(_lib.get().hv_wprep_bwd_layer)), table.n,
                    ctypes.c_longlong(max_numel), int(any_sn), stream())




def act_backward(dy, y, act, dbias=None, dbias_accumulate=False):
    L = _lib.get()
    need = L.size('hv_act_backward_workspace_bytes', ctypes.c_longlong(dy.npix), dy.C) if dbias is not None else 0
    b, nb = _ws(need, dy.t.device)
    L.call('hv_act_backward', ptr(dy.t), dy.f16, ptr(y.t), y.f16, ctypes.c_longlong(dy.npix), dy.C, dy.ld, dy.coff, y.ld, y.coff, ACT[act],
           ptr(dbias), int(dbias_accumulate), ptr(b), nb, stream())


def head_seed_backward(seed, y, carrier, act, dbias=None, dbias_accumulate=False):
    L = _lib.get()
    npix = carrier.npix
    need = L.size('hv_head_seed_workspace_bytes', ctypes.c_longlong(npix)) if dbias is not None else 0
    b, nb = _ws(need, carrier.t.device)
    L.call('hv_head_seed_backward', ptr(seed), ptr(y.t), y.f16, y.ld, y.coff, ptr(carrier.t), ctypes.c_longlong(npix), ACT[act], ptr(dbias),
           int(dbias_accumulate), ptr(b), nb, stream())


def copy_channels(src, dst, mode=0, accumulate=False):
    assert src.C == dst.C
    _lib.get().call('hv_copy_channels', ptr(src.t), src.f16, ptr(dst.t), dst.f16, dst.B, dst.H, dst.W, dst.C, src.ld, src.coff, dst.ld, dst.coff,
                    mode, int(accumulate), stream())


def add_channels(a, b, dst):
    assert a.C == b.C == dst.C and a.npix == b.npix == dst.npix
    _lib.get().call('hv_add_channels', ptr(a.t), a.f16, a.ld, a.coff, ptr(b.t), b.f16, b.ld, b.coff, ptr(dst.t), dst.f16, dst.ld, dst.coff,
                    ctypes.c_longlong(dst.npix), dst.C, stream())


def fill(t, value=0.0):
    _lib.get().call('hv_fill', ptr(t), ctypes.c_longlong(t.numel()), ctypes.c_float(value), stream())


def axpy(y, x, a=1.0):
    assert y.numel() == x.numel()
    _lib.get().call('hv_axpy', ptr(y), ptr(x), ctypes.c_longlong(y.numel()), ctypes.c_float(a), stream())


def gen_input(x, seg, mask, ratio, dst, order):
    _lib.get().call('hv_gen_input', ptr(x), ptr(seg), ptr(mask), ptr(ratio), ptr(dst.t), dst.f16, dst.B, dst.H, dst.W, dst.ld, order, stream())


def gap_fc_sigmoid(x, fc_w, fc_b, pooled, pred):
    L = _lib.get()
    need = L.size('hv_gap_fc_workspace_bytes', x.B, x.C)
    b, nb = _ws(need, x.t.device)
    L.call('hv_gap_fc_sigmoid', ptr(x.t), x.f16, x.B, x.H * x.W, x.C, x.ld, ptr(fc_w), ptr(fc_b), ptr(pooled), ptr(pred), ptr(b), nb, stream())

# ... 112 lines not shown
```

include/hvgan.h:

```cpp
#ifndef HVGAN_H
#define HVGAN_H
#include <stddef.h>
#include <stdint.h>

#ifdef __cplusplus
extern "C" {
#endif

#define HV_OK 0
#define HV_ERR_ARG (-1)
#define HV_ERR_UNSUPPORTED (-2)
#define HV_ERR_WORKSPACE (-3)

enum { HV_F32 = 0, HV_F16 = 1 };
enum { HV_ACT_NONE = 0, HV_ACT_ELU = 1, HV_ACT_RELU = 2, HV_ACT_LRELU = 3, HV_ACT_SIGMOID = 4, HV_ACT_CLAMP = 5 };
enum { HV_NORM_NONE = 0, HV_NORM_BATCH = 1, HV_NORM_INSTANCE = 2 };

int hv_version(void);
const char* hv_arch(void);
int hv_last_kernel_path(void);
const char* hv_last_kernel_name(void);
int hv_set_kernel_timing(void* ev_start, void* ev_stop);
int hv_set_s2t_mode(int mode);

typedef struct {
    const float* x; int B, H, W;
    int in_shift; int x_ld, x_coff, Cin;
    const float* w; long long w_bstride;
    int Cout, KH, KW, stride, pad, dil, transposed;
    const float* bias;
    const float* ch_scale;
    long long ch_scale_bstride;
    float alpha; int act; int accumulate;
    float* y; int Ho, Wo, y_ld, y_coff;
    int precision;
    const void* w_f16;
    const void* w_f16_tiled;
    const float* mul_src; int mul_ld, mul_coff, mul_act;
    int x_f16, y_f16, mul_f16;
    void* workspace; size_t workspace_bytes;
    float* stats;
    const void* x1;
    int x1_f16, x1_ld, x1_coff;
    const float* w1; int w1_row, w1_tap;
    int pool2;
    const void* bn_x; int bn_x_ld, bn_x_coff;
    const float* bn_stats; int bn_groups;
    float* bstats;
    const float* xn_stats; const float* xn_gamma; const float* xn_beta; int xn_groups, xn_act;
    void* xn_out; int xn_out_ld, xn_out_coff;
} hv_conv_desc;
int hv_conv2d(const hv_conv_desc* d, void* stream);
size_t hv_conv2d_bstats_parts(const hv_conv_desc* d);
size_t hv_conv2d_workspace_bytes(const hv_conv_desc* d);
size_t hv_conv2d_stats_parts(const hv_conv_desc* d);
int hv_last_weight_tables(void);
int hv_conv2d_supported(const hv_conv_desc* d);

typedef struct {
    const float* slabs; float* dw; long long numel; int nslabs; int accumulate;
    const float* bias_slabs; float* dbias; int Cout; int dbias_accumulate;
} hv_wgrad_fold;

typedef struct {
    const float* x; int B, H, W; int in_shift; int x_ld, x_coff, Cin;
    const float* g; int Ho, Wo, g_ld, g_coff, Cout;
    int KH, KW, stride, pad, dil;
    float* dw; int accumulate;
    float* workspace; size_t workspace_bytes;
    int precision;
    int x_f16, g_f16;
    float* dbias; int dbias_accumulate;
    hv_wgrad_fold* pending;
    const hv_wgrad_fold* carry;
} hv_wgrad_desc;
int hv_wgrad_fold_now(const hv_wgrad_fold* fold , void* stream);
size_t hv_conv2d_wgrad_workspace_bytes(const hv_wgrad_desc* d);
int hv_conv2d_wgrad(const hv_wgrad_desc* d, void* stream);

typedef struct {
    const float* w_orig;
    float* u; float* v;
    float* sigma;
    float* w_fwd;
    float* w_bwd;
    void* w_fwd_h; void* w_bwd_h;
    void* w_fwd_t; void* w_bwd_t;
    int Cout, Cin, taps, CinP, CoutF, CoutP, CinB;
    int sn, power_iter, transposed_src;
    void* w_fwd_t2; int K2;
} hv_wprep_layer;
int hv_weight_prep(const hv_wprep_layer* d_layers, int n_layers, long long max_numel, void* stream);
int hv_weight_prep2(const hv_wprep_layer* d_layers, int n_layers, long long max_numel, int any_sn, int any_legacy, void* stream);

size_t hv_weight_tiled_elems(int rows, int taps, int K);
int hv_weight_tile_f16(const void* w_f16, void* w_tiled, int rows, int taps, int K, void* stream);

typedef struct {
    const float* dw_ohwi; const float* w_fwd; const float* u; const float* v; const float* sigma;
    float* dw_orig; int Cout, Cin, taps, CinP, sn, transposed_src, accumulate;
} hv_wprep_bwd_layer;
int hv_weight_prep_backward(const hv_wprep_bwd_layer* d_layers, int n_layers, long long max_numel, int any_sn, void* stream);

size_t hv_head_seed_workspace_bytes(long long npix);
int hv_head_seed_backward(const float* seed, const void* y, int y_f16, int y_ld, int y_coff, void* carrier_f16, long long npix, int act, float* dbias,
                          int dbias_accumulate, float* workspace, size_t workspace_bytes, void* stream);

int hv_act_backward(void* dy, int dy_f16, const void* y, int y_f16 , long long npix, int C, int dy_ld, int dy_coff,
                    int y_ld, int y_coff, int act, float* dbias, int dbias_accumulate, float* workspace, size_t workspace_bytes, void* stream);
size_t hv_act_backward_workspace_bytes(long long npix, int C);

typedef struct {
    const void* x; void* y; int B, HW, C; int x_ld, x_coff, y_ld, y_coff;
    int norm; int training; float eps, momentum;
    const float* gamma; const float* beta; float* running_mean; float* running_var; long long* num_batches_tracked;
    float* stats; int act; int post_sigmoid;
    float* workspace; size_t workspace_bytes;
    int groups;
    int f16;
    const float* partials; int n_partials;
} hv_norm_desc;
size_t hv_norm_workspace_bytes(int B, int HW, int C);
int hv_norm_act_forward(const hv_norm_desc* d, void* stream);
typedef struct {
    const void* dy; const void* y; const void* x; void* dx; int B, HW, C;
    int dy_ld, dy_coff, y_ld, y_coff, x_ld, x_coff, dx_ld, dx_coff;
    int norm; int training; const float* gamma; const float* stats;
    int act; int post_sigmoid;
    float* dgamma; float* dbeta; int param_accumulate;
    float* workspace; size_t workspace_bytes;
    int groups;
    int f16;
    const float* partials; int n_partials;
} hv_norm_bwd_desc;
int hv_norm_act_backward(const hv_norm_bwd_desc* d, void* stream);

int hv_nchw_to_nhwc(const float* src, void* dst, int dst_f16, int B, int C, int H, int W, int dst_ld, int dst_coff, void* stream);
int hv_nhwc_to_nchw(const void* src, int src_f16, float* dst, int B, int C, int H, int W, int src_ld, int src_coff, int accumulate, void* stream);
int hv_copy_channels(const void* src, int src_f16, void* dst, int dst_f16, int B, int H, int W, int C, int src_ld, int src_coff, int dst_ld,
                     int dst_coff, int mode, int accumulate, void* stream);
int hv_add_channels(const void* a, int a_f16, int a_ld, int a_coff, const void* b, int b_f16, int b_ld, int b_coff, void* dst, int dst_f16, int dst_ld,
                    int dst_coff, long long npix, int C, void* stream);

int hv_gen_input(const float* x, const float* seg, const float* mask, const double* slice_ratio, void* dst, int dst_f16,
                 int B, int H, int W, int CP, int order, void* stream);
size_t hv_gap_fc_workspace_bytes(int B, int C);
int hv_gap_fc_sigmoid(const void* x, int x_f16, int B, int HW, int C, int x_ld, const float* fc_w, const float* fc_b,
                      float* pooled , float* pred , float* workspace, size_t workspace_bytes, void* stream);
int hv_gap_fc_sigmoid_backward(const float* dpred, const float* pred, const float* pooled, const float* fc_w,
                               void* dx, int dx_f16, int B, int HW, int C, int dx_ld, float* dw, float* db, int accumulate,
                               const void* mul_src, int mul_f16, int mul_ld, int mul_act, void* stream);

int hv_ca_patches(const void* f, int f_f16 , int B, int H, int W, int C, int f_ld, float* fd, float* wp, float* wpT, float* norm,
                  float* rnorm, void* stream);
int hv_ca_raw_patches(const float* f, int B, int H, int W, int C, int f_ld, float* raw, float* rawT, void* stream);
int hv_ca_mask(const float* mask, int Himg, int Wimg, int h, int w, float* mm, void* stream);
int hv_ca_mask_batched(const float* mask, int B, long long mask_bstride, int Himg, int Wimg, int h, int w, float* mm, void* stream);
int hv_ca_fuse(const float* S, float* out, int B, int h, int w, int adjoint, void* stream);
int hv_ca_softmax(const float* S, const float* mm, float* A, int B, int L, float scale, int* argmax, void* stream);
int hv_ca_softmax_batched(const float* S, const float* mm, long long mm_bstride, float* A, int B, int L, float scale, int* argmax,
                          void* stream);
int hv_ca_flow(const int* argmax, int B, int h, int w, int up, float* flow, void* stream);
int hv_ca_softmax_backward(const float* dA, const float* A, const float* mm, float* dS, int B, int L, float scale, void* stream);
int hv_transpose_batched(const float* src, float* dst, int B, int R, int C, void* stream);
int hv_bgemm_nt(const void* A, int a_f16, int lda, long long strideA, const void* B, int b_f16, int ldb, long long strideB, float* C, int ldc,
                long long strideC, int M, int N, int K, int batch, float alpha, const float* colscale, long long strideS, int b_split, void* stream);
int hv_ca_fold(const float* src, void* dst, int dst_f16 , int B, int H, int W, int C, int dst_ld, float alpha, int accumulate, void* stream);
int hv_bgemm_nt_h(const void* A, int a_f16, int lda, long long strideA, const void* B, int b_f16, int ldb, long long strideB, void* C_h, int ldc,
                  long long strideC, int M, int N, int K, int batch, float alpha, const float* colscale, long long strideS, int b_split, void* stream);
int hv_ca_fold_h(const void* src_h, void* dst, int dst_f16, int B, int H, int W, int C, int dst_ld, float alpha, int accumulate, void* stream);
int hv_ca_raw_patches_f16(const void* f, int f_f16 , int B, int H, int W, int C, int f_ld, void* raw_h, void* rawT_h, void* stream);
int hv_transpose_batched_f16(const float* src, void* dst_h, int B, int R, int C, void* stream);
int hv_ca_patches_h(const void* f, int f_f16, int B, int H, int W, int C, int f_ld, float* fd, float* wp, void* wp_h, float* norm, float* rnorm,
                    void* stream);
int hv_ca_softmax_f16(const float* S, const float* mm, long long mm_bstride , void* A_h, int B, int L, float scale,
                      int* argmax, void* stream);
int hv_ca_softmax_backward_f16(const float* dA, const void* A_h, const float* mm, float* dS, int B, int L, float scale, void* stream);
int hv_transpose_batched_h2h(const void* src_h, void* dst_h, int B, int R, int C, void* stream);
int hv_ca_score_backward_prep(const float* dS, const float* S0, const float* norm, const float* rnorm, float* Gs, float* coef,
                              int B, int L, void* stream);
int hv_ca_fuse_backward_prep(const float* dS1, const float* S0, const float* norm, const float* rnorm, float* Gs, float* coef, int B, int h, int w,
                             void* stream);
int hv_ca_patches_backward(const float* dwp, const float* wp, const float* coef, float* df, int B, int H, int W, int C,
                           int df_ld, int accumulate, void* stream);

int hv_ca_gram_down(const void* f, int f_f16, int B, int H, int W, int C, int f_ld, void* fd_h, void* fdT_h, float* q, void* stream);
int hv_ca_gram_scores(const void* fd_h, const float* q, int B, int h, int w, int C, float* S0, float* norm, float* rnorm, void* stream);
int hv_ca_gram_backward(const float* Gs, const void* fd_h, const void* fdT_h, const float* coef, int B, int h, int w, int C, float* df, int df_ld,
                        void* stream);

int hv_sobel(const float* img, float* out, int B, int H, int W, void* stream);
typedef struct {
    const float* real_B; const float* mask; const float* x_stage1; const float* x_stage2;
    const float* fine_seg; const float* coarse_seg; const float* pred1; const float* pred2;
    const long long* height; const long long* x1; const long long* x2; const long long* maxheight;
    float* fake_B; float* fake_B_coarse; float* fake_B_local; float* real_B_local;
    float* fine_bin; float* coarse_bin; float* pred1_h; float* pred2_h; int* rows;
    int B, H, W, half_band;
} hv_postg_desc;
int hv_post_generator(const hv_postg_desc* d, void* stream);
int hv_shrm_composite(const float* gen, const float* real, const float* pred_scaled, const long long* height,
                      const long long* x1, const long long* x2, float* out, int* rows, int B, int H, int W, void* stream);

int hv_gan_loss(const float* z, long long n, int target_is_real, int mode, float loss_weight, float* loss, int loss_accumulate,
                float grad_weight, float* dz, void* stream);
// ... 113 lines not shown
```

Before: 2501 slices/s.

## Fuse PatchGAN stem weight gradient into layer-1 transposed dgrad epilogue

Adds a weight-gradient path to the G4 transposed-conv (dgrad) epilogue. The kernel loads the matching window of the single-channel image, forms the stem conv's weight and bias gradient partials with MFMA from the just-computed data gradient held in LDS, and writes per-block partials that are folded afterwards. The discriminator backward uses this for the stem when it qualifies, and skips the input padding copy, the separate stem wgrad kernel, and the store of the layer-1 data gradient when no input gradient is needed. The cost is extra register pressure, LDS use and epilogue work in that dgrad kernel, plus a partials workspace and a fold step.

```diff
diff --git a/healthivert-gan_amd/csrc/conv_g4.hip b/healthivert-gan_amd/csrc/conv_g4.hip
--- a/healthivert-gan_amd/csrc/conv_g4.hip
+++ b/healthivert-gan_amd/csrc/conv_g4.hip
@@ -8,6 +8,8 @@
     float* stats;
     const void* bn_x; const float* bn_stats; float* bstats;
     int bn_x_ld, bn_x_coff, bn_ipg;
+    const void* wg_x; float* wg_parts;
+    int wg_x_ld, wg_x_coff, wg_x_f16; unsigned wg_x_bytes;
     int B, H, W, x_ld, x_coff, Cin;
     int Ho, Wo, y_ld, y_coff, Cout;
     int mul_ld, mul_coff, mul_act, act, accumulate;
@@ -32,9 +34,34 @@
         bias_r[n] = __builtin_bit_cast(f32x4, __builtin_amdgcn_raw_buffer_load_b128(bsrc, (unsigned)(cob + n * 16 + (lane >> 4) * 4) * 4u, 0, 0));
 }
 
-template <int MODE, int MT>
+typedef __fp16 hv_fp16x4 __attribute__((__vector_size__(4 * sizeof(__fp16))));
+__device__ __forceinline__ f16x4 g4_tr_read(const _Float16* lds_addr) {
+    typedef hv_fp16x4 __attribute__((address_space(3)))* lp;
+    return __builtin_bit_cast(f16x4, __builtin_amdgcn_ds_read_tr16_b64_v4f16((lp)(lds_addr)));
+}
+
+template <int MT>
+struct G4Win { static constexpr int ROWS = 16 * MT + 2, COLS = 66, LD = 68, N = (ROWS * COLS + 511) / 512; };
+template <int MT>
+__device__ __forceinline__ void g4_load_window(const G4K& p, int n_img, int i0, int j0, int tid, unsigned (&wgx)[G4Win<MT>::N]) {
+    typedef G4Win<MT> WN;
+    const __amdgpu_buffer_rsrc_t isrc = __builtin_amdgcn_make_buffer_rsrc(const_cast<void*>(p.wg_x), 0, p.wg_x_bytes, 0x00020000);
+    const int Hi = 2 * p.Ho, Wi = 2 * p.Wo;
+#pragma unroll
+    for (int k = 0; k < WN::N; ++k) {
+        const int e = tid + k * 512;
+        const int r = e / WN::COLS, u = e - r * WN::COLS;
+        const int row = 4 * i0 - 1 + r, col = 4 * j0 - 1 + u;
+        const bool ok = e < WN::ROWS * WN::COLS && (unsigned)row < (unsigned)Hi && (unsigned)col < (unsigned)Wi;
+        const unsigned idx = (unsigned)(((n_img * Hi + row) * Wi + col) * p.wg_x_ld + p.wg_x_coff);
+        if (p.wg_x_f16) wgx[k] = __builtin_amdgcn_raw_buffer_load_b16(isrc, ok ? idx * 2u : HV_OOB, 0, 0);
+        else wgx[k] = __builtin_amdgcn_raw_buffer_load_b32(isrc, ok ? idx * 4u : HV_OOB, 0, 0);
+    }
+}
+
+template <int MODE, int MT, int WGN>
 __device__ __forceinline__ void g4_epilogue(const G4K& p, f32x4 (&acc)[4][MT], char* smem, const int (&cls_s)[2], const int (&cob_s)[2], int n_img, int i0,
-                                            int j0, const f32x4 (&bias_r)[4]) {
+                                            int j0, const f32x4 (&bias_r)[4], const unsigned (&wgx)[WGN]) {
     constexpr int TW = 16, TH = 4 * MT, NTHR = 512, LDO = 128 + 8;
     const int tid = threadIdx.x, lane = tid & 63, wave = __builtin_amdgcn_readfirstlane(tid >> 6);
     const int wm = wave >> 1, wn = wave & 1;
@@ -146,9 +173,75 @@
             o[k] = __builtin_bit_cast(u32x4, v8);
         }
     }
-#pragma unroll
-    for (int k = 0; k < OITEMS; ++k)
-        if (ooff[k] >= 0) *reinterpret_cast<u32x4*>(yb + ooff[k]) = o[k];
+    if (yb) {
+#pragma unroll
+        for (int k = 0; k < OITEMS; ++k)
+            if (ooff[k] >= 0) *reinterpret_cast<u32x4*>(yb + ooff[k]) = o[k];
+    }
+    if constexpr (MODE == 1) {
+        if (p.wg_parts) {
+            typedef G4Win<MT> WN;
+            static_assert(WGN == WN::N, "window registers");
+            _Float16* Ws = ot + TH * TW * LDO;
+            float* Rs = reinterpret_cast<float*>(Ws + WN::ROWS * WN::LD);
+            float* Rb = Rs + 8 * 64 * 16;
+#pragma unroll
+            for (int k = 0; k < OITEMS; ++k) {
+                const int it = tid + k * NTHR;
+                *reinterpret_cast<u32x4*>(ot + (it >> 4) * LDO + (it & 15) * 8) = ooff[k] >= 0 ? o[k] : (u32x4){0u, 0u, 0u, 0u};
+            }
+#pragma unroll
+            for (int k = 0; k < WN::N; ++k) {
+                const int e = tid + k * NTHR;
+                const int r = e / WN::COLS, u = e - r * WN::COLS;
+                const _Float16 v = p.wg_x_f16 ? __builtin_bit_cast(_Float16, (unsigned short)wgx[k]) : (_Float16)__builtin_bit_cast(float, wgx[k]);
+                if (e < WN::ROWS * WN::COLS) Ws[r * WN::LD + u] = v;
+            }
+            __syncthreads();
+            const int grp = lane >> 4, sub = lane & 15, qr = sub >> 2, pc = sub & 3;
+            const int py = cls_s[wn] >> 1, px = cls_s[wn] & 1;
+            f32x4 dacc[4], bacc[4];
+#pragma unroll
+            for (int n = 0; n < 4; ++n) dacc[n] = bacc[n] = (f32x4){0.f, 0.f, 0.f, 0.f};
+            const f16x8 ones = {(_Float16)1.f, (_Float16)1.f, (_Float16)1.f, (_Float16)1.f, (_Float16)1.f, (_Float16)1.f, (_Float16)1.f, (_Float16)1.f};
+#pragma unroll
+            for (int h = 0; h < MT / 2; ++h) {
+                const int ty = wm * MT + 2 * h;
+                const _Float16* wr = Ws + (4 * ty + 2 * py + qr) * WN::LD + 16 * grp + 2 * px + pc;
+                f16x8 b;
+#pragma unroll
+                for (int e = 0; e < 4; ++e) { b[e] = wr[4 * e]; b[4 + e] = wr[4 * WN::LD + 4 * e]; }
+#pragma unroll
+                for (int n = 0; n < 4; ++n) {
+                    const _Float16* ap = ot + (ty * TW + 4 * grp + qr) * LDO + wn * 64 + n * 16 + pc * 4;
+                    const f16x4 lo = g4_tr_read(ap), hi = g4_tr_read(ap + TW * LDO);
+                    const f16x8 a = {lo[0], lo[1], lo[2], lo[3], hi[0], hi[1], hi[2], hi[3]};
+                    dacc[n] = __builtin_amdgcn_mfma_f32_16x16x32_f16(a, b, dacc[n], 0, 0, 0);
+                    bacc[n] = __builtin_amdgcn_mfma_f32_16x16x32_f16(a, ones, bacc[n], 0, 0, 0);
+                }
+            }
+#pragma unroll
+            for (int n = 0; n < 4; ++n)
+#pragma unroll
+                for (int r = 0; r < 4; ++r) {
+                    const int ch = n * 16 + 4 * grp + r;
+                    Rs[(wave * 64 + ch) * 16 + sub] = dacc[n][r];
+                    if (sub == 0) Rb[wave * 64 + ch] = bacc[n][r];
+                }
+            __syncthreads();
+            const long long nparts = (long long)gridDim.x * gridDim.y, part = (long long)blockIdx.y * gridDim.x + blockIdx.x;
+            auto fold8 = [](const float* q, int st) __attribute__((always_inline)) {
+                const float s0 = (q[0] + q[2 * st]) + (q[4 * st] + q[6 * st]), s1 = (q[st] + q[3 * st]) + (q[5 * st] + q[7 * st]);
+                return s0 + s1;
+            };
+#pragma unroll
+            for (int k = 0; k < 2; ++k) {
+                const int e = tid + k * NTHR;
+                *reinterpret_cast<f32x4*>(p.wg_parts + (part * 1024 + e) * 4) = (f32x4){fold8(Rs + e, 1024), 0.f, 0.f, 0.f};
+            }
+            if (tid < 64) p.wg_parts[nparts * 4096 + part * 64 + tid] = fold8(Rb + tid, 64);
+        }
+    }
     if (p.bstats) {
         const int pc = tid & 15, s = pc >> 3;
         const int ch0 = cob_s[s] + (pc & 7) * 8;
@@ -243,6 +336,12 @@
     const __amdgpu_buffer_rsrc_t xsrc = __builtin_amdgcn_make_buffer_rsrc(const_cast<void*>(p.x), 0, p.x_bytes, 0x00020000);
     f32x4 bias_r[4];
     g4_load_bias(p, cob_s[wn], lane, bias_r);
+    unsigned wgx[MODE == 1 ? G4Win<MT>::N : 1];
+#pragma unroll
+    for (int k = 0; k < (MODE == 1 ? G4Win<MT>::N : 1); ++k) wgx[k] = 0u;
+    if constexpr (MODE == 1) {
+        if (p.wg_parts) g4_load_window<MT>(p, n_img, i0, j0, tid, wgx);
+    }
 
     int pbase[BPW], pval[BPW];
     const int xbase = (n_img * p.H * p.W * p.x_ld + p.x_coff) * 2;
@@ -372,7 +471,7 @@
     __syncthreads();
     G4_STAMP(3);
 
-    g4_epilogue<MODE, MT>(p, acc, smem, cls_s, cob_s, n_img, i0, j0, bias_r);
+    g4_epilogue<MODE, MT>(p, acc, smem, cls_s, cob_s, n_img, i0, j0, bias_r, wgx);
 #ifdef G4_STAMPS
     __builtin_amdgcn_s_waitcnt(0);
     G4_STAMP(5);
@@ -523,7 +622,8 @@
 #ifdef G4_STAMPS
     st[2] = __builtin_amdgcn_s_memrealtime();
 #endif
-    g4_epilogue<0, MT>(p, acc, smem, cls_s, cob_s, n_img, i0, j0, bias_r);
+    const unsigned no_window[1] = {0u};
+    g4_epilogue<0, MT>(p, acc, smem, cls_s, cob_s, n_img, i0, j0, bias_r, no_window);
 #ifdef G4_STAMPS
     st[3] = __builtin_amdgcn_s_memrealtime();
     __builtin_amdgcn_s_waitcnt(0);
@@ -567,6 +667,7 @@
     constexpr size_t lds_loop = (size_t)(3 * 32 * 512 + (3 * ((PH * PW + 15) / 16) + 1) * 512) * 2, lds_out = (size_t)TH * 16 * 136 * 2, lds_red = 32 * 16 * 16 * 4;
     constexpr size_t lds = lds_loop > lds_out ? (lds_loop > lds_red ? lds_loop : lds_red) : (lds_out > lds_red ? lds_out : lds_red);
     static_assert(lds <= 160 * 1024, "LDS");
+    static_assert(lds_out + (size_t)G4Win<MT>::ROWS * G4Win<MT>::LD * 2 + 8 * 64 * 17 * 4 <= lds, "LDS of the weight-gradient epilogue");
     k.tiles_x = hv_cdiv(k.Wc, 16);
     k.tiles = k.tiles_x * hv_cdiv(k.Hc, TH);
     auto kern = conv_g4_kernel<MODE, MT>;
@@ -589,6 +690,7 @@
 }
 
 size_t hv_conv2d_g4_bstats_parts(const hv_conv_desc* d);
+size_t hv_conv2d_g4_wg_parts(const hv_conv_desc* d);
 static bool g4_eligible(const hv_conv_desc* d) {
     if (d->KH != 4 || d->KW != 4 || (d->stride != 2 && d->stride != 1) || d->pad != 1 || d->dil != 1 || d->in_shift || d->w_bstride || d->ch_scale) return false;
     if (d->precision != HV_F16 || !d->w_f16_tiled || !d->x_f16 || !d->y_f16 || d->accumulate > 1) return false;
@@ -621,6 +723,12 @@
         k.bn_x = d->bn_x; k.bn_stats = d->bn_stats; k.bstats = d->bstats; k.bn_x_ld = d->bn_x_ld; k.bn_x_coff = d->bn_x_coff;
         k.bn_ipg = d->B / (d->bn_groups > 0 ? d->bn_groups : 1);
     }
+    k.wg_x = nullptr; k.wg_parts = nullptr; k.wg_x_ld = k.wg_x_coff = k.wg_x_f16 = 0; k.wg_x_bytes = 0;
+    if (d->wg_parts) {
+        if (!hv_conv2d_g4_wg_parts(d)) return HV_ERR_UNSUPPORTED;
+        k.wg_x = d->wg_x; k.wg_parts = d->wg_parts; k.wg_x_ld = d->wg_x_ld; k.wg_x_coff = d->wg_x_coff; k.wg_x_f16 = d->wg_x_f16 ? 1 : 0;
+        k.wg_x_bytes = (unsigned)((size_t)d->B * 4 * d->Ho * d->Wo * d->wg_x_ld * (d->wg_x_f16 ? 2 : 4));
+    } else if (!d->y) return HV_ERR_ARG;
     k.B = d->B; k.H = d->H; k.W = d->W; k.x_ld = d->x_ld; k.x_coff = d->x_coff; k.Cin = d->Cin;
     k.Ho = d->Ho; k.Wo = d->Wo; k.y_ld = d->y_ld; k.y_coff = d->y_coff; k.Cout = d->Cout;
     k.mul_ld = d->mul_ld; k.mul_coff = d->mul_coff; k.mul_act = d->mul_act; k.act = d->act; k.accumulate = d->accumulate; k.alpha = d->alpha;
@@ -658,6 +766,16 @@
     return (size_t)d->B * hv_cdiv(d->H, th) * hv_cdiv(d->W, 16) * 4;
 }
 
+size_t hv_conv2d_g4_wg_parts(const hv_conv_desc* d) {
+    if (!d->transposed || d->stride != 2 || d->Cout != 64 || d->bstats || !g4_eligible(d)) return 0;
+    if (!d->wg_x || d->wg_x_ld < 1 || d->wg_x_coff < 0 || d->wg_x_coff >= d->wg_x_ld || ((uintptr_t)d->wg_x & (d->wg_x_f16 ? 1 : 3))) return 0;
+    if (!d->y && d->accumulate) return 0;
+    if ((long long)d->B * 4 * d->Ho * d->Wo * d->wg_x_ld >= (1ll << 29)) return 0;
+    const int ny = 2 * (d->Cout / 64);
+    const int th = g4_tile_rows(d->B, d->H, d->W, ny);
+    return (size_t)d->B * hv_cdiv(d->H, th) * hv_cdiv(d->W, 16) * ny;
+}
+
 size_t hv_conv2d_g4_stats_floats(const hv_conv_desc* d, int* nparts) {
     hv_conv_desc t = *d;
     if (t.transposed || t.accumulate || !g4_eligible(&t)) return 0;
diff --git a/healthivert-gan_amd/csrc/conv_igemm.hip b/healthivert-gan_amd/csrc/conv_igemm.hip
--- a/healthivert-gan_amd/csrc/conv_igemm.hip
+++ b/healthivert-gan_amd/csrc/conv_igemm.hip
@@ -24,6 +24,7 @@
 int hv_conv2d_logits_dgrad(const hv_conv_desc* d, hipStream_t s);
 size_t hv_conv2d_g4_stats_floats(const hv_conv_desc* d, int* nparts);
 size_t hv_conv2d_g4_bstats_parts(const hv_conv_desc* d);
+size_t hv_conv2d_g4_wg_parts(const hv_conv_desc* d);
 size_t hv_conv2d_logits_bstats_parts(const hv_conv_desc* d);
 size_t hv_wgrad_halo_workspace_bytes(const hv_wgrad_desc* d);
 int hv_wgrad_halo(const hv_wgrad_desc* d, int* nslabs, hipStream_t s);
@@ -356,9 +357,16 @@
     return hv_conv2d_g4_bstats_parts(d);
 }
 
+extern "C" size_t hv_conv2d_wg_parts(const hv_conv_desc* d) {
+    if (!d || !d->x || !d->w || !d->transposed || d->precision != HV_F16 || !d->w_f16 || !d->w_f16_tiled || d->KH != 4 || d->KW != 4) return 0;
+    if (d->B <= 0 || d->H <= 0 || d->W <= 0 || d->Cin <= 0 || d->Ho <= 0 || d->Wo <= 0 || d->y_ld < d->y_coff + d->Cout || d->x_ld < d->x_coff + d->Cin) return 0;
+    if (d->stats || d->xn_stats || d->x1 || d->pool2) return 0;
+    return hv_conv2d_g4_wg_parts(d);
+}
+
 static int conv2d_dispatch(const hv_conv_desc* d, void* stream) {
     hv_wtable_used = 0;
-    if (!d || !d->x || !d->w || !d->y) return HV_ERR_ARG;
+    if (!d || !d->x || !d->w || (!d->y && !d->wg_parts)) return HV_ERR_ARG;
     if (d->B <= 0 || d->H <= 0 || d->W <= 0 || d->Cin <= 0 || d->Cout <= 0 || d->KH <= 0 || d->KW <= 0 ||
         d->stride <= 0 || d->dil <= 0 || d->pad < 0 || d->Ho <= 0 || d->Wo <= 0)
         return HV_ERR_ARG;
@@ -375,6 +383,10 @@
 
     if (d->stats && !hv_conv2d_g4_stats_floats(d, nullptr)) return HV_ERR_UNSUPPORTED;
     if (d->bstats && !hv_conv2d_bstats_parts(d)) return HV_ERR_UNSUPPORTED;
+    if (d->wg_parts) {
+        if (!hv_conv2d_wg_parts(d)) return HV_ERR_UNSUPPORTED;
+        return hv_conv2d_g4(d, (hipStream_t)stream);
+    }
     if (d->xn_stats) {
         if (d->Cout != 1 || !d->workspace) return HV_ERR_UNSUPPORTED;
         return hv_conv2d_head(d, (hipStream_t)stream);
@@ -503,6 +515,7 @@
 extern "C" int hv_conv2d_supported(const hv_conv_desc* d) {
     if (!d) return 0;
     if (d->bstats && !hv_conv2d_bstats_parts(d)) return 0;
+    if (d->wg_parts) return hv_conv2d_wg_parts(d) ? 1 : 0;
     if (!d->x1 && !d->pool2 && !d->xn_stats) return d->stats ? (hv_conv2d_g4_stats_floats(d, nullptr) ? 1 : 0) : 1;
     hv_probe_only = 1;
     const int rc = conv2d_dispatch(d, nullptr);
diff --git a/healthivert-gan_amd/csrc/prep.hip b/healthivert-gan_amd/csrc/prep.hip
--- a/healthivert-gan_amd/csrc/prep.hip
+++ b/healthivert-gan_amd/csrc/prep.hip
@@ -727,5 +727,5 @@
     return HV_OK;
 }
 
-extern "C" int hv_version(void) { return 104; }
+extern "C" int hv_version(void) { return 105; }
 extern "C" const char* hv_arch(void) { return "gfx950"; }
diff --git a/healthivert-gan_amd/engine.py b/healthivert-gan_amd/engine.py
--- a/healthivert-gan_amd/engine.py
+++ b/healthivert-gan_amd/engine.py
@@ -232,7 +232,7 @@
         C = a.C if form == 'pool_to' else self.p.cin_fwd
         return Act(g.t, C if form == 'src' else self.dx_c or C, g.coff)
 
-    def dx_call(self, book, prec, form, dst, accumulate, mul_x=None, bn=None):
+    def dx_call(self, book, prec, form, dst, accumulate, mul_x=None, bn=None, wg=None):
         p = self.p
         gy = book.twin(self.y)
         mul = None
@@ -241,7 +241,7 @@
         elif form in ('pool', 'plain') and mul_x:
             mul = (Act(self.x.t, p.cin_fwd, self.x.coff), mul_x)
         return ops.ConvCall(Act(gy.t, p.coutP, gy.coff), p.w_bwd, dst, self.k, self.s, self.pad, self.d, transposed=form != 'src', pool2=form in ('pool', 'pool_to'),
-                            accumulate=int(accumulate), precision=prec, w_h=p.w_bwd_h, w_t=p.w_bwd_t, mul=mul, bn=bn, wuse=(p, 'use_bwd'))
+                            accumulate=int(accumulate), precision=prec, w_h=p.w_bwd_h, w_t=p.w_bwd_t, mul=mul, bn=bn, wuse=(p, 'use_bwd'), wg=wg)
 
     def full_scratch(self):
         if self.full is None:
@@ -370,7 +370,7 @@
 
 
 def conv_backward(node, book, prec, dbias_accumulate=False, wgrad_accumulate=False, wgrad=True, x_wg=None, premultiplied=False,
-                  mul_x=None, dbias_done=False, bn=None):
+                  mul_x=None, dbias_done=False, bn=None, below_wg=None):
     p = node.p
     assert bn is None or (node.need_dx and not node.transposed and node.pool_to is None and not node.shift), 'conv_backward: bn= needs the plain data-gradient branch'
     gy = book.twin(node.y)
@@ -403,6 +403,13 @@
         node.dx_call(book, prec, 'full', full, False).launch()
         gx = node.dx_view(book, 'plain')
         ops.copy_channels(full, gx, mode=3, accumulate=book.mark(gx))
+    elif below_wg is not None:
+        assert form == 'plain' and mul_x and wgrad, 'conv_backward: below_wg= needs the plain data-gradient branch of a backward that makes parameter gradients'
+        pb, ximg, store = below_wg
+        dst = node.dx_view(book, form)
+        call = node.dx_call(book, prec, form, dst, book.mark(dst), mul_x=mul_x, bn=bn, wg=ximg)
+        ops.conv2d_dgrad_wgrad(call, pb.dw, pb.bias.grad, accumulate=wgrad_accumulate, dbias_accumulate=dbias_accumulate,
+                               chain=pb.owner.fold_chain() if pb.owner is not None else None, store=store)
     else:
         dst = node.dx_view(book, form)
         node.dx_call(book, prec, form, dst, book.mark(dst), mul_x=mul_x, bn=bn).launch()
diff --git a/healthivert-gan_amd/models/networks.py b/healthivert-gan_amd/models/networks.py
--- a/healthivert-gan_amd/models/networks.py
+++ b/healthivert-gan_amd/models/networks.py
@@ -133,10 +133,29 @@
 
 
 class _Stem:
-    __slots__ = ('p', 'y', 'node')
+    __slots__ = ('p', 'y', 'node', '_x4', '_wg_fused')
 
     def __init__(self, p, y):
         self.p, self.y, self.node = p, y, None
+        self._x4 = None
+        self._wg_fused = {}
+
+    def wgrad_fused(self, consumer, book, prec):
+        x = self.node.x
+        key = (x.f16, x.ld, x.coff)
+        if key not in self._wg_fused:
+            ok = bool(self.y.f16 and self.p.bias is not None and self.node.use_bias and self.p.cin_wg == 4 and self.p.cout == self.p.coutP)
+            if ok:
+                gx = consumer.dx_view(book, 'plain')
+                ok = consumer.dx_call(book, prec, 'plain', gx, False, mul_x=self.node.act, wg=x).wg_parts() > 0
+            self._wg_fused[key] = ok
+        return self._wg_fused[key]
+
+    def padded_input(self):
+        if self._x4 is None:
+            x = self.node.x
+            self._x4 = Act(torch.zeros(x.B, x.H, x.W, 4, dtype=self.y.t.dtype, device=self.y.t.device), 1, 0)
+        return self._x4
 
 
 class _Normed:
@@ -193,7 +212,6 @@
         dt = ops.storage_dtype(net.precision)
         z = lambda h, w, C: Act(torch.zeros(B, h, w, rup(C, 4), dtype=dt, device=device), C, 0)
         self.book = E.GradBook()
-        self.x4 = z(H, W, 1)
         self.layers = []
         h, w = H, W
         prev = None
@@ -369,7 +387,7 @@
         dz, ready = self._loss_seed(P, [(slice(0, B), False, loss_fake), (slice(B, None), True, loss_real)], mode, grad_weight, dz=dz)
         return self.run_backward(P, dz, need_dx=False, param_grads=True, accumulate=False, logits_ready=ready)
 
-    def run_backward(self, P, dlogits, need_dx=False, param_grads=True, accumulate=False, logits_ready=False):
+    def run_backward(self, P, dlogits, need_dx=False, param_grads=True, accumulate=False, logits_ready=False, fused_stem_wgrad=True):
         prec = ops.precision_id(self.precision)
         book = P.book
         book.reset()
@@ -379,6 +397,7 @@
             ops.copy_channels(Act(dlogits.contiguous().view(B, head.y.H, head.y.W, 1)), head.carrier, mode=0)
         bn = self.norm_kind == 'batch'
         fuse0 = stem.node.act != 'none' and not P.layers[1].node.shift
+        stem_fused = False
         sums = (None, 0)
         for li in range(len(P.layers) - 1, 0, -1):
             ent, below = P.layers[li], P.layers[li - 1]
@@ -395,13 +414,20 @@
             sums = (None, 0)
             if prev_normed and mul_x and CONV_BSTATS and bn and P.training:
                 sums = below.backward_sums(node, book, prec, mul_x, P.groups)
+            if li == 1:
+                stem_fused = bool(fused_stem_wgrad and param_grads and fuse0 and stem.wgrad_fused(node, book, prec))
             E.conv_backward(node, book, prec, dbias_accumulate=accumulate, wgrad_accumulate=accumulate, wgrad=param_grads, dbias_done=bool(logits_ready and ent is head),
-                            mul_x=mul_x, bn=(below.z, below.stats, P.groups, sums[0]) if sums[1] else None)
-        if param_grads:
-            ops.copy_channels(P.x_in, P.x4, mode=0)
+                            mul_x=mul_x, bn=(below.z, below.stats, P.groups, sums[0]) if sums[1] else None,
+                            below_wg=(stem.p, P.x_in, need_dx) if (li == 1 and stem_fused) else None)
         stem.node.need_dx = need_dx
-        E.conv_backward(stem.node, book, prec, dbias_accumulate=accumulate, wgrad_accumulate=accumulate, wgrad=param_grads,
-                        x_wg=P.x4 if param_grads else None, premultiplied=fuse0)
+        if stem_fused:
+            if need_dx:
+                E.conv_backward(stem.node, book, prec, wgrad=False, premultiplied=fuse0)
+        else:
+            if param_grads:
+                ops.copy_channels(P.x_in, stem.padded_input(), mode=0)
+            E.conv_backward(stem.node, book, prec, dbias_accumulate=accumulate, wgrad_accumulate=accumulate, wgrad=param_grads,
+                            x_wg=stem.padded_input() if param_grads else None, premultiplied=fuse0)
         return book.twin(P.x_in).t.view(B, 1, P.H, P.W) if need_dx else None
 
     def finish(self):
diff --git a/healthivert-gan_amd/ops.py b/healthivert-gan_amd/ops.py
--- a/healthivert-gan_amd/ops.py
+++ b/healthivert-gan_amd/ops.py
@@ -144,7 +144,7 @@
 
     def __init__(self, x, w, y, k, stride=1, pad=0, dil=1, bias=None, act='none', transposed=False, in_shift=0, alpha=1.0, accumulate=0, ch_scale=None,
                  w_bstride=0, ch_scale_bstride=0, precision=None, cin=None, cout=None, w_h=None, mul=None, w_t=None, pool2=False, x1=None, wuse=None, bn=None,
-                 xn=None):
+                 xn=None, wg=None):
         L = _lib.get()
         self.d = d = L.hv_conv_desc()
         self.x, self.y, self.wuse = x, y, wuse
@@ -189,6 +189,9 @@
             if nout is not None:
                 assert nout.f16 and nout.B == x.B and nout.H == x.H and nout.W == x.W
                 d.xn_out, d.xn_out_ld, d.xn_out_coff = ptr(nout.t).value, nout.ld, nout.coff
+        if wg is not None:
+            assert wg.C == 1 and wg.B == y.B and wg.H == 2 * d.Ho and wg.W == 2 * d.Wo
+            d.wg_x, d.wg_x_ld, d.wg_x_coff, d.wg_x_f16 = ptr(wg.t).value, wg.ld, wg.coff, wg.f16
         if d.Cout == 1:
             need = L.size('hv_conv2d_workspace_bytes', ctypes.byref(d))
             if need:
@@ -209,6 +212,9 @@
 
     def bstats_parts(self):
         return self._probe('hv_conv2d_bstats_parts')
+
+    def wg_parts(self):
+        return self._probe('hv_conv2d_wg_parts')
 
     def launch(self, stats=None):
         L, d, x, y = _lib.get(), self.d, self.x, self.y
@@ -264,6 +270,34 @@
             assert torch.cuda.current_stream().cuda_stream == self.stream, 'FoldChain.flush() on another stream than its weight gradients'
             f, self.pending = self.pending, None
             _lib.get().call('hv_wgrad_fold_now', ctypes.byref(f), stream())
+
+
+def conv2d_dgrad_wgrad(call, dw, dbias, accumulate=False, dbias_accumulate=False, chain=None, store=True):
+    L, d = _lib.get(), call.d
+    parts = int(L.size('hv_conv2d_wg_parts', ctypes.byref(d)))
+    assert parts > 0 and (store or not d.accumulate)
+    nW = 64 * d.Cout
+    if chain is not None and not FOLD_CHAIN:
+        chain = None
+    dev = call.x.t.device
+    if chain is not None:
+        assert torch.cuda.current_stream(dev).cuda_stream == chain.stream, 'a FoldChain belongs to one stream'
+        chain.flush()
+        b, _ = _ws(parts * (nW + d.Cout) * 4, dev, slot=('fold-chain', chain.slot))
+        chain.slot ^= 1
+    else:
+        b, _ = _ws(parts * (nW + d.Cout) * 4, dev)
+    d.wg_parts = ptr(b).value
+    if not store:
+        d.y = None
+    call.launch()
+    fold = L.hv_wgrad_fold()
+    fold.slabs, fold.dw, fold.numel, fold.nslabs, fold.accumulate = ptr(b).value, ptr(dw).value, nW, parts, int(accumulate)
+    fold.bias_slabs, fold.dbias, fold.Cout, fold.dbias_accumulate = ptr(b).value + 4 * parts * nW, ptr(dbias).value, d.Cout, int(dbias_accumulate)
+    if chain is not None:
+        chain.pending = fold
+    else:
+        L.call('hv_wgrad_fold_now', ctypes.byref(fold), stream())
 
 
 FOLD_CHAIN = True
diff --git a/include/hvgan.h b/include/hvgan.h
--- a/include/hvgan.h
+++ b/include/hvgan.h
@@ -49,8 +49,11 @@
     float* bstats;
     const float* xn_stats; const float* xn_gamma; const float* xn_beta; int xn_groups, xn_act;
     void* xn_out; int xn_out_ld, xn_out_coff;
+    const void* wg_x; int wg_x_ld, wg_x_coff, wg_x_f16;
+    float* wg_parts;
 } hv_conv_desc;
 int hv_conv2d(const hv_conv_desc* d, void* stream);
+size_t hv_conv2d_wg_parts(const hv_conv_desc* d);
 size_t hv_conv2d_bstats_parts(const hv_conv_desc* d);
 size_t hv_conv2d_workspace_bytes(const hv_conv_desc* d);
 size_t hv_conv2d_stats_parts(const hv_conv_desc* d);
```

Result: no change. 2526 slices/s, median of 6 (+1.0%).
